# MorphIQ-Labs/VectorWave

Hardware: AMD Instinct MI355X
Metric: Msamples/sec MODWT fwd+inv db4 L=6, batch 4096×4096 fp64 @ 1/2/4/8 GPU (higher is better)
Workload: dtype f64

## Files before the change

vectorwave_amd/csrc/vw_capi.cpp:

```cpp
#include "../../include/vectorwave_amd.h"
#include "vw_internal.h"
#include "vw_deep.h"

#include <algorithm>
#include <cmath>
#include <cstdarg>
#include <cstdio>
#include <cstring>
#include <map>
#include <mutex>
#include <set>
#include <string>
#include <thread>
#include <vector>

using namespace vw;

static thread_local std::string t_err;
static thread_local int64_t t_err_index = -1;
static thread_local int64_t t_signal_base = 0;

static vw_status fail(vw_status code, const char* fmt, ...) {
  char buf[512];
  va_list ap;
  va_start(ap, fmt);
  vsnprintf(buf, sizeof(buf), fmt, ap);
  va_end(ap);
  t_err = buf;
  if (code != VW_ERR_NONFINITE) t_err_index = -1;
  return code;
}

static vw_status ok() {
  t_err.clear();
  t_err_index = -1;
  return VW_OK;
}

#define VW_HIP(call)                                                                         \
  do {                                                                                       \
    hipError_t e_ = (call);                                                                  \
    if (e_ != hipSuccess) return fail(VW_ERR_DEVICE, "%s: %s", #call, hipGetErrorString(e_)); \
  } while (0)

#define VW_TRY(expr)                      \
  do {                                    \
    vw_status s_ = (expr);                \
    if (s_ != VW_OK) return s_;           \
  } while (0)

struct TimedLaunch {
  std::string family;
  hipEvent_t start, stop;
  bool graph_owned = false;
};

struct Tuning {
  int nv = 4;
  bool fwd_persist = true;
  int fwd_buf = 0;
  bool force_tiled = false;
  int fwd_rev = 0, inv_rev = 0;
  int dma_nt = -1;
  int fwd_tile = 0;
  bool multi = true;
  int multi_div = 4;
  int multi_tile = 0;
  int inv_buf = 0;
  int inv_tile = 0;
  int multi_rblk = 1;
  int multi_pf = 1;
  int multi_pad = 1;
  int multi_inv_tile = 0;
  int multi_ni = 4;
  bool no_sweep = false;
  int sweep_qc = kSweepChunk;
  int unroll_max = kMaxTaps;
  int blk = 10;
  bool deep = true;
  bool deep_inv = false;
  int deep_lds = 80;
  int deep_waves = 4;
  int deep_pf_fwd = 1;
  int deep_pf_inv = 1;
  int fwd_nv = 0;
  int inv_nv = 0;
  int sweep2 = 3;
  int sweep2_ka = 8;
  int sweep2_uc = 2048;
  int sweep2_r = 0;
  int sweep2_minb = 64;
  int blk_fwd8 = 1;
  int ref_grid = 0;
  int mfma = 0;
};

static bool set_tuning(Tuning& t, const char* key, int v) {
  const Tuning d;
  const std::string k(key);
  if (k == "VW_NV") t.nv = v < 0 ? d.nv : v <= 4 ? 4 : 8;
  else if (k == "VW_FWD_PERSIST") t.fwd_persist = v < 0 ? d.fwd_persist : v != 0;
  else if (k == "VW_FWD_BUF") t.fwd_buf = v < 0 ? d.fwd_buf : v;
  else if (k == "VW_FORCE_TILED") t.force_tiled = v > 0;
  else if (k == "VW_FWD_REV") t.fwd_rev = v < 0 ? 0 : v;
  else if (k == "VW_INV_REV") t.inv_rev = v < 0 ? 0 : v;
  else if (k == "VW_DMA_NT") t.dma_nt = v < 0 ? d.dma_nt : v;
  else if (k == "VW_FWD_TILE") t.fwd_tile = v < 0 ? 0 : v;
  else if (k == "VW_MULTI") t.multi = v < 0 ? d.multi : v != 0;
  else if (k == "VW_MULTI_DIV") t.multi_div = v <= 0 ? d.multi_div : v;
  else if (k == "VW_MULTI_TILE") t.multi_tile = v < 0 ? 0 : v;
  else if (k == "VW_INV_BUF") t.inv_buf = v < 0 ? 0 : v;
  else if (k == "VW_INV_TILE") t.inv_tile = v < 0 ? 0 : v;
  else if (k == "VW_MULTI_RBLK") t.multi_rblk = v < 0 ? d.multi_rblk : v;
  else if (k == "VW_MULTI_PF") t.multi_pf = v < 0 ? d.multi_pf : v;
  else if (k == "VW_MULTI_PAD") t.multi_pad = v < 0 ? d.multi_pad : v;
  else if (k == "VW_MULTI_INV_TILE") t.multi_inv_tile = v < 0 ? 0 : v;
  else if (k == "VW_MULTI_NI") t.multi_ni = v < 0 ? d.multi_ni : v == 4 ? 4 : 8;
  else if (k == "VW_NO_SWEEP") t.no_sweep = v > 0;
  else if (k == "VW_SWEEP_QC") t.sweep_qc = v >= 16 ? v : d.sweep_qc;
  else if (k == "VW_UNROLL_MAX") t.unroll_max = v < 0 ? d.unroll_max : v;
  else if (k == "VW_BLK") t.blk = v < 0 ? d.blk : v;
  else if (k == "VW_DEEP") { t.deep = v < 0 ? d.deep : v != 0; t.deep_inv = v < 0 ? d.deep_inv : v != 0; }
  else if (k == "VW_DEEP_INV") t.deep_inv = v < 0 ? d.deep_inv : v != 0;
  else if (k == "VW_DEEP_LDS") t.deep_lds = v <= 0 ? d.deep_lds : v;
  else if (k == "VW_DEEP_WAVES") t.deep_waves = v <= 0 ? d.deep_waves : v;
  else if (k == "VW_DEEP_PF_FWD") t.deep_pf_fwd = v <= 0 ? d.deep_pf_fwd : std::min(v, 16);
  else if (k == "VW_DEEP_PF_INV") t.deep_pf_inv = v <= 0 ? d.deep_pf_inv : std::min(v, 16);
  else if (k == "VW_FWD_NV") t.fwd_nv = v < 0 ? d.fwd_nv : v;
  else if (k == "VW_INV_NV") t.inv_nv = v < 0 ? d.inv_nv : v;
  else if (k == "VW_SWEEP2") t.sweep2 = v < 0 ? d.sweep2 : v;
  else if (k == "VW_SWEEP2_KA") t.sweep2_ka = v == 16 ? 16 : v == 8 ? 8 : d.sweep2_ka;
  else if (k == "VW_SWEEP2_UC") t.sweep2_uc = v >= 32 ? v : d.sweep2_uc;
  else if (k == "VW_SWEEP2_R") t.sweep2_r = v == 32 ? 32 : 0;
  else if (k == "VW_SWEEP2_MINB") t.sweep2_minb = v < 0 ? d.sweep2_minb : v;
  else if (k == "VW_BLK_FWD8") t.blk_fwd8 = v < 0 ? d.blk_fwd8 : v;
  else if (k == "VW_MFMA") t.mfma = v < 0 ? d.mfma : v;
  else if (k == "VW_REF_GRID") t.ref_grid = v < 0 ? d.ref_grid : v;
  else return false;
  return true;
}

static const char* const kTuningKeys[] = {
    "VW_NV", "VW_FWD_PERSIST", "VW_FWD_BUF", "VW_FORCE_TILED", "VW_FWD_REV", "VW_INV_REV",
    "VW_FWD_TILE", "VW_MULTI", "VW_MULTI_DIV", "VW_MULTI_TILE", "VW_INV_BUF", "VW_INV_TILE", "VW_MULTI_RBLK", "VW_MULTI_PF", "VW_MULTI_PAD", "VW_MULTI_INV_TILE", "VW_NO_SWEEP", "VW_SWEEP_QC",
    "VW_UNROLL_MAX", "VW_BLK", "VW_FWD_NV",
    "VW_INV_NV", "VW_DEEP", "VW_DEEP_INV", "VW_DEEP_LDS", "VW_DEEP_WAVES", "VW_DEEP_PF_FWD", "VW_DEEP_PF_INV",
    "VW_SWEEP2", "VW_SWEEP2_KA", "VW_SWEEP2_UC", "VW_SWEEP2_R", "VW_SWEEP2_MINB", "VW_BLK_FWD8",
    "VW_DMA_NT", "VW_MULTI_NI", "VW_MFMA", "VW_REF_GRID"};

static Tuning read_tuning() {
  Tuning t;
  for (const char* k : kTuningKeys) {
    const char* e = getenv(k);
    if (!e) continue;
    const int v = (*e == '\0') ? 1 : atoi(e);
    set_tuning(t, k, v);
  }
  return t;
}

struct vw_graph;
struct vw_ctx;
static void kill_pipelines_of(vw_ctx* c);

struct vw_ctx {
  int device = 0;
  hipStream_t stream = nullptr;
  bool own_stream = false;
  bool capturing = false;
  unsigned ws_gen = 0;
  Tuning tune;
  int cus = 256;
  std::recursive_mutex mu;
  void* ws = nullptr;
  size_t ws_bytes = 0;
  void* ws2 = nullptr;
  size_t ws2_bytes = 0;
  unsigned long long* bad = nullptr;
  bool timing = false;
  std::vector<TimedLaunch> pending;
  std::vector<TimedLaunch> captured;
  std::vector<hipEvent_t> event_pool;
  std::map<std::string, std::pair<double, int64_t>> totals;
  std::set<vw_graph*> graphs;
  std::vector<std::pair<void*, size_t>> stage;
  void* med = nullptr;
  size_t med_bytes = 0;
  int* nf = nullptr;
  int64_t nf_rows = 0;
};

struct vw_graph {
  vw_ctx* ctx = nullptr;
  int device = 0;
  unsigned ws_gen = 0;
  std::vector<TimedLaunch> timed;
  hipGraph_t graph = nullptr;
  hipGraphExec_t exec = nullptr;
};

static void release_graph(vw_graph* gr) {
  for (auto& t : gr->timed) { hipEventDestroy(t.start); hipEventDestroy(t.stop); }
  gr->timed.clear();
  if (gr->exec) hipGraphExecDestroy(gr->exec);
  if (gr->graph) hipGraphDestroy(gr->graph);
  gr->exec = nullptr;
  gr->graph = nullptr;
}

struct vw_stream {
  vw_ctx* ctx = nullptr;
  std::vector<double> lo, hi;
  int L = 0;
  int boundary = 0;
  int levels = 0;
  int64_t last_batch = -1;
  bool hist_init = false;
  std::vector<double*> hist;
  std::vector<double*> snap;
  std::vector<int> hist_len;
};

static hipEvent_t pool_event(vw_ctx* c) {
  if (!c->event_pool.empty()) {
    hipEvent_t e = c->event_pool.back();
    c->event_pool.pop_back();
    return e;
  }
  hipEvent_t e = nullptr;
  if (hipEventCreate(&e) != hipSuccess) return nullptr;
  return e;
}

static bool capture_event(hipStream_t st, hipEvent_t ev) {
  hipStreamCaptureStatus status;
  unsigned long long id = 0;
  hipGraph_t g = nullptr;
  const hipGraphNode_t* deps = nullptr;
  size_t ndeps = 0;
  if (hipStreamGetCaptureInfo_v2(st, &status, &id, &g, &deps, &ndeps) == hipSuccess &&
      status == hipStreamCaptureStatusActive && g) {
    hipGraphNode_t node = nullptr;
    if (hipGraphAddEventRecordNode(&node, g, deps, ndeps, ev) == hipSuccess &&
        hipStreamUpdateCaptureDependencies(st, &node, 1, hipStreamSetCaptureDependencies) == hipSuccess)
      return true;
  }
  (void)hipGetLastError();
  if (hipEventRecordWithFlags(ev, st, hipEventRecordExternal) == hipSuccess) return true;
  (void)hipGetLastError();
  return false;
}

struct LaunchTimer {
  vw_ctx* c;
  TimedLaunch tl;
  bool on;
  LaunchTimer(vw_ctx* ctx, const char* family) : c(ctx), on(ctx->timing) {
    if (!on) return;
    tl.family = family;
    if (c->capturing) {
      tl.graph_owned = true;
      tl.start = tl.stop = nullptr;
      if (hipEventCreate(&tl.start) != hipSuccess || hipEventCreate(&tl.stop) != hipSuccess ||
          !capture_event(c->stream, tl.start)) {
        if (tl.start) hipEventDestroy(tl.start);
        if (tl.stop) hipEventDestroy(tl.stop);
        on = false;
      }
      return;
    }
    tl.start = pool_event(c);
    tl.stop = pool_event(c);
    if (!tl.start || !tl.stop) { on = false; return; }
    hipEventRecord(tl.start, c->stream);
  }
  ~LaunchTimer() {
    if (!on) return;
    if (tl.graph_owned) {
      if (capture_event(c->stream, tl.stop)) {
        c->captured.push_back(tl);
      } else {
        hipEventDestroy(tl.start);
        hipEventDestroy(tl.stop);
      }
      return;
    }
    hipEventRecord(tl.stop, c->stream);
    c->pending.push_back(tl);
  }
};

static void collect_timing(vw_ctx* c) {
  for (auto& tl : c->pending) {
    float ms = 0.f;
    if (hipEventSynchronize(tl.stop) == hipSuccess && hipEventElapsedTime(&ms, tl.start, tl.stop) == hipSuccess) {
      auto& t = c->totals[tl.family];
      t.first += ms;
      t.second += 1;
    }
    if (!tl.graph_owned) {
      c->event_pool.push_back(tl.start);
      c->event_pool.push_back(tl.stop);
    }
  }
  c->pending.clear();
}

static vw_status ensure_ws(vw_ctx* c, size_t bytes) {
  if (bytes <= c->ws_bytes) return VW_OK;
  if (c->capturing) return fail(VW_ERR_STATE, "workspace growth during capture: run the call once before capturing it");
  if (c->ws) {
    hipDeviceSynchronize();
    ++c->ws_gen;
    hipFree(c->ws);
    c->ws = nullptr;
    c->ws_bytes = 0;
  }
  size_t want = std::max(bytes, (size_t)1 << 20);
  VW_HIP(hipMalloc(&c->ws, want));
  c->ws_bytes = want;
  return VW_OK;
}

static vw_status ensure_nf(vw_ctx* c, int64_t B) {
  if (B <= c->nf_rows) return VW_OK;
  if (c->capturing) return fail(VW_ERR_STATE, "row-flag growth during capture: run the call once before capturing it");
  if (c->nf) {
    hipDeviceSynchronize();
    ++c->ws_gen;
    hipFree(c->nf);
    c->nf = nullptr;
    c->nf_rows = 0;
  }
  const int64_t rows = std::max<int64_t>(B, 4096);
  VW_HIP(hipMalloc(&c->nf, (size_t)rows * sizeof(int)));
  VW_HIP(hipMemset(c->nf, 0, (size_t)rows * sizeof(int)));
  VW_HIP(hipDeviceSynchronize());
  c->nf_rows = rows;
  return VW_OK;
}

static inline size_t align_up(size_t v, size_t a) { return (v + a - 1) / a * a; }
static inline int64_t round_up(int64_t v, int64_t a) { return (v + a - 1) / a * a; }


extern "C" int vw_max_levels(int64_t N, int L) {
  if (L <= 0 || N <= L) return 0;
  int max_level = 1;
  const long long lm1 = L - 1;
  while (max_level < 10) {
    const long long scaled = lm1 * (1LL << (max_level - 1)) + 1LL;
    if (scaled > N) break;
    max_level++;
  }
  return max_level - 1;
}

extern "C" int64_t vw_upsampled_length(int L, int level) {
  const int64_t up = (level <= 1) ? 1 : ((int64_t)1 << (level - 1));
  return (int64_t)(L - 1) * up + 1;
}

static void sym_decide(int wid, int L, int level, int* ap, int* dh, int* dp, int* dg) {
  int detailPlus = 1, deltaG = 0, deltaH = 0;
  const bool isHaar = L <= 2;
  int approxPlus = isHaar ? 1 : 0;
  if (isHaar) {
    deltaG = 0;
    deltaH = (level <= 1) ? 0 : -1;
  } else if (wid == VW_WID_DB6) {
    deltaH = (level <= 1) ? 0 : -1;
    deltaG = (level >= 3) ? 1 : 0;
  } else if (wid == VW_WID_DB8) {
    deltaH = (level <= 1) ? 0 : 1;
    deltaG = (level >= 2) ? 1 : 0;
  } else if (wid == VW_WID_SYM4) {
    approxPlus = 1; detailPlus = 0; deltaH = 0; deltaG = 0;
  } else if (wid == VW_WID_SYM8) {
    if (level <= 1) { deltaH = 0; deltaG = 0; }
    else if (level == 2) { deltaH = 1; deltaG = 0; }
    else { deltaH = 1; deltaG = 1; }
  } else if (wid == VW_WID_COIF2) {
    approxPlus = 1; deltaH = (level <= 1) ? 0 : 1; detailPlus = 0; deltaG = 0;
  } else if (wid == VW_WID_COIF3) {
    detailPlus = 0;
    if (level <= 1) { deltaH = 0; deltaG = 0; } else { deltaH = -1; deltaG = 1; }
  } else if (L >= 12) {
    if (level <= 1) { deltaH = 0; deltaG = 0; }
    else { const bool even = level % 2 == 0; deltaH = even ? 0 : -1; deltaG = even ? 0 : -1; }
  } else {
    if (level <= 1) { deltaH = 0; deltaG = 0; } else { deltaH = -1; deltaG = 0; }
  }
  *ap = approxPlus; *dh = deltaH; *dp = detailPlus; *dg = deltaG;
}

static int compute_tau(int base_len, int level) {
  const int lm1 = base_len - 1;
  if (level <= 1) return std::max(0, lm1 / 2);
  const long long up = 1LL << (level - 1);
  const long long Lj = (long long)lm1 * up + 1LL;
  const long long tau = (Lj - 1LL) / 2LL;
  if (tau < 0) return 0;
  if (tau > 2147483647LL) return 2147483647;
  return (int)tau;
}

static int next_pow2(int64_t n) {
  int64_t p = 1;
  while (p < n) p <<= 1;
  return (int)p;
}

static bool is_pow2(int64_t n) { return n > 0 && (n & (n - 1)) == 0; }

static void branch_extent(int N, int tmax, int L, int s, int dir, int off, int* hl, int* hr) {
  const long long reach = (long long)(L - 1) * s;
  long long mn, mx;
  if (dir > 0) { mn = off; mx = (long long)tmax + reach + off; }
  else { mn = (long long)off - reach; mx = (long long)tmax + off; }
  *hl = (int)std::max<long long>(*hl, -mn);
  *hr = (int)std::max<long long>(*hr, mx - (N - 1));
}

template <typename T> static constexpr int vec_width() { return 16 / (int)sizeof(T); }

static bool aligned16(const void* p) { return ((uintptr_t)p & 15u) == 0; }

extern "C" vw_status vw_ctx_create(int device, vw_ctx** out) {
  if (!out) return fail(VW_ERR_NULL, "out is null");
  int n = 0;
  VW_HIP(hipGetDeviceCount(&n));
  if (device < 0 || device >= n) return fail(VW_ERR_ARG, "device %d out of range (%d devices)", device, n);
  VW_HIP(hipSetDevice(device));
  vw_ctx* c = new vw_ctx();
  c->device = device;
  c->tune = read_tuning();
  { int n = 0; if (hipDeviceGetAttribute(&n, hipDeviceAttributeMultiprocessorCount, device) == hipSuccess && n > 0) c->cus = n; }
  if (hipStreamCreateWithFlags(&c->stream, hipStreamNonBlocking) != hipSuccess) {
    delete c;
    return fail(VW_ERR_DEVICE, "hipStreamCreate failed");
  }
  c->own_stream = true;
  if (hipMalloc(&c->bad, sizeof(unsigned long long)) != hipSuccess) {
    hipStreamDestroy(c->stream);
    delete c;
    return fail(VW_ERR_DEVICE, "hipMalloc failed");
  }
  *out = c;
  return ok();
}

// ... 425 lines not shown
}

template <typename T>
static void copy_taps(T* dst, const double* src, int L) {
  const double s = 1.0 / std::sqrt(2.0);
  for (int i = 0; i < L; ++i) dst[i] = (T)(src[i] * s);
  for (int i = L; i < kMaxTaps; ++i) dst[i] = T(0);
}

static vw_status capture_guard(vw_ctx* c, unsigned flags) {
  if (c->capturing && (flags & (VW_FLAG_VALIDATE | VW_FLAG_HOST_MEMORY | VW_FLAG_SYNC)))
    return fail(VW_ERR_STATE, "validation, host memory and SYNC cannot be captured");
  return VW_OK;
}

static vw_status read_bad(vw_ctx* c, unsigned long long* out) {
  VW_HIP(hipMemcpyAsync(out, c->bad, sizeof(unsigned long long), hipMemcpyDeviceToHost, c->stream));
  VW_HIP(hipStreamSynchronize(c->stream));
  return VW_OK;
}

static vw_status report_bad(unsigned long long bad, int64_t N) {
  if (bad == ~0ull) return VW_OK;
  const bool out = (bad >> 62) & 1ull;
  const unsigned long long flat = bad & ((1ull << 62) - 1);
  t_err_index = (int64_t)(flat % (unsigned long long)N);
  return fail(VW_ERR_NONFINITE, "%s contains non-finite value at index %lld (signal %lld)",
              out ? "coefficients" : "signal", (long long)(flat % (unsigned long long)N),
              (long long)(flat / (unsigned long long)N) + (long long)t_signal_base);
}

static bool fused_plan(const Tuning& tu, int64_t N, int V, int elem, int64_t lds_elems_extra, int* threads, int* nv,
                       int* lds, bool* fit, int nv_req = 0) {
  const int64_t nvec = (N + V - 1) / V;
  int want = tu.nv;
  if ((nvec + want - 1) / want > 512) want = 8;
  if (nv_req == 2 && nvec % 2 == 0 && nvec / 2 <= kMaxThreads) want = 2;
  const int64_t th = (nvec + want - 1) / want;
  if (th > kMaxThreads) return false;
  const int64_t bytes = lds_elems_extra * elem;
  if (bytes > kLdsBytes) return false;
  *nv = want;
  *threads = (int)th;
  *lds = (int)bytes;
  *fit = (int64_t)(want - 1) * th <= nvec;
  return true;
}


static void set_halo_images(LevelDesc& d, int64_t N, int64_t npow2, int V, int threads, int nv) {
  int64_t s_el = 0, e_el = N;
  d.il_a = 0; d.il_b = 1; d.ir_a = 0; d.ir_b = -1;
  switch (d.mode) {
    case kHaloPeriodic:
      d.il_a = 1; d.il_b = (int)-N; d.ir_a = 1; d.ir_b = (int)N;
      s_el = d.hr; e_el = N - d.hl;
      break;
    case kHaloSymmetric:
      d.il_a = -1; d.il_b = -1; d.ir_a = -1; d.ir_b = (int)(2 * N - 1);
      s_el = d.hl; e_el = N - d.hr;
      break;
    case kHaloFftPad:
      d.il_a = 1; d.il_b = (int)-npow2;
      e_el = npow2 - d.hl;
      break;
    default:
      break;
  }
  e_el = std::min<int64_t>(std::max<int64_t>(e_el, 0), N);
  d.vs = (int)((s_el + V - 1) / V);
  d.ve = (int)(e_el / V);
  d.own = (d.hl <= N && d.hr <= N && d.vs <= threads && (int64_t)d.ve >= (int64_t)(nv - 1) * threads) ? 1 : 0;
}

template <typename T>
static int multi_tile(const Tuning& tu) {
  constexpr int V = vec_width<T>();
  const int v = tu.multi_tile ? tu.multi_tile : (int)(16384 / sizeof(T));
  return v >= 64 * V ? v / V * V : 64 * V;
}

static std::vector<int> level_groups(const Tuning& tu, const std::vector<LevelDesc>& lv, int J, int L, int V, int tile,
                                     bool ok) {
  std::vector<int> g(J, 1);
  if (!ok || !tu.multi) return g;
  const int64_t cap = tile / tu.multi_div;
  for (int j = 1; j <= J;) {
    int n = 0;
    int64_t ext = 0;
    while (j + n <= J && n < kMaxGroup && lv[j + n - 1].mode == kHaloPeriodic) {
      const int64_t e2 = ext + round_up((int64_t)(L - 1) * lv[j + n - 1].s, V);
      if (e2 > cap) break;
      ext = e2;
      ++n;
    }
    if (n >= 2) {
      g[j - 1] = n;
      for (int k = 1; k < n; ++k) g[j - 1 + k] = 0;
      j += n;
    } else {
      ++j;
    }
  }
  return g;
}

template <typename T>
static bool sweepg_plan(const Tuning& tu, const std::vector<LevelDesc>& lv, int j, int levels, int L, int64_t N,
                        const std::vector<char>& in_group, const std::vector<int>& start_of, int* ka_out, int* r_out) {
  if (levels < 2 || levels > 3 || j < levels) return false;
  const int G = levels == 2 ? 2 : 4;
  const int64_t h = lv[j - levels].s;
  if (h < kSweepMinS || h % 32 != 0 || lv[j - 1].s != G * h) return false;
  for (int k = j - levels + 1; k <= j; ++k) {
    const LevelDesc& d = lv[k - 1];
    if (d.mode != kHaloPeriodic || d.dir_a != 1 || d.dir_d != 1 || d.off_a != 0 || d.off_d != 0) return false;
    if (k < j && (in_group[k] || start_of[k] != 0)) return false;
  }
  const int R = (h % 64 == 0 && tu.sweep2_r != 32) ? 64 : 32;
  const int kmin = (levels == 2 ? 1 : 2) * (L - 1);
  for (int ka : {L <= 17 ? tu.sweep2_ka : 16, 16}) {
    for (int r : {R, 32}) {
      const int64_t kb = (int64_t)G * ka;
      const int64_t lds = (levels == 2 ? 1 : 2) * 3 * kb * r * (int64_t)sizeof(T);
      if (kb < kmin || lds > kLdsBytes || h % r != 0) continue;
      if (N % (G * h) != 0 || (2 * kb + 2 * L) * G * h > N) continue;
      if (N / h < (int64_t)tu.sweep2_minb * kb) continue;
      *ka_out = ka;
      *r_out = r;
      return true;
    }
  }
  return false;
}

constexpr int kDeepTile = 128;

template <typename T>
static int deep_plan(const Tuning& tu, const std::vector<LevelDesc>& lv, int jlo, int jhi, int L, int64_t N,
                     bool inverse, DeepArgs<T>* a) {
  constexpr int V = vec_width<T>();
  const int C = 64 / (int)sizeof(T);
  const int g = jhi - jlo + 1;
  if (!(inverse ? tu.deep_inv : tu.deep) || g < 1 || g > kMaxGroup || !has_unrolled_taps(L)) return 0;
  const int P = lv[jlo - 1].s;
  if (P < C || P % C != 0 || N % P != 0 || N / P < 2 * kDeepTile) return 0;
  for (int j = jlo; j <= jhi; ++j)
    if (lv[j - 1].mode != kHaloPeriodic) return 0;
  (void)V;
  int caps[2 * kMaxGroup] = {}, nr = 0;
  int64_t reach = 0;
  const int D = inverse ? tu.deep_pf_inv : tu.deep_pf_fwd;
  for (int k = 0; k < g; ++k) {
    const int64_t H = (int64_t)(L - 1) << k;
    reach += H;
    const bool dma_fed = inverse ? (k == g - 1) : (k == 0);
    caps[k] = dma_fed ? (int)round_up(H + (D + 1) * kDeepTile, 16) : (int)(H + kDeepTile);
    if (inverse) caps[g + k] = (int)round_up(H + (D + 1) * kDeepTile, 16);
  }
  nr = inverse ? 2 * g : g;
  int64_t pos = 0;
  for (int r = 0; r < nr; ++r) pos += caps[r];
  const int64_t bytes = pos * 64;
  if (bytes > (int64_t)tu.deep_lds * 1024 || bytes > kLdsBytes) return 0;
  if (a) {
    a->P = P; a->C = C; a->nq = (int)(N / P); a->nb = P / C; a->g = g; a->N = (int)N;
    a->warm = (int)round_up(reach, kDeepTile);
    a->depth = D;
    int64_t o = 0;
    for (int r = 0; r < nr; ++r) { a->cap[r] = caps[r]; a->off[r] = (int)(o * C); o += caps[r]; }
  }
  return (int)bytes;
}

template <typename T>
static void deep_segments(const Tuning& tu, int cus, int64_t B, DeepArgs<T>* a) {
  const int64_t wg0 = B * a->nb;
  int64_t seg = std::max<int64_t>(1, ((int64_t)tu.deep_waves * cus + wg0 - 1) / wg0);
  seg = std::min<int64_t>(seg, std::max<int64_t>(1, a->nq / (4 * (int64_t)a->warm)));
  a->seg = (int)seg;
  a->seglen = (int)round_up((a->nq + seg - 1) / seg, kDeepTile);
  a->seg = (int)((a->nq + a->seglen - 1) / a->seglen);
}

template <typename T>
struct ScanPlane {
  const T* p;
  int64_t ld;
  int len;
};

template <typename T>
static vw_status ref_nonfinite(vw_ctx* c, const std::vector<ScanPlane<T>>& planes, RefArgs<T>& r,
                               bool inverse, bool flagged) {
  const int64_t B = r.B, N = r.N;
  if ((int)planes.size() > kRefPlanes) return fail(VW_ERR_ARG, "too many planes for the non-finite scan");
  int64_t grid = std::min<int64_t>(B, c->tune.ref_grid > 0 ? c->tune.ref_grid : 2LL * c->cus);
  grid = std::max<int64_t>(1, std::min<int64_t>(grid, ((int64_t)512 << 20) / (2 * N * (int64_t)sizeof(T))));
  VW_TRY(ensure_nf(c, B));
  VW_TRY(ensure_ws(c, (size_t)grid * 2 * (size_t)N * sizeof(T)));
  LaunchTimer lt(c, flagged ? "ref_nonfinite" : "ref_nonfinite_scan");
  hipError_t e;
  if (!flagged) {
    RefScan<T> s;
    memset(&s, 0, sizeof(s));
    for (const auto& p : planes) {
      s.p[s.np] = p.p;
      s.ld[s.np] = p.ld;
      s.len[s.np] = p.len;
      ++s.np;
    }
    s.B = B; s.N = (int)N; s.chunks = ref_scan_chunks((int)N); s.flag = c->nf;
    e = launch_flag_nonfinite<T>(s, c->stream);
    if (e != hipSuccess) return fail(VW_ERR_DEVICE, "non-finite scan launch failed: %s", hipGetErrorString(e));
  }
  r.flag = c->nf;
  r.scratch = reinterpret_cast<T*>(c->ws);
  e = launch_ref_cascade<T>(r, (int)grid, inverse, c->stream);
  if (e != hipSuccess) return fail(VW_ERR_DEVICE, "reference-arithmetic launch failed: %s", hipGetErrorString(e));
  return VW_OK;
}

static hipError_t mfma_forward(const FwdArgs<float>& a, int lds, hipStream_t st) { return launch_forward_mfma(a, lds, st); }
static hipError_t mfma_forward(const FwdArgs<double>&, int, hipStream_t) { return hipErrorNotSupported; }
static hipError_t mfma_inverse(const InvArgs<float>& a, int lds, hipStream_t st) { return launch_inverse_mfma(a, lds, st); }
static hipError_t mfma_inverse(const InvArgs<double>&, int, hipStream_t) { return hipErrorNotSupported; }

static int ref_mode(int boundary) {
  return boundary == VW_PERIODIC ? kHaloPeriodic : boundary == VW_ZERO_PADDING ? kHaloZero : kHaloSymmetric;
}

template <typename T>
static vw_status forward_impl(vw_ctx* c, const T* x, int64_t B, int64_t N, int64_t ldx, const double* lo,
                              const double* hi, int L, int boundary, int J, unsigned flags, T* details, T* approx,
                              bool single_level, int mode_override, T* const* hist, bool hist_update,
                              T* const* hist_snap = nullptr, bool hist_first = false) {
  constexpr int V = vec_width<T>();
  VW_TRY(capture_guard(c, flags));
  const bool fma = flags & VW_FLAG_FMA;
  const bool validate = flags & VW_FLAG_VALIDATE;
  const int64_t nvec = (N + V - 1) / V;

  std::vector<LevelDesc> lv(J);
  int max_hl = 0;
  const int npow2 = next_pow2(N);
  for (int j = 1; j <= J; ++j) {
    LevelDesc& d = lv[j - 1];
    memset(&d, 0, sizeof(d));
    d.s = 1 << (j - 1);
    const int64_t Lj = vw_upsampled_length(L, j);
    d.hl = (int)(Lj - 1);
    d.hr = 0;
    d.hist_len = (int)(Lj - 1);
    if (boundary == VW_PERIODIC) {
      d.mode = kHaloPeriodic;
      if ((flags & VW_FLAG_FFT_SWITCH) && !single_level && !(N < 64 || Lj > N / 2) && N >= 1024 &&
          (double)Lj > N * (1.0 / 8.0) && !is_pow2(N))
        d.mode = kHaloFftPad;
    } else {
      d.mode = boundary == VW_ZERO_PADDING ? kHaloZero : kHaloSymmetric;
    }
    if (mode_override >= 0) d.mode = mode_override;
    max_hl = std::max(max_hl, d.hl);
  }
  if ((flags & VW_FLAG_REF_NONFINITE) && hist && hist_update && hist_snap && !hist_first && J >= 2)
    for (int j = 0; j < J; ++j)
      if (lv[j].hist_len > 0)
        VW_HIP(hipMemcpyAsync(hist_snap[j], hist[j], (size_t)B * lv[j].hist_len * sizeof(T), hipMemcpyDeviceToDevice,
                              c->stream));

  const int hlpad = (int)round_up(max_hl, V);
  int threads = 0, lds = 0, nv = 4;
  const Tuning& tu = c->tune;
  const bool persist_on = tu.fwd_persist;
  const bool ref_nf = (flags & VW_FLAG_REF_NONFINITE) && !validate && !single_level && J >= 2 &&
                      !(flags & VW_FLAG_FFT_SWITCH) && (!hist || !hist_update || hist_first || hist_snap);
  bool nf_probed = false;
  const bool io_aligned = (ldx % V == 0) && (N % V == 0) && aligned16(x) && aligned16(details) && aligned16(approx);
  auto persist_ok = [&](int th, int nvv, bool ft) {
    return persist_on && io_aligned && ft && nvv == 4 && !validate && !hist && (int64_t)th * nvv == nvec &&
           th % 64 == 0 && nvec % 64 == 0 && has_unrolled_taps(L) && J >= 1;
  };
  const int64_t region = round_up(hlpad + nvec * V + V, V);
  bool dbl = tu.fwd_buf ? tu.fwd_buf == 2 : true;
  bool fused = false, fit = false;
  const int fwd_nv2 = (tu.fwd_nv == 2 && io_aligned && L <= 8 && L <= tu.unroll_max && has_unrolled_taps(L) &&
                       !(tu.blk > 0 && L >= tu.blk)) ? 2 : 0;
  if (J <= kMaxLevels && !tu.force_tiled) {
    if (dbl) dbl = fused_plan(tu, N, V, sizeof(T), 2 * region, &threads, &nv, &lds, &fit, fwd_nv2);
    if (dbl && !tu.fwd_buf && !fma && !persist_ok(threads, nv, fit)) dbl = false;
    fused = dbl || fused_plan(tu, N, V, sizeof(T), region, &threads, &nv, &lds, &fit, fwd_nv2);
  }
  if (fused && nv == 2 && !(fit && (int64_t)threads * 2 == nvec)) return fail(VW_ERR_STATE, "NV=2 plan without full slabs");
  if (fused) {
    for (int j = 0; j < J; ++j) set_halo_images(lv[j], N, npow2, V, threads, nv);
    FwdArgs<T> a;
    memset(&a, 0, sizeof(a));
    a.x = x; a.ldx = ldx; a.details = details; a.approx = approx; a.B = B; a.N = (int)N; a.J = J;
    a.npow2 = npow2; a.hlpad = hlpad; a.region1 = dbl ? (int)region : 0;
    a.vec_io = (ldx % V == 0) && (N % V == 0) && aligned16(x) && aligned16(details) && aligned16(approx);
    a.unrolled = a.vec_io && fit && L <= tu.unroll_max;
    a.validate = validate; a.bad = c->bad;
    a.rev = tu.fwd_rev;
    a.dma_nt = tu.dma_nt >= 0 ? tu.dma_nt : (B <= 2LL * c->cus ? 1 : 0);
    for (int j = 0; j < J; ++j) a.hist[j] = hist ? hist[j] : nullptr;
    a.hist_update = hist_update ? 1 : 0;
    a.taps = L;
    copy_taps(a.lo, lo, L);
    copy_taps(a.hi, hi, L);
    for (int j = 0; j < J; ++j) a.lv[j] = lv[j];
    if (validate) VW_HIP(hipMemsetAsync(c->bad, 0xFF, sizeof(unsigned long long), c->stream));
    const bool persist = dbl && a.unrolled && persist_ok(threads, nv, fit);
    int blk_lds = 0;
    if (tu.blk > 0 && L >= tu.blk && a.unrolled && !validate && !hist && (int64_t)threads * nv == nvec &&
        (nv == 4 || (nv == 8 && tu.blk_fwd8))) {
      bool okb = true;
      int hlv = 0;
      for (int j = 0; j < J; ++j) {
        if (lv[j].mode != kHaloPeriodic) okb = false;
        hlv = std::max<int>(hlv, (int)(((int64_t)(L - 1) * lv[j].s + V - 1) / V));
      }
      if (round_up(hlv, 16) <= nvec) hlv = (int)round_up(hlv, 16);
      const int mJ = std::max(1, lv[J - 1].s / V);
      if (nvec % ((int64_t)nv * mJ) != 0 || hlv > nvec) okb = false;
      auto buf_of = [&](int tight) {
        int64_t bf = 0;
        for (int j = 0; j < J; ++j) {
          int sh, pd;
          blk_layout_host(lv[j].s / V, nv, &sh, &pd, tight);
          const int64_t u = hlv + nvec - 1;
          bf = std::max(bf, u + (u >> sh) * pd + 1);
        }
        return bf;
      };
      int64_t buf = buf_of(0);
      if (buf * 16 + 2 * L * (int64_t)sizeof(T) > kLdsBytes && nv >= 8) {
        a.blk_tight = 1;
        buf = buf_of(1);
      }
      if (okb && buf * 16 <= kLdsBytes) {
        const bool two = 2 * buf * 16 <= 80 * 1024;
        a.region1 = two ? (int)(buf * V) : 0;
        a.hlpad = hlv * V;
        a.tap_lds = (int)(buf * V * (two ? 2 : 1));
        blk_lds = (int)(buf * 16 * (two ? 2 : 1)) + 2 * L * (int)sizeof(T);
        if (blk_lds > kLdsBytes) blk_lds = 0;
      }
    }
    int mfma_lds = 0;
    if constexpr (std::is_same<T, float>::value) {
      bool ok = (tu.mfma & 1) && fma && !single_level && a.vec_io && !validate && !hist && mfma_supported(L, N);
      for (int j = 0; ok && j < J; ++j) ok = lv[j].mode == kHaloPeriodic;
      const int H = ok ? mfma_halo(L, J) : 0;
      const int region = ok ? mfma_region((int)N + H) : 0;
      const int scratch = 8 * 256 + 4;
      if (ok && H <= N && (int64_t)(region + 2 * L + scratch) * 4 <= kLdsBytes) {
        a.hlpad = H;
        a.tap_lds = region;
        mfma_lds = (int)((region + 2 * L + scratch) * 4);
      }
    }
    if (ref_nf && !mfma_lds && (blk_lds || persist)) {
      VW_TRY(ensure_nf(c, B));
      a.nf_flag = c->nf;
      nf_probed = true;
    }
    {
      LaunchTimer lt(c, "forward");
      hipError_t e = mfma_lds ? mfma_forward(a, mfma_lds, c->stream)
                   : blk_lds ? launch_forward_blk<T>(a, threads, blk_lds, fma, nv, c->stream)
                   : persist ? launch_forward_persist<T>(a, threads, lds, fma, nv, c->stream)
                             : launch_forward_fused<T>(a, threads, lds, fma, nv, c->stream);
      if (e != hipSuccess) return fail(VW_ERR_DEVICE, "forward launch failed: %s", hipGetErrorString(e));
    }
  } else {
    for (int j = 1; hist && j <= J; ++j)
      if (lv[j - 1].hist_len > N) return fail(VW_ERR_UNSUPPORTED, "streaming block shorter than level %d history", j);
    const int tile_max = tu.fwd_tile ? tu.fwd_tile / V * V : 256 * kNV * V;
    const size_t plane = (size_t)B * (size_t)N;
    const vw_status st = ensure_ws(c, 2 * plane * sizeof(T) + 256);
    if (st != VW_OK) return st;
    T* tmp[2] = {reinterpret_cast<T*>(c->ws), reinterpret_cast<T*>(c->ws) + plane};
    if (validate) VW_HIP(hipMemsetAsync(c->bad, 0xFF, sizeof(unsigned long long), c->stream));
    const T* src = x;
    int64_t lda = ldx;
    const int mtile = multi_tile<T>(tu);
    const std::vector<int> groups = level_groups(tu, lv, J, L, V, mtile, !validate && !hist);
    for (int j = 1; j <= J; ++j) {
      T* const nxt = (src == tmp[0]) ? tmp[1] : tmp[0];
      if (groups[j - 1] == 1 && !validate && !hist && (lda % V) == 0 && aligned16(src) && aligned16(details) &&
          aligned16(approx) && deep_plan<T>(tu, lv, j, j, L, N, false, nullptr)) {
        int je = j;
        while (je < J && groups[je] == 1 && deep_plan<T>(tu, lv, j, je + 1, L, N, false, nullptr)) ++je;
        DeepArgs<T> d;
        memset(&d, 0, sizeof(d));
        const int lds = deep_plan<T>(tu, lv, j, je, L, N, false, &d);
        deep_segments<T>(tu, c->cus, B, &d);
        d.src = src; d.lda = lda; d.B = B; d.taps = L;
        d.out = (je == J) ? approx : nxt;
        if (ref_nf && je == J) {
          VW_TRY(ensure_nf(c, B));
          d.nf_flag = c->nf;
          nf_probed = true;
        }
        for (int k = 0; k < d.g; ++k) d.out_d[k] = details + (size_t)(j - 1 + k) * plane;
        copy_taps(d.lo, lo, L);
        copy_taps(d.hi, hi, L);
        {
          LaunchTimer lt(c, "forward_level");
          hipError_t e = launch_deep<T>(d, lds, fma, false, c->stream);
          if (e != hipSuccess) return fail(VW_ERR_DEVICE, "forward deep launch failed: %s", hipGetErrorString(e));
        }
        src = d.out;
        lda = N;
        j = je;
        continue;
      }
      if (groups[j - 1] >= 2) {
        const int g = groups[j - 1], je = j + g - 1;
        MultiArgs<T> m;
        memset(&m, 0, sizeof(m));
        m.src_a = src; m.lda = lda;
        m.out_a = (je == J) ? approx : nxt;
        bool al = aligned16(src) && aligned16(m.out_a);
        for (int k = 0; k < g; ++k) {
          m.out_d[k] = details + (size_t)(j - 1 + k) * plane;
          al = al && aligned16(m.out_d[k]);
        }
        m.ext[g] = 0;
        for (int k = g - 1; k >= 0; --k)
          m.ext[k] = m.ext[k + 1] + (int)round_up((int64_t)(L - 1) * lv[j - 1 + k].s, V);
        m.B = B; m.N = (int)N; m.tile = mtile; m.nlev = g; m.s0 = lv[j - 1].s;
        m.region = (int)round_up(m.ext[0] + mtile + V, V);
        m.vec_io = (N % V == 0) && (lda % V == 0) && al;
        m.taps = L;
        copy_taps(m.lo, lo, L);
        copy_taps(m.hi, hi, L);
        {
          LaunchTimer lt(c, "forward_level");
          hipError_t e = launch_forward_multi<T>(m, (int)(2 * m.region * sizeof(T)), fma, c->stream);
          if (e != hipSuccess) return fail(VW_ERR_DEVICE, "forward multi-level launch failed: %s", hipGetErrorString(e));
        }
        src = m.out_a;
        lda = N;
        j = je;
        continue;
      }
      LevelArgs<T> a;
      memset(&a, 0, sizeof(a));
      a.lv = lv[j - 1];
      const int hp = (int)round_up(a.lv.hl, V);
      const int64_t fit = ((int64_t)kLdsBytes / (int64_t)sizeof(T) - hp - 2 * V) / V * V;
      const int tile = (int)std::min<int64_t>(tile_max, fit);
      if (tile < 64 * V) return fail(VW_ERR_UNSUPPORTED, "level %d halo (%d samples) exceeds LDS", j, a.lv.hl);
      const int64_t elems = hp + tile + V;
      a.src_a = src; a.lda = lda;
      a.out_a = (j == J) ? approx : nxt;
      a.out_d = details + (size_t)(j - 1) * plane;
      a.hist = hist ? hist[j - 1] : nullptr;
      a.B = B; a.N = (int)N; a.tile = tile; a.hlpad = hp;
      a.vec_io = (N % V == 0) && (lda % V == 0) && aligned16(src) && aligned16(a.out_a) && aligned16(a.out_d);
      a.validate = validate; a.bad = c->bad; a.npow2 = npow2; a.taps = L;
      copy_taps(a.lo, lo, L);
      copy_taps(a.hi, hi, L);
      const bool sweep = a.lv.s >= kSweepMinS && has_unrolled_taps(L) && !tu.no_sweep;
      {
        LaunchTimer lt(c, "forward_level");
        hipError_t e;
        if (sweep) {
          a.tile = tu.sweep_qc;
          e = launch_forward_sweep<T>(a, fma, c->stream);
        } else {
          e = launch_forward_level<T>(a, (int)(elems * sizeof(T)), fma, c->stream);
        }
        if (e != hipSuccess) return fail(VW_ERR_DEVICE, "forward level launch failed: %s", hipGetErrorString(e));
      }
      if (hist && hist_update) {
        hipError_t e = launch_history_update<T>(src, lda, hist[j - 1], hist[j - 1], B, (int)N, a.lv.hist_len,
                                                c->stream);
        if (e != hipSuccess) return fail(VW_ERR_DEVICE, "history update failed: %s", hipGetErrorString(e));
      }
      src = a.out_a;
      lda = N;
    }
  }
  if (ref_nf) {
    std::vector<ScanPlane<T>> planes{{approx, N, 0}};
    RefArgs<T> r;
    memset(&r, 0, sizeof(r));
    r.x = x; r.ldx = ldx; r.details = details; r.approx = approx;
    r.B = B; r.N = (int)N; r.J = J; r.L = L; r.mode = ref_mode(boundary);
    if (hist) {
      r.hist_mode = 1;
      r.hist_first = hist_first ? 1 : 0;
      for (int j = 0; j < J; ++j) {
        const int hl = lv[j].hist_len;
        r.hist_len[j] = hl;
        r.hist_old[j] = hist_first ? nullptr : (hist_update ? hist_snap[j] : hist[j]);
        r.hist_new[j] = hist_update ? hist[j] : nullptr;
      }
    }
    copy_taps(r.lo, lo, L);
    copy_taps(r.hi, hi, L);
    VW_TRY(ref_nonfinite<T>(c, planes, r, false, nf_probed));
  }
  if (validate) {
    unsigned long long bad = 0;
    vw_status st = read_bad(c, &bad);
    if (st != VW_OK) return st;
    st = report_bad(bad, N);
    if (st != VW_OK) return st;
  }
  if (flags & VW_FLAG_SYNC) VW_HIP(hipStreamSynchronize(c->stream));
  return VW_OK;
}

template <typename T>
static vw_status inverse_impl(vw_ctx* c, const T* details, const T* approx, int64_t B, int64_t N, const double* lo,
                              const double* hi, int L, int wid, int boundary, int J, unsigned detail_mask,
                              int approx_zero, unsigned flags, T* y, bool single_level, const T* thr, int soft,
                              int64_t thr_ld = 0) {
  constexpr int V = vec_width<T>();
  VW_TRY(capture_guard(c, flags));
  const bool fma = flags & VW_FLAG_FMA;
  const int64_t nvec = (N + V - 1) / V;
  const int tmax = (int)(nvec * V - 1);
  const bool pair = single_level || boundary == VW_ZERO_PADDING;
  const bool ref_nf = (flags & VW_FLAG_REF_NONFINITE) && !single_level && J >= 2;
  bool nf_probed = false;

  std::vector<LevelDesc> lv(J);
  int max_hl = 0, max_hr = 0;
  for (int j = 1; j <= J; ++j) {
    LevelDesc& d = lv[j - 1];
    memset(&d, 0, sizeof(d));
    d.s = 1 << (j - 1);
    d.use_d = (detail_mask >> (j - 1)) & 1u;
    d.mode = boundary == VW_PERIODIC ? kHaloPeriodic : boundary == VW_ZERO_PADDING ? kHaloZero : kHaloSymmetric;
    if (boundary == VW_SYMMETRIC && !single_level) {
      int ap, dh, dp, dg;
      sym_decide(wid, L, j, &ap, &dh, &dp, &dg);
      const int tauH = compute_tau(L, j) + dh;
      const int tauG = compute_tau(L, j) + dg;
      d.dir_a = ap ? 1 : -1; d.off_a = ap ? -tauH : tauH;
      d.dir_d = dp ? 1 : -1; d.off_d = dp ? -tauG : tauG;
    } else if (boundary == VW_SYMMETRIC) {
      const int dir = (flags & VW_FLAG_BATCH_SYM_INVERSE) ? 1 : -1;
      d.dir_a = d.dir_d = dir; d.off_a = d.off_d = 0;
    } else {
      d.dir_a = d.dir_d = 1; d.off_a = d.off_d = 0;
    }
    int hl = 0, hr = 0;
    branch_extent((int)N, tmax, L, d.s, d.dir_a, d.off_a, &hl, &hr);
    branch_extent((int)N, tmax, L, d.s, d.dir_d, d.off_d, &hl, &hr);
    d.hl = hl; d.hr = hr;
    max_hl = std::max(max_hl, hl);
    max_hr = std::max(max_hr, hr);
  }
  const int hlpad = (int)round_up(max_hl, V);
  const int64_t region = round_up(hlpad + nvec * V + max_hr + V, V);
  int threads = 0, lds = 0, nv = 4;
  const Tuning& tu = c->tune;
  const bool blk_pref = tu.blk > 0 && L >= tu.blk && boundary == VW_PERIODIC;
  bool db = !pair && (tu.inv_buf ? tu.inv_buf == 2 : (B <= 2LL * c->cus && !blk_pref));
  bool fused = false, fit = false;
  const bool inv_io = (N % V == 0) && aligned16(details) && aligned16(approx) && aligned16(y);
  const int inv_nv2 = (tu.inv_nv == 2 && inv_io && L <= 8 && L <= tu.unroll_max && has_unrolled_taps(L)) ? 2 : 0;
  if (!tu.force_tiled) {
    if (pair || db) fused = fused_plan(tu, N, V, sizeof(T), 2 * region, &threads, &nv, &lds, &fit, inv_nv2);
    if (!fused && !pair) {
      db = false;
      fused = fused_plan(tu, N, V, sizeof(T), region, &threads, &nv, &lds, &fit, inv_nv2);
    }
  }
  if (fused) {
    for (int j = 0; j < J; ++j) set_halo_images(lv[j], N, 0, V, threads, nv);
    InvArgs<T> a;
    memset(&a, 0, sizeof(a));
    a.details = details; a.approx = approx; a.y = y; a.B = B; a.N = (int)N; a.J = J;
    a.db = db ? 1 : 0;
    a.hlpad_a = hlpad; a.hlpad_d = hlpad; a.region_d = (int)region;
    a.vec_io = (N % V == 0) && aligned16(details) && aligned16(approx) && aligned16(y);
    a.unrolled = a.vec_io && fit && L <= tu.unroll_max;
    a.pair = pair; a.approx_zero = approx_zero; a.thr = thr; a.thr_ld = thr_ld; a.soft = soft; a.taps = L;
    a.rev = tu.inv_rev;
    if (tu.blk > 0 && L >= tu.blk && nv != 2 && !pair && !db && boundary == VW_PERIODIC && a.unrolled &&
        (int64_t)threads * nv == nvec) {
      bool okb = true;
      int64_t buf = 0;
      const int mJ = std::max(1, lv[J - 1].s / V);
      if (nvec % ((int64_t)nv * mJ) != 0) okb = false;
      int64_t buf_t = 0;
      for (int j = 0; j < J && okb; ++j) {
        if (lv[j].dir_a != 1 || lv[j].dir_d != 1 || lv[j].off_a != 0 || lv[j].off_d != 0) okb = false;
        const int64_t hrv = ((int64_t)(L - 1) * lv[j].s + V - 1) / V;
        if (hrv > nvec) okb = false;
        int sh, pd;
        const int64_t u = nvec + hrv - 1;
        blk_layout_host(lv[j].s / V, nv, &sh, &pd);
        buf = std::max(buf, u + (u >> sh) * pd + 1);
        blk_layout_host(lv[j].s / V, nv, &sh, &pd, 1);
        buf_t = std::max(buf_t, u + (u >> sh) * pd + 1);
      }
      const int64_t taps_b = 2 * L * (int64_t)sizeof(T);
      if (okb && buf * 16 + taps_b > kLdsBytes && nv >= 8 && buf_t * 16 + taps_b <= kLdsBytes) {
        a.blk_tight = 1;
        buf = buf_t;
      }
      if (okb && buf * 16 + taps_b <= kLdsBytes) {
        a.blk = 1;
        a.tap_lds = (int)(buf * V);
        lds = (int)(buf * 16) + 2 * L * (int)sizeof(T);
      }
    }
    copy_taps(a.lo, lo, L);
    copy_taps(a.hi, hi, L);
    for (int j = 0; j < J; ++j) a.lv[j] = lv[j];
    int mfma_lds = 0;
    if constexpr (std::is_same<T, float>::value) {
      bool ok = (tu.mfma & 2) && fma && !pair && boundary == VW_PERIODIC && a.vec_io && mfma_supported(L, N);
      for (int j = 0; ok && j < J; ++j) ok = lv[j].dir_a == 1 && lv[j].dir_d == 1 && lv[j].off_a == 0 && lv[j].off_d == 0;
      const int H = ok ? mfma_halo(L, J) : 0;
      const int region = ok ? mfma_region((int)N + H) : 0;
      if (ok && H <= N && (int64_t)(region + 2 * L) * 4 <= kLdsBytes) {
        a.hlpad_a = H;
        a.tap_lds = region;
        mfma_lds = (int)((region + 2 * L) * 4);
      }
    }
    if (ref_nf && !mfma_lds && !a.pair && !a.db) {
      VW_TRY(ensure_nf(c, B));
      a.nf_flag = c->nf;
      nf_probed = true;
    }
    LaunchTimer lt(c, "inverse");
    hipError_t e = mfma_lds ? mfma_inverse(a, mfma_lds, c->stream) : launch_inverse_fused<T>(a, threads, lds, fma, nv, c->stream);
    if (e != hipSuccess) return fail(VW_ERR_DEVICE, "inverse launch failed: %s", hipGetErrorString(e));
  } else {
    const int tile_max = tu.inv_tile ? tu.inv_tile / V * V : 1024;
    const size_t plane = (size_t)B * (size_t)N;
    const vw_status st = ensure_ws(c, 2 * plane * sizeof(T) + 256);
    if (st != VW_OK) return st;
    T* tmp[2] = {reinterpret_cast<T*>(c->ws), reinterpret_cast<T*>(c->ws) + plane};
    const T* cur = approx_zero ? nullptr : approx;
    const int mtile = tu.multi_inv_tile >= 64 * V ? tu.multi_inv_tile / V * V : multi_tile<T>(tu);
    const std::vector<int> groups = level_groups(tu, lv, J, L, V, mtile, !pair && boundary == VW_PERIODIC);
    std::vector<int> start_of(J + 1, 0);
    for (int j = 1; j <= J; ++j) {
      if (groups[j - 1] < 2) continue;
      int64_t ext = 0;
      for (int k = 0; k < groups[j - 1]; ++k) ext += round_up((int64_t)(L - 1) * lv[j - 1 + k].s, V);
      if ((mtile + ext) / V <= (int64_t)kMultiInvNI * 256) start_of[j + groups[j - 1] - 1] = j;
    }
    std::vector<char> in_group(J + 1, 0);
    for (int e = 1; e <= J; ++e)
      for (int k = start_of[e]; start_of[e] > 0 && k <= e; ++k) in_group[k] = 1;
    for (int j = J; j >= 1; --j) {
      T* const nxt = (cur == tmp[0]) ? tmp[1] : tmp[0];
      if (!pair && boundary == VW_PERIODIC && !in_group[j] && aligned16(cur) && aligned16(details) &&
          aligned16(y) && deep_plan<T>(tu, lv, j, j, L, N, true, nullptr)) {
        int jl = j;
        while (jl > 1 && !in_group[jl - 1] && deep_plan<T>(tu, lv, jl - 1, j, L, N, true, nullptr)) --jl;
        DeepArgs<T> d;
        memset(&d, 0, sizeof(d));
        const int lds = deep_plan<T>(tu, lv, jl, j, L, N, true, &d);
        deep_segments<T>(tu, c->cus, B, &d);
        d.src = cur; d.lda = N; d.B = B; d.taps = L; d.soft = soft;
        d.out = (jl == 1) ? y : nxt;
        for (int k = 0; k < d.g; ++k) {
          const LevelDesc& ld = lv[jl - 1 + k];
          d.src_d[k] = ld.use_d ? details + (size_t)(jl - 1 + k) * plane : nullptr;
          d.thr[k] = thr ? thr + (size_t)(jl - 1 + k) * (size_t)thr_ld : nullptr;
        }
        copy_taps(d.lo, lo, L);
        copy_taps(d.hi, hi, L);
        {
          LaunchTimer lt(c, "inverse_level");
          hipError_t e = launch_deep<T>(d, lds, fma, true, c->stream);
          if (e != hipSuccess) return fail(VW_ERR_DEVICE, "inverse deep launch failed: %s", hipGetErrorString(e));
        }
        cur = d.out;
        j = jl;
        continue;
      }
      if (start_of[j] > 0) {
        const int j0 = start_of[j], g = j - j0 + 1;
        MultiArgs<T> m;
        memset(&m, 0, sizeof(m));
        m.src_a = cur;
        m.out_a = (j0 == 1) ? y : nxt;
        if (ref_nf && j0 == 1) {
          VW_TRY(ensure_nf(c, B));
          m.nf_flag = c->nf;
          nf_probed = true;
        }
        bool al = aligned16(cur) && aligned16(m.out_a);
        for (int k = 0; k < g; ++k) {
          const LevelDesc& d = lv[j0 - 1 + k];
          m.src_d[k] = d.use_d ? details + (size_t)(j0 - 1 + k) * plane : nullptr;
          m.thr[k] = thr ? thr + (size_t)(j0 - 1 + k) * (size_t)thr_ld : nullptr;
          al = al && aligned16(m.src_d[k]);
          m.ext[k] = (k > 0 ? m.ext[k - 1] : 0) + (int)round_up((int64_t)(L - 1) * d.s, V);
        }
        m.B = B; m.N = (int)N; m.tile = mtile; m.nlev = g; m.s0 = lv[j0 - 1].s;
        m.region = (int)round_up(mtile + m.ext[g - 1] + V, V);
        m.vec_io = (N % V == 0) && al;
        m.soft = soft; m.taps = L;
        m.rblk = tu.multi_rblk;
        m.pf = tu.multi_pf && m.vec_io && (int64_t)(mtile + m.ext[g - 1]) / V <= (int64_t)kMultiPF * 256;
        m.pad = tu.multi_pad && m.pf && m.rblk && has_unrolled_taps(L);
        if (m.pad) {
          const int nvmax = (mtile + m.ext[g - 1]) / V + 1;
          m.region = (nvmax + nvmax / 8 + 1) * V;
        }
        m.slack = 160;
        m.ni = kMultiInvNI;
        if (tu.multi_ni == 4 && sizeof(T) == 8 && m.pad) {
          auto fits = [&](int64_t t) {
            if ((t + m.ext[g - 1]) / V > (int64_t)kMultiPF * 256) return false;
            for (int k = 0; k < g; ++k) {
              const int64_t s = lv[j0 - 1 + k].s, M = s % V == 0 ? s / V : 0;
              const int64_t nv = (t + (k > 0 ? m.ext[k - 1] : 0)) / V;
              const bool blk = M == 1 || M == 2 || M == 4 || M == 8;
              if (blk ? (nv + 4 * M - 1) / (4 * M) * M > 256 : nv > 4 * 256) return false;
            }
            return true;
          };
          int64_t t = mtile;
          while (t >= 512 && !fits(t)) t -= 64 * V;
          if (t >= 512) {
            m.ni = 4;
            m.tile = (int)t;
            const int nvmax = (int)((t + m.ext[g - 1]) / V) + 1;
            m.region = (nvmax + nvmax / 4 + 1) * V;
          }
        }
        copy_taps(m.lo, lo, L);
        copy_taps(m.hi, hi, L);
        LaunchTimer lt(c, "inverse_level");
        hipError_t e = launch_inverse_multi<T>(m, (int)((2 * m.region + m.slack * V) * sizeof(T)), fma, c->stream);
        if (e != hipSuccess) return fail(VW_ERR_DEVICE, "inverse multi-level launch failed: %s", hipGetErrorString(e));
        cur = m.out_a;
        j = j0;
        continue;
      }
      if (tu.sweep2 && !tu.deep_inv && !tu.no_sweep && !pair && j >= 2 && has_unrolled_taps(L)) {
        int G = 0, ka = 0, R = 0;
        for (int levels = std::min(tu.sweep2 >= 3 ? 3 : 2, j); levels >= 2 && !G; --levels)
          if (sweepg_plan<T>(tu, lv, j, levels, L, N, in_group, start_of, &ka, &R)) G = levels;
        if (G) {
          const LevelDesc& lj = lv[j - 1];
          LevelArgs<T> a;
          memset(&a, 0, sizeof(a));
          a.lv = lj;
          a.src_a = cur;
          a.src_d = lj.use_d ? details + (size_t)(j - 1) * plane : nullptr;
          a.use_d = lj.use_d;
          a.thr = thr ? thr + (size_t)(j - 1) * (size_t)thr_ld : nullptr;
          a.src_d2 = lv[j - 2].use_d ? details + (size_t)(j - 2) * plane : nullptr;
          a.use_d2 = lv[j - 2].use_d;
          a.thr2 = thr ? thr + (size_t)(j - 2) * (size_t)thr_ld : nullptr;
          if (G == 3) {
            a.src_d3 = lv[j - 3].use_d ? details + (size_t)(j - 3) * plane : nullptr;
            a.use_d3 = lv[j - 3].use_d;
            a.thr3 = thr ? thr + (size_t)(j - 3) * (size_t)thr_ld : nullptr;
          }
          a.soft = soft;
          a.out_a = (j == G) ? y : nxt;
          a.B = B; a.N = (int)N; a.taps = L;
          const int kb = (G == 2 ? 2 : 4) * ka;
          a.tile = (int)round_up(tu.sweep2_uc, kb);
          copy_taps(a.lo, lo, L);
          copy_taps(a.hi, hi, L);
          LaunchTimer lt(c, "inverse_level");
          hipError_t e = launch_inverse_sweepg<T>(a, G == 2 ? 2 : 4, ka, R, fma, c->stream);
          if (e != hipSuccess) return fail(VW_ERR_DEVICE, "inverse level-group launch failed: %s", hipGetErrorString(e));
          cur = a.out_a;
          j -= G - 1;
          continue;
        }
      }
      LevelArgs<T> a;
      memset(&a, 0, sizeof(a));
      a.lv = lv[j - 1];
      const int hp = (int)round_up(a.lv.hl, V);
      const int64_t fit = ((int64_t)kLdsBytes / (int64_t)sizeof(T) / 2 - hp - a.lv.hr - 2 * V) / V * V;
      const int tile = (int)std::min<int64_t>(tile_max, fit);
      if (tile < 64 * V) return fail(VW_ERR_UNSUPPORTED, "level %d halo exceeds LDS", j);
      const int64_t reg = round_up(hp + tile + a.lv.hr + V, V);
      a.src_a = cur;
      a.src_d = a.lv.use_d ? details + (size_t)(j - 1) * plane : nullptr;
      a.use_d = a.lv.use_d;
      a.out_a = (j == 1) ? y : nxt;
      a.B = B; a.N = (int)N; a.tile = tile; a.hlpad = hp; a.hlpad_d = hp; a.region_d = (int)reg;
      a.pair = pair; a.thr = thr ? thr + (size_t)(j - 1) * (size_t)thr_ld : nullptr; a.soft = soft; a.taps = L;
      a.vec_io = (N % V == 0) && aligned16(a.out_a) && aligned16(a.src_a) && aligned16(a.src_d);
      copy_taps(a.lo, lo, L);
      copy_taps(a.hi, hi, L);
      LaunchTimer lt(c, "inverse_level");
      hipError_t e;
      if (a.lv.s >= kSweepMinS && has_unrolled_taps(L) && !tu.no_sweep) {
        a.tile = tu.sweep_qc;
        e = launch_inverse_sweep<T>(a, fma, c->stream);
      } else {
        e = launch_inverse_level<T>(a, (int)(2 * reg * sizeof(T)), fma, c->stream);
      }
      if (e != hipSuccess) return fail(VW_ERR_DEVICE, "inverse level launch failed: %s", hipGetErrorString(e));
      cur = a.out_a;
    }
  }
  if (ref_nf) {
    std::vector<ScanPlane<T>> planes{{y, N, 0}};
    RefArgs<T> r;
    memset(&r, 0, sizeof(r));
    r.x = approx_zero ? nullptr : approx; r.det_in = details; r.y = y;
    r.thr = thr; r.thr_ld = thr_ld; r.soft = soft;
    r.B = B; r.N = (int)N; r.J = J; r.L = L; r.mode = ref_mode(boundary);
    copy_taps(r.lo, lo, L);
    copy_taps(r.hi, hi, L);
    for (int j = 0; j < J; ++j) r.lv[j] = lv[j];
    VW_TRY(ref_nonfinite<T>(c, planes, r, true, nf_probed));
  }
  if (flags & VW_FLAG_SYNC) VW_HIP(hipStreamSynchronize(c->stream));
  return VW_OK;
}

struct Staging {
  vw_ctx* c;
  size_t used_block = 0, used_off = 0;
  explicit Staging(vw_ctx* ctx) : c(ctx) {}
  ~Staging() {
    hipStreamSynchronize(c->stream);
    if (c->stage.size() > 1) {
      auto big = std::max_element(c->stage.begin(), c->stage.end(),
                                  [](const std::pair<void*, size_t>& a, const std::pair<void*, size_t>& b) {
                                    return a.second < b.second;
                                  });
      const auto keep = *big;
      for (auto& blk : c->stage)
        if (blk.first != keep.first) hipFree(blk.first);
      c->stage.assign(1, keep);
    }
  }
  vw_status carve(size_t bytes, void** out) {
    bytes = align_up(std::max<size_t>(bytes, 16), 256);
    for (; used_block < c->stage.size(); ++used_block, used_off = 0) {
      auto& blk = c->stage[used_block];
      if (used_off + bytes <= blk.second) {
        *out = static_cast<char*>(blk.first) + used_off;
        used_off += bytes;
        return VW_OK;
      }
    }
    size_t carved = bytes;
    for (size_t k = 0; k < used_block && k < c->stage.size(); ++k) carved += c->stage[k].second;
    if (used_block < c->stage.size()) carved += used_off;
    const size_t want = std::max({carved, (size_t)4 << 20});
    void* p = nullptr;
    VW_HIP(hipMalloc(&p, want));
    c->stage.push_back({p, want});
    used_block = c->stage.size() - 1;
    used_off = bytes;
    *out = p;
    return VW_OK;
  }
  template <typename T>
  vw_status in(const T* host, size_t count, T** dev) {
    void* p = nullptr;
    VW_TRY(carve(count * sizeof(T), &p));
    if (host && count) VW_HIP(hipMemcpyAsync(p, host, count * sizeof(T), hipMemcpyHostToDevice, c->stream));
    *dev = reinterpret_cast<T*>(p);
    return VW_OK;
  }
  template <typename T>
  vw_status in_planes(const T* host, size_t planes, size_t count, size_t host_stride, T** dev) {
    void* p = nullptr;
    VW_TRY(carve(planes * count * sizeof(T), &p));
    if (host && count && planes)
      VW_HIP(hipMemcpy2DAsync(p, count * sizeof(T), host, host_stride * sizeof(T), count * sizeof(T), planes,
                              hipMemcpyHostToDevice, c->stream));
    *dev = reinterpret_cast<T*>(p);
    return VW_OK;
  }
  template <typename T>
  vw_status out(T* host, const T* dev, size_t count) {
    if (host && count) VW_HIP(hipMemcpyAsync(host, dev, count * sizeof(T), hipMemcpyDeviceToHost, c->stream));
    return VW_OK;
  }
// ... 1021 lines not shown
```

vectorwave_amd/csrc/vw_device.h:

```cpp
#pragma once
#include <hip/hip_runtime.h>
#include <cstdint>
#include <type_traits>
#include "vw_internal.h"

#pragma clang fp contract(off)

namespace vw {

template <typename T> struct VT;
template <> struct VT<double> { typedef double v __attribute__((ext_vector_type(2))); static constexpr int V = 2; };
template <> struct VT<float>  { typedef float  v __attribute__((ext_vector_type(4))); static constexpr int V = 4; };

__device__ __forceinline__ double fma_t(double a, double b, double c) { return __builtin_fma(a, b, c); }
__device__ __forceinline__ float fma_t(float a, float b, float c) { return __builtin_fmaf(a, b, c); }

template <bool FMA, typename T>
__device__ __forceinline__ T madd(T acc, T x, T f) {
  if constexpr (FMA) return fma_t(x, f, acc);
  else return acc + x * f;
}

#ifndef VW_PK_F32
#define VW_PK_F32 0
#endif
#ifndef VW_PK_F32_FWD
#define VW_PK_F32_FWD 1
#endif
constexpr bool kPkFwd = VW_PK_F32_FWD != 0;
template <bool FMA, bool PK = (VW_PK_F32 != 0), typename T, typename X>
__device__ __forceinline__ void vmadd(T* acc, const X& x, T f) {
  if constexpr (PK && std::is_same<T, float>::value) {
    typedef float f2 __attribute__((ext_vector_type(2)));
    const f2 fv = {f, f};
#pragma unroll
    for (int h = 0; h < 2; ++h) {
      f2 a = {acc[2 * h], acc[2 * h + 1]};
      const f2 xv = {x[2 * h], x[2 * h + 1]};
      if constexpr (FMA) a = __builtin_elementwise_fma(xv, fv, a);
      else a = a + xv * fv;
      acc[2 * h] = a[0];
      acc[2 * h + 1] = a[1];
    }
  } else {
#pragma unroll
    for (int e = 0; e < VT<T>::V; ++e) acc[e] = madd<FMA>(acc[e], x[e], f);
  }
}

template <typename T>
__device__ __forceinline__ T load_uniform(const T* q) {
  typedef const __attribute__((address_space(4))) T* cptr;
  return *(cptr)(q);
}

__device__ __forceinline__ bool finite_t(double v) { return __builtin_isfinite(v); }
__device__ __forceinline__ bool finite_t(float v) { return __builtin_isfinite(v); }

__device__ __forceinline__ int sym_index(int idx, int n) {
  if (idx >= 0 && idx < n) return idx;
  int period = 2 * n;
  idx = ((idx % period) + period) % period;
  if (idx >= n) idx = period - idx - 1;
  return idx;
}

#pragma clang diagnostic push
#pragma clang diagnostic ignored "-Wint-to-pointer-cast"
template <typename vec>
__device__ __forceinline__ vec lds_vec_at(unsigned a) {
  return *(const __attribute__((address_space(3))) vec*)a;
}
#pragma clang diagnostic pop
template <typename T>
__device__ __forceinline__ unsigned lds_base(const T* p) {
  unsigned a = (unsigned)(uintptr_t)p;
  asm volatile("" : "+v"(a));
  return a;
}

__device__ __forceinline__ void lds_barrier() {
  asm volatile("" ::: "memory");
  __builtin_amdgcn_s_waitcnt(0xC07F);
  __builtin_amdgcn_s_barrier();
  asm volatile("" ::: "memory");
}

__device__ __forceinline__ void wait_vmem() { __builtin_amdgcn_s_waitcnt(0x0F70); }

template <typename T>
__device__ __forceinline__ T halo_value_lds(const T* buf, int idx, int N, int mode, int npow2,
                                            const T* hist_b, int hist_len) {
  switch (mode) {
    case kHaloPeriodic: { int r = idx % N; if (r < 0) r += N; return buf[r]; }
    case kHaloSymmetric: return buf[sym_index(idx, N)];
    case kHaloFftPad: { int r = idx < 0 ? idx + npow2 : idx; return (r >= 0 && r < N) ? buf[r] : T(0); }
    case kHaloHistory: return (idx < 0 && idx >= -hist_len) ? hist_b[hist_len + idx] : T(0);
    default: return T(0);
  }
}

template <typename T>
__device__ __forceinline__ void fill_halo(T* buf, int N, int hl, int hr, int mode, int npow2,
                                          const T* hist_b, int hist_len) {
  const int total = hl + hr;
  if (mode == kHaloHistory) {
    for (int q = threadIdx.x; q < total; q += blockDim.x) {
      const int idx = q < hl ? q - hl : N + (q - hl);
      buf[idx] = (idx < 0 && idx >= -hist_len) ? hist_b[hist_len + idx] : T(0);
    }
    return;
  }
  for (int q = threadIdx.x; q < total; q += blockDim.x) {
    const int idx = q < hl ? q - hl : N + (q - hl);
    buf[idx] = halo_value_lds(buf, idx, N, mode, npow2, (const T*)nullptr, 0);
  }
}

constexpr int kWinTaps = 8;

__host__ __device__ constexpr int floor_div(int a, int b) { return a >= 0 ? a / b : -((-a + b - 1) / b); }

template <int C, int NC, typename F>
__device__ __forceinline__ void static_for(F&& f) {
  if constexpr (C < NC) {
    f(std::integral_constant<int, C>{});
    static_for<C + 1, NC>(f);
  }
}

template <typename T, int L, bool FMA, int S>
__device__ __forceinline__ void fwd_window(const T* buf, int t0, const T* lo, const T* hi,
                                           T (&al)[VT<T>::V], T (&ah)[VT<T>::V]) {
  constexpr int V = VT<T>::V;
  using vec = typename VT<T>::v;
  static_for<0, (L + kWinTaps - 1) / kWinTaps>([&](auto c) __attribute__((always_inline)) {
    constexpr int I0 = decltype(c)::value * kWinTaps;
    constexpr int I1 = (I0 + kWinTaps < L) ? I0 + kWinTaps : L;
    constexpr int A = floor_div(-(I1 - 1) * S, V) * V;
    constexpr int E = (floor_div(V - 1 - I0 * S, V) + 1) * V;
    constexpr int NE = E - A;
    T w[NE];
#pragma unroll
    for (int k = 0; k < NE / V; ++k) {
      vec v = *reinterpret_cast<const vec*>(buf + t0 + A + k * V);
#pragma unroll
      for (int e = 0; e < V; ++e) w[k * V + e] = v[e];
    }
    T fl[I1 - I0], fh[I1 - I0];
#pragma unroll
    for (int i = I0; i < I1; ++i) { fl[i - I0] = lo[i]; fh[i - I0] = hi[i]; }
#pragma unroll
    for (int i = I0; i < I1; ++i) {
      vmadd<FMA, kPkFwd>(al, &w[-i * S - A], fl[i - I0]);
      vmadd<FMA, kPkFwd>(ah, &w[-i * S - A], fh[i - I0]);
    }
  });
}

template <typename T, int L, bool FMA>
__device__ __forceinline__ void fwd_vec(const T* buf, int t0, int S, const T* lo, const T* hi, int taps,
                                        T (&al)[VT<T>::V], T (&ah)[VT<T>::V]) {
  constexpr int V = VT<T>::V;
  using vec = typename VT<T>::v;
  if constexpr (L > 0) {
    if (S == 1) { fwd_window<T, L, FMA, 1>(buf, t0, lo, hi, al, ah); return; }
    if constexpr (V == 4) {
      if (S == 2) { fwd_window<T, L, FMA, 2>(buf, t0, lo, hi, al, ah); return; }
    }
#pragma unroll
    for (int i = 0; i < L; ++i) {
      const vec v = *reinterpret_cast<const vec*>(buf + t0 - i * S);
      vmadd<FMA, kPkFwd>(al, v, lo[i]);
      vmadd<FMA, kPkFwd>(ah, v, hi[i]);
    }
  } else {
    for (int i = 0; i < taps; ++i) {
      const T fl = lo[i], fh = hi[i];
#pragma unroll
      for (int e = 0; e < V; ++e) {
        const T xv = buf[t0 + e - i * S];
        al[e] = madd<FMA>(al[e], xv, fl);
        ah[e] = madd<FMA>(ah[e], xv, fh);
      }
    }
  }
}

template <typename T, int L, bool FMA, int S, int DIR>
__device__ __forceinline__ void inv_window(const T* buf, int base, const T* f, T (&acc)[VT<T>::V]) {
  constexpr int V = VT<T>::V;
  using vec = typename VT<T>::v;
  static_for<0, (L + kWinTaps - 1) / kWinTaps>([&](auto c) __attribute__((always_inline)) {
    constexpr int I0 = decltype(c)::value * kWinTaps;
    constexpr int I1 = (I0 + kWinTaps < L) ? I0 + kWinTaps : L;
    constexpr int A = DIR > 0 ? floor_div(I0 * S, V) * V : floor_div(-(I1 - 1) * S, V) * V;
    constexpr int E = DIR > 0 ? (floor_div(V - 1 + (I1 - 1) * S, V) + 1) * V : (floor_div(V - 1 - I0 * S, V) + 1) * V;
    constexpr int NE = E - A;
    T w[NE];
#pragma unroll
    for (int k = 0; k < NE / V; ++k) {
      vec v = *reinterpret_cast<const vec*>(buf + base + A + k * V);
#pragma unroll
      for (int e = 0; e < V; ++e) w[k * V + e] = v[e];
    }
    T fc[I1 - I0];
#pragma unroll
    for (int i = I0; i < I1; ++i) fc[i - I0] = f[i];
#pragma unroll
    for (int i = I0; i < I1; ++i) vmadd<FMA>(acc, &w[DIR * i * S - A], fc[i - I0]);
  });
}

template <typename T, int L, bool FMA>
__device__ __forceinline__ void inv_branch(const T* buf, int t0, int S, int dir, int off, const T* f, int taps,
                                           T (&acc)[VT<T>::V]) {
  constexpr int V = VT<T>::V;
  using vec = typename VT<T>::v;
  if constexpr (L > 0) {
    if ((off & (V - 1)) == 0) {
      const int base = t0 + off;
      if (S == 1) {
        if (dir > 0) inv_window<T, L, FMA, 1, 1>(buf, base, f, acc);
        else inv_window<T, L, FMA, 1, -1>(buf, base, f, acc);
        return;
      }
      if constexpr (V == 4) {
        if (S == 2) {
          if (dir > 0) inv_window<T, L, FMA, 2, 1>(buf, base, f, acc);
          else inv_window<T, L, FMA, 2, -1>(buf, base, f, acc);
          return;
        }
      }
      const int step = dir * S;
#pragma unroll
      for (int i = 0; i < L; ++i) {
        const vec v = *reinterpret_cast<const vec*>(buf + base + i * step);
        vmadd<FMA>(acc, v, f[i]);
      }
      return;
    }
#pragma unroll
    for (int i = 0; i < L; ++i) {
#pragma unroll
      for (int e = 0; e < V; ++e) acc[e] = madd<FMA>(acc[e], buf[t0 + e + dir * i * S + off], f[i]);
    }
  } else {
    for (int i = 0; i < taps; ++i) {
      const T fi = f[i];
#pragma unroll
      for (int e = 0; e < V; ++e) acc[e] = madd<FMA>(acc[e], buf[t0 + e + dir * i * S + off], fi);
    }
  }
}

template <typename T, bool FMA>
__device__ __forceinline__ T pair_term(T h, T a, T g, T d) {
  if constexpr (FMA) return fma_t(h, a, g * d);
  else return h * a + g * d;
}

template <typename T, int L, bool FMA>
__device__ __forceinline__ void inv_pair(const T* A, const T* D, int t0, int S, int dir, const T* h, const T* g,
                                         int taps, T (&acc)[VT<T>::V]) {
  constexpr int V = VT<T>::V;
  using vec = typename VT<T>::v;
  if constexpr (L > 0) {
    if (S % V == 0) {
      const int step = dir * S;
#pragma unroll
      for (int i = 0; i < L; ++i) {
        const vec va = *reinterpret_cast<const vec*>(A + t0 + i * step);
        const vec vd = *reinterpret_cast<const vec*>(D + t0 + i * step);
#pragma unroll
        for (int e = 0; e < V; ++e) acc[e] = acc[e] + pair_term<T, FMA>(h[i], va[e], g[i], vd[e]);
        if ((i & 3) == 3) __builtin_amdgcn_sched_barrier(0);
      }
      return;
    }
#pragma unroll
    for (int i = 0; i < L; ++i) {
#pragma unroll
      for (int e = 0; e < V; ++e) {
        const int idx = t0 + e + dir * i * S;
        acc[e] = acc[e] + pair_term<T, FMA>(h[i], A[idx], g[i], D[idx]);
      }
      if ((i & 1) == 1) __builtin_amdgcn_sched_barrier(0);
    }
  } else {
    for (int i = 0; i < taps; ++i) {
#pragma unroll
      for (int e = 0; e < V; ++e) {
        const int idx = t0 + e + dir * i * S;
        acc[e] = acc[e] + pair_term<T, FMA>(h[i], A[idx], g[i], D[idx]);
      }
    }
  }
}

template <int L, int NV, typename F>
__device__ __forceinline__ void for_vecs(int nvec, F&& fn) {
  const int NT = blockDim.x;
#pragma unroll
  for (int k = 0; k < NV; ++k) {
    int w = threadIdx.x + k * NT;
    asm volatile("" : "+v"(w));
    if ((L > 0 && k < NV - 1) || w < nvec) fn(k, w);
    __builtin_amdgcn_sched_barrier(0);
  }
}

#ifndef VW_STORE_AUX
#define VW_STORE_AUX -1
#endif
#ifndef VW_LOAD_AUX
#define VW_LOAD_AUX -1
#endif
#ifndef VW_FWD_STORE_AUX
#define VW_FWD_STORE_AUX 16
#endif
#ifndef VW_BLK_NT_M
#define VW_BLK_NT_M 8
#endif
#ifndef VW_INV_STORE_AUX
#define VW_INV_STORE_AUX VW_STORE_AUX
#endif
typedef int vw_i4 __attribute__((ext_vector_type(4)));

__device__ __forceinline__ __amdgpu_buffer_rsrc_t row_rsrc(const void* p) {
  return __builtin_amdgcn_make_buffer_rsrc(const_cast<void*>(p), (short)0, 0x7fffffff, 0x00020000);
}

template <int AUX, typename V16, typename T>
__device__ __forceinline__ void stream_store(T* base, int i, V16 v) {
  if constexpr (AUX < 0) {
    __builtin_nontemporal_store(v, reinterpret_cast<V16*>(base) + i);
  } else {
    __builtin_amdgcn_raw_buffer_store_b128(__builtin_bit_cast(vw_i4, v), row_rsrc(base), i * 16, 0, AUX);
  }
}

template <typename V16, typename T>
__device__ __forceinline__ V16 stream_load(const T* base, int i) {
  if constexpr (VW_LOAD_AUX < 0) {
    return __builtin_nontemporal_load(reinterpret_cast<const V16*>(base) + i);
  } else {
    return __builtin_bit_cast(V16, __builtin_amdgcn_raw_buffer_load_b128(row_rsrc(base), i * 16, 0, VW_LOAD_AUX));
  }
}

template <int AUX = VW_STORE_AUX, typename T>
__device__ __forceinline__ void store_vec(T* __restrict__ dst, int t0, int N, bool vec_ok, const T (&v)[VT<T>::V]) {
  constexpr int V = VT<T>::V;
  using vec = typename VT<T>::v;
  if (vec_ok && t0 + V <= N) {
    vec o;
#pragma unroll
    for (int e = 0; e < V; ++e) o[e] = v[e];
    stream_store<AUX, vec>(dst, t0 / V, o);
  } else {
#pragma unroll
    for (int e = 0; e < V; ++e)
      if (t0 + e < N) dst[t0 + e] = v[e];
  }
}

template <typename T>
__device__ __forceinline__ void check_out(int validate, unsigned long long* bad, unsigned long long flat0, int t0,
                                          int N, const T (&v)[VT<T>::V]) {
  if (!validate) return;
  constexpr int V = VT<T>::V;
#pragma unroll
  for (int e = 0; e < V; ++e)
    if (t0 + e < N && !finite_t(v[e])) atomicMin(bad, (1ull << 62) | (flat0 + (unsigned long long)(t0 + e)));
}

template <typename T>
__device__ __forceinline__ T threshold_t(T c, T thr, int soft) {
  const T av = c < T(0) ? -c : c;
  if (soft) {
    if (av > thr) return c == T(0) ? c * (av - thr) : __builtin_copysign(av - thr, c);
    return T(0);
  }
  return av <= thr ? T(0) : c;
}

template <typename T, int NV>
__device__ __forceinline__ void load_row_regs(T (&r)[NV][VT<T>::V], const T* __restrict__ src, int N, int nvec,
                                              bool vec_ok, bool zero) {
  constexpr int V = VT<T>::V;
  using vec = typename VT<T>::v;
  const int NT = blockDim.x;
  if (zero) return;
  if (vec_ok) {
#pragma unroll
    for (int k = 0; k < NV; ++k) {
      int w = (int)threadIdx.x + k * NT;
      asm volatile("" : "+v"(w));
      w = min(w, nvec - 1);
      const vec v = stream_load<vec>(src, w);
#pragma unroll
      for (int e = 0; e < V; ++e) r[k][e] = v[e];
    }
  } else {
#pragma unroll
    for (int k = 0; k < NV; ++k) {
      const int w = threadIdx.x + k * NT;
      if (w < nvec) {
        const int t0 = w * V;
#pragma unroll
        for (int e = 0; e < V; ++e) r[k][e] = (t0 + e < N) ? src[t0 + e] : T(0);
      }
    }
  }
}

template <typename T>
__device__ __forceinline__ void halo_images(T* buf, int w, const typename VT<T>::v& o, int N, const LevelDesc& lv) {
  constexpr int V = VT<T>::V;
#pragma unroll
  for (int e = 0; e < V; ++e) {
    const int t = w * V + e;
    if (t < N) {
      const int l = lv.il_a * t + lv.il_b;
      const int r = lv.ir_a * t + lv.ir_b;
      if (l < 0 && l >= -lv.hl) buf[l] = o[e];
      if (r >= N && r < N + lv.hr) buf[r] = o[e];
    }
  }
}

template <typename T>
__device__ __forceinline__ void halo_fixed(T* buf, int N, const LevelDesc& lv, int npow2, const T* hist_b) {
  if (lv.mode == kHaloPeriodic || lv.mode == kHaloSymmetric) return;
  const int total = lv.hl + lv.hr;
  for (int q = threadIdx.x; q < total; q += blockDim.x) {
    const int idx = q < lv.hl ? q - lv.hl : N + (q - lv.hl);
    if (lv.mode == kHaloFftPad && idx < 0 && idx + npow2 < N) continue;
    T v = T(0);
    if (lv.mode == kHaloHistory && idx < 0 && idx >= -lv.hist_len) v = hist_b[lv.hist_len + idx];
    buf[idx] = v;
  }
}

template <typename T, int L, int NV, int MODE>
__device__ __forceinline__ void regs_to_level_m(T* buf, const T (&r)[NV][VT<T>::V], int nvec, int N,
                                                const LevelDesc& lv, T thr_b, int soft) {
  constexpr int V = VT<T>::V;
  using vec = typename VT<T>::v;
  const bool own = lv.own != 0;
  for_vecs<L, NV>(nvec, [&](int k, int w) {
    vec o;
#pragma unroll
    for (int e = 0; e < V; ++e) {
      if constexpr (MODE == 1) {
        T z = T(0);
        asm volatile("" : "+v"(z));
        o[e] = z;
      }
      else if constexpr (MODE == 2) o[e] = threshold_t(r[k][e], thr_b, soft);
      else o[e] = r[k][e];
    }
    if (L > 0 || w * V + V <= N) {
      *reinterpret_cast<vec*>(buf + w * V) = o;
    } else {
#pragma unroll
      for (int e = 0; e < V; ++e)
        if (w * V + e < N) buf[w * V + e] = o[e];
    }
    if (own && ((k == 0 && w < lv.vs) || (k == NV - 1 && w >= lv.ve))) halo_images(buf, w, o, N, lv);
  });
}

template <typename T, int L, int NV>
__device__ __forceinline__ void regs_to_level(T* buf, const T (&r)[NV][VT<T>::V], int nvec, int N, const LevelDesc& lv,
                                              int npow2, const T* hist_b, bool zero = false, const T* thr = nullptr,
                                              T thr_b = T(0), int soft = 0) {
  if (zero) regs_to_level_m<T, L, NV, 1>(buf, r, nvec, N, lv, thr_b, soft);
  else if (thr) regs_to_level_m<T, L, NV, 2>(buf, r, nvec, N, lv, thr_b, soft);
  else regs_to_level_m<T, L, NV, 0>(buf, r, nvec, N, lv, thr_b, soft);
  if (lv.own) {
    halo_fixed(buf, N, lv, npow2, hist_b);
  } else {
    lds_barrier();
    fill_halo(buf, N, lv.hl, lv.hr, lv.mode, npow2, hist_b, lv.hist_len);
  }
}

template <typename T, int L, bool FMA, int NV, int SC, typename Emit>
__device__ __forceinline__ void fwd_row_t(const T* buf, int nvec, int s, const T* lo, const T* hi, int taps,
                                          Emit&& emit) {
  constexpr int V = VT<T>::V;
  using vec = typename VT<T>::v;
  for_vecs<L, NV>(nvec, [&](int k, int w) {
    const int t0 = w * V;
    T al[V], ah[V];
#pragma unroll
    for (int e = 0; e < V; ++e) { al[e] = T(0); ah[e] = T(0); }
    if constexpr (L > 0 && SC > 0) {
      fwd_window<T, L, FMA, SC>(buf, t0, lo, hi, al, ah);
    } else if constexpr (L > 0) {
#pragma unroll
      for (int i = 0; i < L; ++i) {
        const vec v = *reinterpret_cast<const vec*>(buf + t0 - i * s);
        vmadd<FMA, kPkFwd>(al, v, lo[i]);
        vmadd<FMA, kPkFwd>(ah, v, hi[i]);
        if ((i & 3) == 3) __builtin_amdgcn_sched_barrier(0);
      }
    } else {
      fwd_vec<T, 0, FMA>(buf, t0, s, lo, hi, taps, al, ah);
    }
    emit(k, w, al, ah);
  });
}

template <typename T, int L, bool FMA, int NV, typename Emit>
__device__ __forceinline__ void fwd_row(const T* buf, int nvec, int s, const T* lo, const T* hi, int taps,
                                        Emit&& emit) {
  constexpr int V = VT<T>::V;
  if constexpr (L > 0) {
    if (s == 1) return fwd_row_t<T, L, FMA, NV, 1>(buf, nvec, s, lo, hi, taps, emit);
    if constexpr (V == 4) {
      if (s == 2) return fwd_row_t<T, L, FMA, NV, 2>(buf, nvec, s, lo, hi, taps, emit);
    }
  }
  fwd_row_t<T, L, FMA, NV, 0>(buf, nvec, s, lo, hi, taps, emit);
}

template <typename T, int L, bool FMA, int NV, int SC, int DIR>
__device__ __forceinline__ void inv_row_t(const T* buf, int nvec, int s, int dir, int off, const T* f, int taps,
                                          T (&acc)[NV][VT<T>::V]) {
  constexpr int V = VT<T>::V;
  using vec = typename VT<T>::v;
  for_vecs<L, NV>(nvec, [&](int k, int w) {
    const int t0 = w * V;
    if constexpr (L > 0 && SC > 0) {
      inv_window<T, L, FMA, SC, DIR>(buf, t0 + off, f, acc[k]);
    } else if constexpr (L > 0 && SC == 0) {
#pragma unroll
      for (int i = 0; i < L; ++i) {
        const vec v = *reinterpret_cast<const vec*>(buf + t0 + off + DIR * i * s);
        vmadd<FMA>(acc[k], v, f[i]);
        if ((i & 3) == 3) __builtin_amdgcn_sched_barrier(0);
      }
    } else {
      inv_branch<T, L, FMA>(buf, t0, s, dir, off, f, taps, acc[k]);
    }
#pragma unroll
    for (int e = 0; e < V; ++e) asm volatile("" : "+v"(acc[k][e]));
  });
}

template <typename T, int L, bool FMA, int NV>
__device__ __forceinline__ void inv_row(const T* buf, int nvec, int s, int dir, int off, const T* f, int taps,
                                        T (&acc)[NV][VT<T>::V]) {
  constexpr int V = VT<T>::V;
  if constexpr (L > 0) {
    if ((off & (V - 1)) == 0) {
      if (s == 1) {
        if (dir > 0) return inv_row_t<T, L, FMA, NV, 1, 1>(buf, nvec, s, dir, off, f, taps, acc);
        return inv_row_t<T, L, FMA, NV, 1, -1>(buf, nvec, s, dir, off, f, taps, acc);
      }
      if constexpr (V == 4) {
        if (s == 2) {
          if (dir > 0) return inv_row_t<T, L, FMA, NV, 2, 1>(buf, nvec, s, dir, off, f, taps, acc);
          return inv_row_t<T, L, FMA, NV, 2, -1>(buf, nvec, s, dir, off, f, taps, acc);
        }
      }
      if (dir > 0) return inv_row_t<T, L, FMA, NV, 0, 1>(buf, nvec, s, dir, off, f, taps, acc);
      return inv_row_t<T, L, FMA, NV, 0, -1>(buf, nvec, s, dir, off, f, taps, acc);
    }
  }
  inv_row_t<T, L, FMA, NV, -1, 1>(buf, nvec, s, dir, off, f, taps, acc);
}

template <typename T, int NV>
__device__ __forceinline__ void zero_regs(T (&r)[NV][VT<T>::V]) {
#pragma unroll
  for (int k = 0; k < NV; ++k)
#pragma unroll
    for (int e = 0; e < VT<T>::V; ++e) r[k][e] = T(0);
}

#ifndef VW_LONG_WAVES
#define VW_LONG_WAVES 4
#endif
#define VW_FUSED_W(L, W) ((L) <= 8 ? (W) : VW_LONG_WAVES)
#define VW_FUSED_BOUNDS(NV, W)                                                        \
  __attribute__((amdgpu_flat_work_group_size(1, ((NV) <= 4 && (NV) != 2) ? 512 : 1024), \
                 amdgpu_waves_per_eu((NV) == 2 ? 8 : (NV) <= 4 ? (W) : 4)))

template <typename T>
__device__ __forceinline__ T nf_step(T v, T z) {
  if constexpr (sizeof(T) == 8) return __builtin_fma(v, T(0), z);
  else return __builtin_fmaf(v, T(0), z);
}
template <typename T, int V>
__device__ __forceinline__ void nf_probe(T& z, const T (&v)[V]) {
#pragma unroll
  for (int e = 0; e < V; ++e) z = nf_step<T>(v[e], z);
}
template <typename T, int L, int NV, int V>
__device__ __forceinline__ void nf_probe_rows(T& z, const T (&v)[NV][V], int nvec) {
  for_vecs<L, NV>(nvec, [&](int k, int) { nf_probe<T, V>(z, v[k]); });
}
template <typename T>
__device__ __forceinline__ void nf_flag_row(int* flag, long long b, T z) {
  if (__any(z != z) && (threadIdx.x & 63) == 0) flag[b] = 1;
}

template <typename T, int L, bool FMA, int NV, bool VALIDATE, bool NFP = false>
__device__ __forceinline__ void fwd_level(const FwdArgs<T>& p, const T* X, int nvec, const LevelDesc& lv, T* dout,
                                          T* aout, bool vec_ok, unsigned long long flat0, T (&areg)[NV][VT<T>::V],
                                          T* nf = nullptr) {
  constexpr int V = VT<T>::V;
  const int N = p.N;
  fwd_row<T, L, FMA, NV>(X, nvec, lv.s, p.lo, p.hi, p.taps, [&](int k, int w, const T (&al)[V], const T (&ah)[V]) {
    const int t0 = w * V;
    store_vec<VW_FWD_STORE_AUX>(dout, t0, N, vec_ok, ah);
    if (aout) store_vec<VW_FWD_STORE_AUX>(aout, t0, N, vec_ok, al);
    if constexpr (VALIDATE) {
      check_out<T>(1, p.bad, flat0, t0, N, ah);
      check_out<T>(1, p.bad, flat0, t0, N, al);
    }
    if constexpr (NFP) {
      if (aout) nf_probe<T, V>(*nf, al);
    }
#pragma unroll
    for (int e = 0; e < V; ++e) areg[k][e] = al[e];
  });
}

template <typename T, int L, bool FMA, int NV, bool HIST>
__global__ void VW_FUSED_BOUNDS(NV, VW_FUSED_W(L, 8)) k_forward_fused(const FwdArgs<T> p) {
  constexpr int V = VT<T>::V;
  extern __shared__ __attribute__((aligned(16))) unsigned char smem[];
  T* X = reinterpret_cast<T*>(smem) + p.hlpad;
  T* Y = p.region1 ? reinterpret_cast<T*>(smem) + p.region1 + p.hlpad : X;
  const bool dbl = p.region1 != 0;
  const long long b = p.rev ? p.B - 1 - (long long)blockIdx.x : (long long)blockIdx.x;
  const int N = p.N;
  const int nvec = (N + V - 1) / V;
  const int NT = blockDim.x;
  const int tid = threadIdx.x;
  const bool vec_ok = (L > 0) || p.vec_io != 0;
  const unsigned long long flat0 = (unsigned long long)b * (unsigned long long)N;
  auto hist_of = [&](int j) -> const T* {
    if constexpr (!HIST) return nullptr;
    const LevelDesc& d = p.lv[j - 1];
    return d.mode == kHaloHistory ? p.hist[j - 1] + b * d.hist_len : nullptr;
  };

  T areg[NV][V];
  load_row_regs<T, NV>(areg, p.x + b * p.ldx, N, nvec, vec_ok, false);
  wait_vmem();
  if (p.validate) {
    for_vecs<L, NV>(nvec, [&](int k, int w) {
#pragma unroll
      for (int e = 0; e < V; ++e)
        if (w * V + e < N && !finite_t(areg[k][e])) atomicMin(p.bad, flat0 + (unsigned long long)(w * V + e));
    });
  }
  regs_to_level<T, L, NV>(X, areg, nvec, N, p.lv[0], p.npow2, hist_of(1));

  for (int j = 1; j <= p.J; ++j) {
    const LevelDesc lv = p.lv[j - 1];
    lds_barrier();
    T* dout = p.details + ((size_t)(j - 1) * (size_t)p.B + (size_t)b) * (size_t)N;
    T* aout = (j == p.J) ? p.approx + b * (size_t)N : nullptr;
    if (p.validate) fwd_level<T, L, FMA, NV, true>(p, X, nvec, lv, dout, aout, vec_ok, flat0, areg);
    else fwd_level<T, L, FMA, NV, false>(p, X, nvec, lv, dout, aout, vec_ok, flat0, areg);
    if (HIST && p.hist_update && lv.hist_len > 0) {
      T* hnew = p.hist[j - 1] + b * lv.hist_len;
      for (int q = tid; q < lv.hist_len; q += NT) hnew[q] = X[q + N - lv.hist_len];
    }
    if (j < p.J) {
      if (!dbl) lds_barrier();
      regs_to_level<T, L, NV>(Y, areg, nvec, N, p.lv[j], p.npow2, hist_of(j + 1));
      T* t = X; X = Y; Y = t;
    }
  }
}

__device__ __forceinline__ void lds_dma16(unsigned lds, const void* g, bool nt) {
  unsigned keep;
  if (nt) {
    asm volatile(
        "s_mov_b32 %0, m0\n\t"
        "s_mov_b32 m0, %2\n\t"
        "s_nop 0\n\t"
        "global_load_lds_dwordx4 %1, off nt\n\t"
        "s_mov_b32 m0, %0"
        : "=&s"(keep)
        : "v"(g), "s"(__builtin_amdgcn_readfirstlane(lds))
        : "memory");
  } else {
    asm volatile(
        "s_mov_b32 %0, m0\n\t"
        "s_mov_b32 m0, %2\n\t"
        "s_nop 0\n\t"
        "global_load_lds_dwordx4 %1, off\n\t"
        "s_mov_b32 m0, %0"
        : "=&s"(keep)
        : "v"(g), "s"(__builtin_amdgcn_readfirstlane(lds))
        : "memory");
  }
}

template <typename T>
__device__ __forceinline__ void dma_row(T* buf, const T* __restrict__ src, int nvec, bool nt) {
  constexpr int V = VT<T>::V;
  const int lane = threadIdx.x & 63, wv = __builtin_amdgcn_readfirstlane(threadIdx.x >> 6), nw = blockDim.x >> 6;
  for (int c = wv; c * 64 < nvec; c += nw)
    lds_dma16((unsigned)(uintptr_t)(buf + c * 64 * V), src + (size_t)(c * 64 + lane) * V, nt);
}

template <int N>
__device__ __forceinline__ void wait_vmcnt() {
  static_assert(N >= 0 && N < 64, "vmcnt range");
  __builtin_amdgcn_s_waitcnt((N & 0xF) | ((N >> 4) << 14) | (0x7 << 4) | (0xF << 8));
}

__device__ __forceinline__ void wait_vmcnt_rt(int n) {
  switch (__builtin_amdgcn_readfirstlane(n)) {
    case 0: wait_vmcnt<0>(); break;
    case 1: wait_vmcnt<1>(); break;
    case 2: wait_vmcnt<2>(); break;
    case 3: wait_vmcnt<3>(); break;
    case 4: wait_vmcnt<4>(); break;
    case 5: wait_vmcnt<5>(); break;
    case 6: wait_vmcnt<6>(); break;
    case 7: wait_vmcnt<7>(); break;
    case 8: wait_vmcnt<8>(); break;
    case 9: wait_vmcnt<9>(); break;
    case 10: wait_vmcnt<10>(); break;
    case 11: wait_vmcnt<11>(); break;
    case 12: wait_vmcnt<12>(); break;
    case 13: wait_vmcnt<13>(); break;
    case 14: wait_vmcnt<14>(); break;
    case 15: wait_vmcnt<15>(); break;
    case 16: wait_vmcnt<16>(); break;
    case 17: wait_vmcnt<17>(); break;
    case 18: wait_vmcnt<18>(); break;
    case 19: wait_vmcnt<19>(); break;
    case 20: wait_vmcnt<20>(); break;
    case 21: wait_vmcnt<21>(); break;
    case 22: wait_vmcnt<22>(); break;
    case 23: wait_vmcnt<23>(); break;
    case 24: wait_vmcnt<24>(); break;
    case 25: wait_vmcnt<25>(); break;
    case 26: wait_vmcnt<26>(); break;
    case 27: wait_vmcnt<27>(); break;
    case 28: wait_vmcnt<28>(); break;
    case 29: wait_vmcnt<29>(); break;
    case 30: wait_vmcnt<30>(); break;
    case 31: wait_vmcnt<31>(); break;
    case 32: wait_vmcnt<32>(); break;
    case 33: wait_vmcnt<33>(); break;
    case 34: wait_vmcnt<34>(); break;
    case 35: wait_vmcnt<35>(); break;
    case 36: wait_vmcnt<36>(); break;
    case 37: wait_vmcnt<37>(); break;
    case 38: wait_vmcnt<38>(); break;
    case 39: wait_vmcnt<39>(); break;
    case 40: wait_vmcnt<40>(); break;
    case 41: wait_vmcnt<41>(); break;
    case 42: wait_vmcnt<42>(); break;
    case 43: wait_vmcnt<43>(); break;
    case 44: wait_vmcnt<44>(); break;
    case 45: wait_vmcnt<45>(); break;
    case 46: wait_vmcnt<46>(); break;
    case 47: wait_vmcnt<47>(); break;
    case 48: wait_vmcnt<48>(); break;
    case 49: wait_vmcnt<49>(); break;
    case 50: wait_vmcnt<50>(); break;
    case 51: wait_vmcnt<51>(); break;
    case 52: wait_vmcnt<52>(); break;
    case 53: wait_vmcnt<53>(); break;
    case 54: wait_vmcnt<54>(); break;
    case 55: wait_vmcnt<55>(); break;
    case 56: wait_vmcnt<56>(); break;
    case 57: wait_vmcnt<57>(); break;
    case 58: wait_vmcnt<58>(); break;
    case 59: wait_vmcnt<59>(); break;
    case 60: wait_vmcnt<60>(); break;
    case 61: wait_vmcnt<61>(); break;
    case 62: wait_vmcnt<62>(); break;
    case 63: wait_vmcnt<63>(); break;
    default: wait_vmcnt<63>(); break;
  }
}

template <typename T, int L, bool FMA, int NV>
__global__ void __attribute__((amdgpu_flat_work_group_size(1, NV <= 4 ? 512 : 1024), amdgpu_waves_per_eu(4)))
k_forward_persist(const FwdArgs<T> p) {
  constexpr int V = VT<T>::V;
  extern __shared__ __attribute__((aligned(16))) unsigned char smem[];
  T* const B0 = reinterpret_cast<T*>(smem) + p.hlpad;
  T* const B1 = reinterpret_cast<T*>(smem) + p.region1 + p.hlpad;
  const int N = p.N;
  const int nvec = N / V;
  const long long G = gridDim.x;
  long long b = blockIdx.x;
  if (b >= p.B) return;
  int cur = 0;
  T nf = T(0);
  dma_row<T>(B0, p.x + b * p.ldx, nvec, p.dma_nt != 0);
  wait_vmem();
  for (;;) {
    T* X = cur ? B1 : B0;
    T* Y = cur ? B0 : B1;
    lds_barrier();
    const LevelDesc lv0 = p.lv[0];
    fill_halo(X, N, lv0.hl, lv0.hr, lv0.mode, p.npow2, (const T*)nullptr, 0);
    const long long bn = b + G;
    T areg[NV][V];
    for (int j = 1; j <= p.J; ++j) {
      const LevelDesc lv = p.lv[j - 1];
      lds_barrier();
      if (j == p.J && bn < p.B) {
        dma_row<T>(Y, p.x + bn * p.ldx, nvec, p.dma_nt != 0);
      }
      T* dout = p.details + ((size_t)(j - 1) * (size_t)p.B + (size_t)b) * (size_t)N;
      T* aout = (j == p.J) ? p.approx + b * (size_t)N : nullptr;
      if (p.nf_flag) fwd_level<T, L, FMA, NV, false, true>(p, X, nvec, lv, dout, aout, true, 0ull, areg, &nf);
      else fwd_level<T, L, FMA, NV, false>(p, X, nvec, lv, dout, aout, true, 0ull, areg);
      if (j < p.J) {
        regs_to_level<T, L, NV>(Y, areg, nvec, N, p.lv[j], p.npow2, (const T*)nullptr);
        T* t = X; X = Y; Y = t;
      }
    }
    if (p.nf_flag) {
      nf_flag_row<T>(p.nf_flag, b, nf);
      nf = T(0);
    }
    if (bn >= p.B) break;
    wait_vmcnt<2 * NV>();
    cur = (cur + p.J) & 1;
    b = bn;
  }
}

template <typename T, int L, bool FMA, int NV>
__global__ void VW_FUSED_BOUNDS(NV, VW_FUSED_W(L, 6)) k_inverse_fused(const InvArgs<T> p) {
  constexpr int V = VT<T>::V;
  extern __shared__ __attribute__((aligned(16))) unsigned char smem[];
  T* A = reinterpret_cast<T*>(smem) + p.hlpad_a;
  T* D = reinterpret_cast<T*>(smem) + p.region_d + p.hlpad_d;
  const long long b = p.rev ? p.B - 1 - (long long)blockIdx.x : (long long)blockIdx.x;
  const int N = p.N;
  const int nvec = (N + V - 1) / V;
  const bool vec_ok = (L > 0) || p.vec_io != 0;
  auto thr_of = [&](int j) { return p.thr ? load_uniform(p.thr + (size_t)(j - 1) * (size_t)p.thr_ld + (size_t)b) : T(0); };
  const size_t plane = (size_t)p.B * (size_t)N;

  T reg[NV][V];
  T dnext[NV][V];
  load_row_regs<T, NV>(reg, p.approx + b * (size_t)N, N, nvec, vec_ok, p.approx_zero != 0);
  load_row_regs<T, NV>(dnext, p.details + (size_t)(p.J - 1) * plane + b * (size_t)N, N, nvec, vec_ok,
                       p.lv[p.J - 1].use_d == 0);
  wait_vmem();
  regs_to_level<T, L, NV>(A, reg, nvec, N, p.lv[p.J - 1], 0, (const T*)nullptr, p.approx_zero != 0);
  regs_to_level<T, L, NV>(D, dnext, nvec, N, p.lv[p.J - 1], 0, (const T*)nullptr, p.lv[p.J - 1].use_d == 0, p.thr,
                          thr_of(p.J), p.soft);

  for (int j = p.J; j >= 1; --j) {
    const LevelDesc lv = p.lv[j - 1];
    lds_barrier();
    if (j > 1) {
      load_row_regs<T, NV>(dnext, p.details + (size_t)(j - 2) * plane + b * (size_t)N, N, nvec, vec_ok,
                           p.lv[j - 2].use_d == 0);
    }
    for_vecs<L, NV>(nvec, [&](int k, int w) {
      T acc[V];
#pragma unroll
      for (int e = 0; e < V; ++e) acc[e] = T(0);
      inv_pair<T, L, FMA>(A, D, w * V, lv.s, lv.dir_a, p.lo, p.hi, p.taps, acc);
#pragma unroll
      for (int e = 0; e < V; ++e) {
        asm volatile("" : "+v"(acc[e]));
        reg[k][e] = acc[e];
      }
    });
    if (j == 1) {
      for_vecs<L, NV>(nvec, [&](int k, int w) { store_vec<VW_INV_STORE_AUX>(p.y + b * (size_t)N, w * V, N, vec_ok, reg[k]); });
    } else {
      const LevelDesc ln = p.lv[j - 2];
      lds_barrier();
      regs_to_level<T, L, NV>(A, reg, nvec, N, ln, 0, (const T*)nullptr);
      wait_vmem();
      regs_to_level<T, L, NV>(D, dnext, nvec, N, ln, 0, (const T*)nullptr, ln.use_d == 0, p.thr, thr_of(j - 1), p.soft);
    }
  }
}

template <typename T, int L, bool FMA, int NV>
__global__ void VW_FUSED_BOUNDS(NV, VW_FUSED_W(L, 6)) k_inverse_db(const InvArgs<T> p) {
  constexpr int V = VT<T>::V;
  extern __shared__ __attribute__((aligned(16))) unsigned char smem[];
  T* const X = reinterpret_cast<T*>(smem) + p.hlpad_a;
  T* const Y = reinterpret_cast<T*>(smem) + p.region_d + p.hlpad_d;
  const long long b = p.rev ? p.B - 1 - (long long)blockIdx.x : (long long)blockIdx.x;
  const int N = p.N;
  const int nvec = (N + V - 1) / V;
  const bool vec_ok = (L > 0) || p.vec_io != 0;
  auto thr_of = [&](int j) { return p.thr ? load_uniform(p.thr + (size_t)(j - 1) * (size_t)p.thr_ld + (size_t)b) : T(0); };
  const size_t plane = (size_t)p.B * (size_t)N;

  T acc[NV][V];
  T dreg[NV][V];
  load_row_regs<T, NV>(acc, p.approx + b * (size_t)N, N, nvec, vec_ok, p.approx_zero != 0);
  load_row_regs<T, NV>(dreg, p.details + (size_t)(p.J - 1) * plane + b * (size_t)N, N, nvec, vec_ok,
                       p.lv[p.J - 1].use_d == 0);
  wait_vmem();
  regs_to_level<T, L, NV>(X, acc, nvec, N, p.lv[p.J - 1], 0, (const T*)nullptr, p.approx_zero != 0);

  for (int j = p.J; j >= 1; --j) {
    const LevelDesc lv = p.lv[j - 1];
    lds_barrier();
    wait_vmem();
    regs_to_level<T, L, NV>(Y, dreg, nvec, N, lv, 0, (const T*)nullptr, lv.use_d == 0, p.thr, thr_of(j), p.soft);
    if (j > 1)
      load_row_regs<T, NV>(dreg, p.details + (size_t)(j - 2) * plane + b * (size_t)N, N, nvec, vec_ok,
                           p.lv[j - 2].use_d == 0);
    zero_regs<T, NV>(acc);
    inv_row<T, L, FMA, NV>(X, nvec, lv.s, lv.dir_a, lv.off_a, p.lo, p.taps, acc);
    lds_barrier();
    inv_row<T, L, FMA, NV>(Y, nvec, lv.s, lv.dir_d, lv.off_d, p.hi, p.taps, acc);
    if (j > 1) regs_to_level<T, L, NV>(X, acc, nvec, N, p.lv[j - 2], 0, (const T*)nullptr);
  }
  for_vecs<L, NV>(nvec, [&](int k, int w) { store_vec<VW_INV_STORE_AUX>(p.y + b * (size_t)N, w * V, N, vec_ok, acc[k]); });
}

#ifndef VW_INV_LATE_PF
#define VW_INV_LATE_PF 0
#endif
#ifndef VW_INV_W
#define VW_INV_W 6
#endif
template <typename T, int L, bool FMA, int NV>
__global__ void VW_FUSED_BOUNDS(NV, VW_FUSED_W(L, VW_INV_W)) k_inverse_seq(const InvArgs<T> p) {
  constexpr int V = VT<T>::V;
  extern __shared__ __attribute__((aligned(16))) unsigned char smem[];
  T* R = reinterpret_cast<T*>(smem) + p.hlpad_a;
  const long long b = p.rev ? p.B - 1 - (long long)blockIdx.x : (long long)blockIdx.x;
  const int N = p.N;
  const int nvec = (N + V - 1) / V;
  const bool vec_ok = (L > 0) || p.vec_io != 0;
  auto thr_of = [&](int j) { return p.thr ? load_uniform(p.thr + (size_t)(j - 1) * (size_t)p.thr_ld + (size_t)b) : T(0); };
  const size_t plane = (size_t)p.B * (size_t)N;

  T acc[NV][V];
  T dreg[NV][V];
  T nf = T(0);
  const bool nfp = p.nf_flag != nullptr;
  load_row_regs<T, NV>(acc, p.approx + b * (size_t)N, N, nvec, vec_ok, p.approx_zero != 0);
  load_row_regs<T, NV>(dreg, p.details + (size_t)(p.J - 1) * plane + b * (size_t)N, N, nvec, vec_ok,
                       p.lv[p.J - 1].use_d == 0);
  wait_vmem();
  regs_to_level<T, L, NV>(R, acc, nvec, N, p.lv[p.J - 1], 0, (const T*)nullptr, p.approx_zero != 0);

  for (int j = p.J; j >= 1; --j) {
    const LevelDesc lv = p.lv[j - 1];
    lds_barrier();
#if VW_INV_LATE_PF
    if (j < p.J)
      load_row_regs<T, NV>(dreg, p.details + (size_t)(j - 1) * plane + b * (size_t)N, N, nvec, vec_ok,
                           lv.use_d == 0);
#endif
    zero_regs<T, NV>(acc);
    inv_row<T, L, FMA, NV>(R, nvec, lv.s, lv.dir_a, lv.off_a, p.lo, p.taps, acc);
    lds_barrier();
    wait_vmem();
    regs_to_level<T, L, NV>(R, dreg, nvec, N, lv, 0, (const T*)nullptr, lv.use_d == 0, p.thr, thr_of(j), p.soft);
#if !VW_INV_LATE_PF
    if (j > 1)
      load_row_regs<T, NV>(dreg, p.details + (size_t)(j - 2) * plane + b * (size_t)N, N, nvec, vec_ok,
                           p.lv[j - 2].use_d == 0);
#endif
    lds_barrier();
    inv_row<T, L, FMA, NV>(R, nvec, lv.s, lv.dir_d, lv.off_d, p.hi, p.taps, acc);
    if (j > 1) {
      lds_barrier();
      regs_to_level<T, L, NV>(R, acc, nvec, N, p.lv[j - 2], 0, (const T*)nullptr);
    }
  }
  for_vecs<L, NV>(nvec, [&](int k, int w) { store_vec<VW_INV_STORE_AUX>(p.y + b * (size_t)N, w * V, N, vec_ok, acc[k]); });
  if (nfp) {
    nf_probe_rows<T, L, NV, V>(nf, acc, nvec);
    nf_flag_row<T>(p.nf_flag, b, nf);
  }
}

struct BlkLayout {
  int sh, pad;
};

__device__ __forceinline__ BlkLayout blk_layout(int m, int nv, int tight = 0) {
  if (m <= 0 || m >= 16) return BlkLayout{30, 0};
  if (nv >= 8) return tight ? BlkLayout{4, 1} : BlkLayout{3, 1};
  if (m == 8) return BlkLayout{3, 2};
  return BlkLayout{2, 1};
}

__device__ __forceinline__ int blk_phys(const BlkLayout& lo, int u) { return u + (u >> lo.sh) * lo.pad; }

template <typename T>
__device__ __forceinline__ void blk_store(T* R, const BlkLayout& lo, int u, const typename VT<T>::v& o) {
  *reinterpret_cast<typename VT<T>::v*>(R + blk_phys(lo, u) * VT<T>::V) = o;
}

template <int NV>
__device__ __forceinline__ int blk_base(int m) {
  const int tid = threadIdx.x;
  return (tid / m) * (m * NV) + tid % m;
}

template <typename T, int NV>
constexpr int blk_chunk() { return (NV >= 8 && sizeof(T) == 8) ? 4 : kWinTaps; }

template <typename T, int L, bool FMA, int NV>
__device__ __forceinline__ void blk_inv_branch(const T* R, const BlkLayout& lo, int vb, int m, const T* f,
                                               T (&acc)[NV][VT<T>::V]) {
  constexpr int V = VT<T>::V;
  using vec = typename VT<T>::v;
  constexpr int TC = blk_chunk<T, NV>();
  static_for<0, (L + TC - 1) / TC>([&](auto c) __attribute__((always_inline)) {
    constexpr int I0 = decltype(c)::value * TC;
    constexpr int I1 = (I0 + TC < L) ? I0 + TC : L;
    T fc[I1 - I0];
#pragma unroll
    for (int i = I0; i < I1; ++i) fc[i - I0] = f[i];
#pragma unroll
    for (int q = I0; q < I1 + NV - 1; ++q) {
      const vec x = *reinterpret_cast<const vec*>(R + blk_phys(lo, vb + q * m) * V);
#pragma unroll
      for (int r = 0; r < NV; ++r) {
        const int i = q - r;
        if (i >= I0 && i < I1) {
          vmadd<FMA>(acc[r], x, fc[i - I0]);
        }
      }
      if (((q - I0) & 3) == 3) __builtin_amdgcn_sched_barrier(0);
    }
  });
#pragma unroll
  for (int r = 0; r < NV; ++r)
#pragma unroll
    for (int e = 0; e < V; ++e) asm volatile("" : "+v"(acc[r][e]));
}

template <int M, int NV, int TIGHT>
struct BlkC {
  static constexpr int SH = (M >= 16) ? 30 : (NV >= 8 ? (TIGHT ? 4 : 3) : (M == 8 ? 3 : 2));
  static constexpr int PAD = (M >= 16) ? 0 : (NV >= 8 ? 1 : (M == 8 ? 2 : 1));
  static constexpr bool ok = PAD == 0 || (M * NV) % (1 << SH) == 0;
  static constexpr int off(int q) { return q * M + ((q * M) >> SH) * PAD; }
};

template <typename T, int L, bool FMA, int NV, int M, int TIGHT>
__device__ __forceinline__ void blk_inv_branch_c(const T* Rb, const T* f, T (&acc)[NV][VT<T>::V]) {
  constexpr int V = VT<T>::V;
  using vec = typename VT<T>::v;
  using C = BlkC<M, NV, TIGHT>;
  constexpr int TC = blk_chunk<T, NV>();
  static_for<0, (L + TC - 1) / TC>([&](auto c) __attribute__((always_inline)) {
    constexpr int I0 = decltype(c)::value * TC;
    constexpr int I1 = (I0 + TC < L) ? I0 + TC : L;
    T fc[I1 - I0];
#pragma unroll
    for (int i = I0; i < I1; ++i) fc[i - I0] = f[i];
#pragma unroll
    for (int q = I0; q < I1 + NV - 1; ++q) {
      const vec x = *reinterpret_cast<const vec*>(Rb + C::off(q) * V);
#pragma unroll
      for (int r = 0; r < NV; ++r) {
        const int i = q - r;
        if (i >= I0 && i < I1) {
          vmadd<FMA>(acc[r], x, fc[i - I0]);
        }
      }
      if (((q - I0) & 3) == 3) __builtin_amdgcn_sched_barrier(0);
    }
  });
#pragma unroll
  for (int r = 0; r < NV; ++r)
#pragma unroll
    for (int e = 0; e < V; ++e) asm volatile("" : "+v"(acc[r][e]));
}

template <typename T, int L, bool FMA, int NV>
__device__ __forceinline__ void blk_inv_branch_s(const T* Rb, int m, int sh, int pad, const T* f,
                                                 T (&acc)[NV][VT<T>::V]) {
  constexpr int V = VT<T>::V;
  using vec = typename VT<T>::v;
  constexpr int TC = blk_chunk<T, NV>();
  static_for<0, (L + TC - 1) / TC>([&](auto c) __attribute__((always_inline)) {
    constexpr int I0 = decltype(c)::value * TC;
    constexpr int I1 = (I0 + TC < L) ? I0 + TC : L;
    T fc[I1 - I0];
#pragma unroll
    for (int i = I0; i < I1; ++i) fc[i - I0] = f[i];
#pragma unroll
    for (int q = I0; q < I1 + NV - 1; ++q) {
      const int qm = __builtin_amdgcn_readfirstlane(q * m);
      const int off = __builtin_amdgcn_readfirstlane(qm + (qm >> sh) * pad);
      const vec x = *reinterpret_cast<const vec*>(Rb + off * V);
#pragma unroll
      for (int r = 0; r < NV; ++r) {
        const int i = q - r;
        if (i >= I0 && i < I1) {
          vmadd<FMA>(acc[r], x, fc[i - I0]);
        }
      }
      if (((q - I0) & 3) == 3) __builtin_amdgcn_sched_barrier(0);
    }
  });
#pragma unroll
  for (int r = 0; r < NV; ++r)
#pragma unroll
    for (int e = 0; e < V; ++e) asm volatile("" : "+v"(acc[r][e]));
}

#ifndef VW_BLK_SOFF
#define VW_BLK_SOFF 1
#endif
#ifndef VW_BLK_CK8
#define VW_BLK_CK8 1
#endif

template <typename T, int L, bool FMA, int NV, int M, int TIGHT>
__device__ __forceinline__ void blk_inv_branch_cl(const T* Rb, const T* f, T (&acc)[NV][VT<T>::V]) {
  constexpr int V = VT<T>::V;
  using vec = typename VT<T>::v;
  using C = BlkC<M, NV, TIGHT>;
  constexpr int TC = blk_chunk<T, NV>();
  const unsigned ab = lds_base(Rb);
  static_for<0, (L + TC - 1) / TC>([&](auto c) __attribute__((always_inline)) {
    constexpr int I0 = decltype(c)::value * TC;
    constexpr int I1 = (I0 + TC < L) ? I0 + TC : L;
    T fc[I1 - I0];
#pragma unroll
    for (int i = I0; i < I1; ++i) fc[i - I0] = f[i];
#pragma unroll
    for (int q = I0; q < I1 + NV - 1; ++q) {
      const vec x = lds_vec_at<vec>(ab + (unsigned)(C::off(q) * V * (int)sizeof(T)));
#pragma unroll
      for (int r = 0; r < NV; ++r) {
        const int i = q - r;
        if (i >= I0 && i < I1) {
          vmadd<FMA>(acc[r], x, fc[i - I0]);
        }
      }
      if (((q - I0) & 3) == 3) __builtin_amdgcn_sched_barrier(0);
    }
  });
#pragma unroll
  for (int r = 0; r < NV; ++r)
#pragma unroll
    for (int e = 0; e < V; ++e) asm volatile("" : "+v"(acc[r][e]));
}

template <typename T, int L, bool FMA, int NV>
__device__ __forceinline__ void blk_inv_any(const T* R, const BlkLayout& lo, int tight, int vb, int m, const T* f,
                                            T (&acc)[NV][VT<T>::V]) {
  constexpr int V = VT<T>::V;
  if constexpr (NV >= 8) {
    const int sh = __builtin_amdgcn_readfirstlane(lo.sh), pad = __builtin_amdgcn_readfirstlane(lo.pad);
    if constexpr (VW_BLK_CK8 != 0 && FMA) {
      const T* Rb = R + blk_phys(lo, vb) * V;
      const int sel = (m == 1 || m == 2 || m == 4 || m == 8) && pad == 1 ? m * 2 + (tight ? 1 : 0)
                      : (m == 16 || m == 32 || m == 64) && pad == 0 ? 4 * m : 0;
      switch (sel) {
        case 2: blk_inv_branch_cl<T, L, FMA, NV, 1, 0>(Rb, f, acc); return;
        case 4: blk_inv_branch_cl<T, L, FMA, NV, 2, 0>(Rb, f, acc); return;
        case 5: blk_inv_branch_cl<T, L, FMA, NV, 2, 1>(Rb, f, acc); return;
        case 8: blk_inv_branch_cl<T, L, FMA, NV, 4, 0>(Rb, f, acc); return;
        case 9: blk_inv_branch_cl<T, L, FMA, NV, 4, 1>(Rb, f, acc); return;
        case 16: blk_inv_branch_cl<T, L, FMA, NV, 8, 0>(Rb, f, acc); return;
        case 17: blk_inv_branch_cl<T, L, FMA, NV, 8, 1>(Rb, f, acc); return;
        case 64: blk_inv_branch_cl<T, L, FMA, NV, 16, 0>(Rb, f, acc); return;
        case 128: blk_inv_branch_cl<T, L, FMA, NV, 32, 0>(Rb, f, acc); return;
        case 256: blk_inv_branch_cl<T, L, FMA, NV, 64, 0>(Rb, f, acc); return;
        default: break;
      }
    }
    if (VW_BLK_SOFF && (pad == 0 || ((m * NV) & ((1 << sh) - 1)) == 0))
      blk_inv_branch_s<T, L, FMA, NV>(R + blk_phys(lo, vb) * V, m, sh, pad, f, acc);
    else
      blk_inv_branch<T, L, FMA, NV>(R, lo, vb, m, f, acc);
  } else {
    const T* Rb = R + blk_phys(lo, vb) * V;
    auto go = [&](auto mc, auto tc) __attribute__((always_inline)) {
      constexpr int M = decltype(mc)::value, TT = decltype(tc)::value;
      if constexpr (BlkC<M, NV, TT>::ok) blk_inv_branch_c<T, L, FMA, NV, M, TT>(Rb, f, acc);
      else blk_inv_branch<T, L, FMA, NV>(R, lo, vb, m, f, acc);
    };
    auto go_m = [&](auto mc) __attribute__((always_inline)) { go(mc, std::integral_constant<int, 0>{}); };
    (void)tight;
    switch (m) {
      case 1: go_m(std::integral_constant<int, 1>{}); break;
      case 2: go_m(std::integral_constant<int, 2>{}); break;
      case 4: go_m(std::integral_constant<int, 4>{}); break;
      case 8: go_m(std::integral_constant<int, 8>{}); break;
      case 16: go_m(std::integral_constant<int, 16>{}); break;
      case 32: go_m(std::integral_constant<int, 32>{}); break;
      case 64: go_m(std::integral_constant<int, 64>{}); break;
      default: blk_inv_branch<T, L, FMA, NV>(R, lo, vb, m, f, acc); break;
    }
  }
}

template <typename T, int L, bool FMA, int NV>
__device__ __forceinline__ void blk_fwd(const T* X, const BlkLayout& lo, int HLV, int vb, int m, const T* flo,
                                        const T* fhi, T (&al)[NV][VT<T>::V], T (&ah)[NV][VT<T>::V]) {
  constexpr int V = VT<T>::V;
  using vec = typename VT<T>::v;
  constexpr int TC = blk_chunk<T, NV>();
#pragma unroll
  for (int r = 0; r < NV; ++r)
#pragma unroll
    for (int e = 0; e < V; ++e) { al[r][e] = T(0); ah[r][e] = T(0); }
  static_for<0, (L + TC - 1) / TC>([&](auto c) __attribute__((always_inline)) {
    constexpr int I0 = decltype(c)::value * TC;
    constexpr int I1 = (I0 + TC < L) ? I0 + TC : L;
    T fl[I1 - I0], fh[I1 - I0];
#pragma unroll
    for (int i = I0; i < I1; ++i) { fl[i - I0] = flo[i]; fh[i - I0] = fhi[i]; }
#pragma unroll
    for (int q = NV - 1 - I0; q > -I1; --q) {
      const vec x = *reinterpret_cast<const vec*>(X + blk_phys(lo, vb + q * m + HLV) * V);
#pragma unroll
      for (int r = 0; r < NV; ++r) {
        const int i = r - q;
        if (i >= I0 && i < I1) {
          vmadd<FMA, kPkFwd>(al[r], x, fl[i - I0]);
          vmadd<FMA, kPkFwd>(ah[r], x, fh[i - I0]);
        }
      }
      if (((NV - 1 - I0 - q) & 3) == 3) __builtin_amdgcn_sched_barrier(0);
    }
  });
#pragma unroll
  for (int r = 0; r < NV; ++r)
#pragma unroll
    for (int e = 0; e < V; ++e) {
      asm volatile("" : "+v"(al[r][e]));
      asm volatile("" : "+v"(ah[r][e]));
    }
}

template <typename T, int L, bool FMA, int NV>
__device__ __forceinline__ void blk_fwd_s(const T* Xb, int m, int sh, int pad, const T* flo, const T* fhi,
                                          T (&al)[NV][VT<T>::V], T (&ah)[NV][VT<T>::V]) {
  constexpr int V = VT<T>::V;
  using vec = typename VT<T>::v;
  constexpr int TC = blk_chunk<T, NV>();
#pragma unroll
  for (int r = 0; r < NV; ++r)
#pragma unroll
    for (int e = 0; e < V; ++e) { al[r][e] = T(0); ah[r][e] = T(0); }
  static_for<0, (L + TC - 1) / TC>([&](auto c) __attribute__((always_inline)) {
    constexpr int I0 = decltype(c)::value * TC;
    constexpr int I1 = (I0 + TC < L) ? I0 + TC : L;
    T fl[I1 - I0], fh[I1 - I0];
#pragma unroll
    for (int i = I0; i < I1; ++i) { fl[i - I0] = flo[i]; fh[i - I0] = fhi[i]; }
#pragma unroll
    for (int q = NV - 1 - I0; q > -I1; --q) {
      const int qm = __builtin_amdgcn_readfirstlane(q * m);
      const int off = __builtin_amdgcn_readfirstlane(qm + (qm >> sh) * pad);
      const vec x = *reinterpret_cast<const vec*>(Xb + off * V);
#pragma unroll
      for (int r = 0; r < NV; ++r) {
        const int i = r - q;
        if (i >= I0 && i < I1) {
          vmadd<FMA, kPkFwd>(al[r], x, fl[i - I0]);
          vmadd<FMA, kPkFwd>(ah[r], x, fh[i - I0]);
        }
      }
      if (((NV - 1 - I0 - q) & 3) == 3) __builtin_amdgcn_sched_barrier(0);
    }
  });
#pragma unroll
  for (int r = 0; r < NV; ++r)
#pragma unroll
    for (int e = 0; e < V; ++e) {
      asm volatile("" : "+v"(al[r][e]));
      asm volatile("" : "+v"(ah[r][e]));
    }
}

#ifndef VW_INV_KTAPS
#define VW_INV_KTAPS -1
#endif

#ifndef VW_FWD_KTAPS
#define VW_FWD_KTAPS -1
#endif

#ifndef VW_BLK_FWD_C
#define VW_BLK_FWD_C 1
#endif

template <typename T, int L, bool FMA, int NV, int M>
__device__ __forceinline__ void blk_fwd_c(const T* Xb, const T* flo, const T* fhi, T (&al)[NV][VT<T>::V],
                                          T (&ah)[NV][VT<T>::V]) {
  constexpr int V = VT<T>::V;
  using vec = typename VT<T>::v;
  using C = BlkC<M, NV, 0>;
  constexpr int TC = blk_chunk<T, NV>();
  constexpr int QMIN = -(L - 1);
  const unsigned aq = lds_base(Xb + C::off(QMIN) * V);
#pragma unroll
  for (int r = 0; r < NV; ++r)
#pragma unroll
    for (int e = 0; e < V; ++e) { al[r][e] = T(0); ah[r][e] = T(0); }
  static_for<0, (L + TC - 1) / TC>([&](auto c) __attribute__((always_inline)) {
    constexpr int I0 = decltype(c)::value * TC;
    constexpr int I1 = (I0 + TC < L) ? I0 + TC : L;
    T fl[I1 - I0], fh[I1 - I0];
#pragma unroll
    for (int i = I0; i < I1; ++i) { fl[i - I0] = flo[i]; fh[i - I0] = fhi[i]; }
#pragma unroll
    for (int q = NV - 1 - I0; q > -I1; --q) {
      const vec x = lds_vec_at<vec>(aq + (unsigned)((C::off(q) - C::off(QMIN)) * V * (int)sizeof(T)));
#pragma unroll
      for (int r = 0; r < NV; ++r) {
        const int i = r - q;
        if (i >= I0 && i < I1) {
          vmadd<FMA, kPkFwd>(al[r], x, fl[i - I0]);
          vmadd<FMA, kPkFwd>(ah[r], x, fh[i - I0]);
        }
      }
      if (((NV - 1 - I0 - q) & 3) == 3) __builtin_amdgcn_sched_barrier(0);
    }
  });
#pragma unroll
  for (int r = 0; r < NV; ++r)
#pragma unroll
    for (int e = 0; e < V; ++e) {
      asm volatile("" : "+v"(al[r][e]));
      asm volatile("" : "+v"(ah[r][e]));
    }
}

template <typename T, int L, bool FMA, int NV>
__device__ __forceinline__ void blk_fwd_any(const T* X, const BlkLayout& lo, int HLV, int vb, int m, const T* flo,
                                            const T* fhi, T (&al)[NV][VT<T>::V], T (&ah)[NV][VT<T>::V]) {
  constexpr int V = VT<T>::V;
  const T* Xb = X + blk_phys(lo, vb + HLV) * V;
  auto go = [&](auto mc) __attribute__((always_inline)) {
    constexpr int M = decltype(mc)::value;
    if constexpr (BlkC<M, NV, 0>::ok) blk_fwd_c<T, L, FMA, NV, M>(Xb, flo, fhi, al, ah);
    else blk_fwd<T, L, FMA, NV>(X, lo, HLV, vb, m, flo, fhi, al, ah);
  };
  switch (m) {
    case 1: go(std::integral_constant<int, 1>{}); break;
    case 2: go(std::integral_constant<int, 2>{}); break;
    case 4: go(std::integral_constant<int, 4>{}); break;
    case 8: go(std::integral_constant<int, 8>{}); break;
    case 16: go(std::integral_constant<int, 16>{}); break;
    case 32: go(std::integral_constant<int, 32>{}); break;
    case 64: go(std::integral_constant<int, 64>{}); break;
    default: blk_fwd<T, L, FMA, NV>(X, lo, HLV, vb, m, flo, fhi, al, ah); break;
  }
}

template <typename T, int L, bool FMA, int NV>
__global__ void VW_FUSED_BOUNDS(NV, VW_FUSED_W(L, 8)) k_forward_blk(const FwdArgs<T> p) {
  constexpr int V = VT<T>::V;
  using vec = typename VT<T>::v;
  extern __shared__ __attribute__((aligned(16))) unsigned char smem[];
  T* X = reinterpret_cast<T*>(smem);
  T* Y = p.region1 ? X + p.region1 : X;
  const bool dbl = p.region1 != 0;
  const long long b = blockIdx.x;
  T* const taps = reinterpret_cast<T*>(smem) + p.tap_lds;
  for (int i = threadIdx.x; i < 2 * L; i += blockDim.x) taps[i] = i < L ? p.lo[i] : p.hi[i - L];
  constexpr bool ktaps = VW_FWD_KTAPS < 0 ? NV >= 8 : VW_FWD_KTAPS != 0;
  const T* const flo = ktaps ? p.lo : taps;
  const T* const fhi = ktaps ? p.hi : taps + L;
  const int N = p.N;
  const int nvec = N / V;
  const int NT = blockDim.x;
  const int tid = threadIdx.x;
  const int HLV = p.hlpad / V;
  auto m_of = [&](int j) { return p.lv[j - 1].s / V; };
  auto hlv_of = [&](int j) { return ((L - 1) * p.lv[j - 1].s + V - 1) / V; };
  auto put = [&](T* buf, int j, int w, const vec& o) {
    const BlkLayout lo = blk_layout(m_of(j), NV, p.blk_tight);
    blk_store<T>(buf, lo, w + HLV, o);
    if (w >= nvec - hlv_of(j)) blk_store<T>(buf, lo, w - nvec + HLV, o);
  };
  {
    T r0[NV][V];
    load_row_regs<T, NV>(r0, p.x + b * p.ldx, N, nvec, true, false);
    wait_vmem();
#pragma unroll
    for (int k = 0; k < NV; ++k) {
      int w = tid + k * NT;
      asm volatile("" : "+v"(w));
      vec o;
#pragma unroll
      for (int e = 0; e < V; ++e) o[e] = r0[k][e];
      put(X, 1, w, o);
      __builtin_amdgcn_sched_barrier(0);
    }
  }
  T nf = T(0);
  for (int j = 1; j <= p.J; ++j) {
    const int m = m_of(j);
    lds_barrier();
    T* dout = p.details + ((size_t)(j - 1) * (size_t)p.B + (size_t)b) * (size_t)N;
    T* aout = p.approx + b * (size_t)N;
    const bool last = j == p.J;
    T al[NV][V], ah[NV][V];
    int vb = 0;
    if (m) {
      vb = blk_base<NV>(m);
      const BlkLayout lo = blk_layout(m, NV, p.blk_tight);
      const int sh = __builtin_amdgcn_readfirstlane(lo.sh), pad = __builtin_amdgcn_readfirstlane(lo.pad);
      bool fc = false;
      if constexpr (NV < 8) {
        if (VW_BLK_FWD_C && (HLV & 15) == 0) {
          blk_fwd_any<T, L, FMA, NV>(X, lo, HLV, vb, m, flo, fhi, al, ah);
          fc = true;
        }
      }
      if (fc) {
      } else if (VW_BLK_SOFF && NV >= 8 && (pad == 0 || (((m * NV) & ((1 << sh) - 1)) == 0 && (HLV & ((1 << sh) - 1)) == 0)))
        blk_fwd_s<T, L, FMA, NV>(X + blk_phys(lo, vb + HLV) * V, m, sh, pad, flo, fhi, al, ah);
      else
        blk_fwd<T, L, FMA, NV>(X, lo, HLV, vb, m, flo, fhi, al, ah);
      if (m < VW_BLK_NT_M) {
#pragma unroll
        for (int r = 0; r < NV; ++r) {
          store_vec<0>(dout, (vb + r * m) * V, N, true, ah[r]);
          if (last) store_vec<0>(aout, (vb + r * m) * V, N, true, al[r]);
        }
      } else {
#pragma unroll
        for (int r = 0; r < NV; ++r) {
          store_vec<VW_FWD_STORE_AUX>(dout, (vb + r * m) * V, N, true, ah[r]);
          if (last) store_vec<VW_FWD_STORE_AUX>(aout, (vb + r * m) * V, N, true, al[r]);
        }
      }
    } else {
      auto em = [&](int k, int w, const T (&l)[V], const T (&h)[V]) {
        store_vec<VW_FWD_STORE_AUX>(dout, w * V, N, true, h);
        if (last) store_vec<VW_FWD_STORE_AUX>(aout, w * V, N, true, l);
#pragma unroll
        for (int e = 0; e < V; ++e) { al[k][e] = l[e]; ah[k][e] = h[e]; }
      };
      if constexpr (V == 4) {
        if (p.lv[j - 1].s == 2) fwd_row_t<T, L, FMA, NV, 2>(X + HLV * V, nvec, 2, flo, fhi, p.taps, em);
        else fwd_row_t<T, L, FMA, NV, 1>(X + HLV * V, nvec, 1, flo, fhi, p.taps, em);
      } else {
        fwd_row_t<T, L, FMA, NV, 1>(X + HLV * V, nvec, 1, flo, fhi, p.taps, em);
      }
    }
    if (p.nf_flag && last) {
#pragma unroll
      for (int r = 0; r < NV; ++r) nf_probe<T, V>(nf, al[r]);
    }
    if (!last) {
      if (!dbl) lds_barrier();
#pragma unroll
      for (int r = 0; r < NV; ++r) {
        int w = m ? vb + r * m : tid + r * NT;
        asm volatile("" : "+v"(w));
        vec o;
#pragma unroll
        for (int e = 0; e < V; ++e) o[e] = al[r][e];
        put(Y, j + 1, w, o);
        __builtin_amdgcn_sched_barrier(0);
      }
      T* t = X; X = Y; Y = t;
    }
  }
  if (p.nf_flag) nf_flag_row<T>(p.nf_flag, b, nf);
}

template <typename T, int L, bool FMA, int NV>
__global__ void VW_FUSED_BOUNDS(NV, VW_FUSED_W(L, 6)) k_inverse_blk(const InvArgs<T> p) {
  constexpr int V = VT<T>::V;
  using vec = typename VT<T>::v;
  extern __shared__ __attribute__((aligned(16))) unsigned char smem[];
  T* R = reinterpret_cast<T*>(smem);
  const long long b = p.rev ? p.B - 1 - (long long)blockIdx.x : (long long)blockIdx.x;
  const int N = p.N;
  const int nvec = N / V;
  const int NT = blockDim.x;
  const int tid = threadIdx.x;
  T* const taps = reinterpret_cast<T*>(smem) + p.tap_lds;
  for (int i = tid; i < 2 * L; i += NT) taps[i] = i < L ? p.lo[i] : p.hi[i - L];
  constexpr bool ktaps = VW_INV_KTAPS < 0 ? NV >= 8 : VW_INV_KTAPS != 0;
  const T* const flo = ktaps ? p.lo : taps;
  const T* const fhi = ktaps ? p.hi : taps + L;
  auto thr_of = [&](int j) { return p.thr ? load_uniform(p.thr + (size_t)(j - 1) * (size_t)p.thr_ld + (size_t)b) : T(0); };
  const size_t plane = (size_t)p.B * (size_t)N;
  auto m_of = [&](int j) { return p.lv[j - 1].s / V; };
  auto hrv_of = [&](int j) { return ((L - 1) * p.lv[j - 1].s + V - 1) / V; };
  auto put = [&](int j, int w, const vec& o) {
    const BlkLayout lo = blk_layout(m_of(j), NV, p.blk_tight);
    blk_store<T>(R, lo, w, o);
    if (w < hrv_of(j)) blk_store<T>(R, lo, w + nvec, o);
  };
  auto stage_std = [&](const T (&r)[NV][V], int j, int mode, T thr_b) {
#pragma unroll
    for (int k = 0; k < NV; ++k) {
      int w = tid + k * NT;
      asm volatile("" : "+v"(w));
      vec o;
#pragma unroll
      for (int e = 0; e < V; ++e) {
        if (mode == 1) o[e] = T(0);
        else if (mode == 2) o[e] = threshold_t(r[k][e], thr_b, p.soft);
        else o[e] = r[k][e];
      }
      put(j, w, o);
      __builtin_amdgcn_sched_barrier(0);
    }
  };

  T acc[NV][V];
  T dreg[NV][V];
  load_row_regs<T, NV>(acc, p.approx + b * (size_t)N, N, nvec, true, p.approx_zero != 0);
  load_row_regs<T, NV>(dreg, p.details + (size_t)(p.J - 1) * plane + b * (size_t)N, N, nvec, true,
                       p.lv[p.J - 1].use_d == 0);
  wait_vmem();
  stage_std(acc, p.J, p.approx_zero ? 1 : 0, T(0));

  for (int j = p.J; j >= 1; --j) {
    const LevelDesc lv = p.lv[j - 1];
    const int m = m_of(j);
    const BlkLayout lo = blk_layout(m, NV, p.blk_tight);
    const int vb = m ? blk_base<NV>(m) : 0;
    lds_barrier();
    zero_regs<T, NV>(acc);
    if (m) blk_inv_any<T, L, FMA, NV>(R, lo, p.blk_tight, vb, m, flo, acc);
    else inv_row<T, L, FMA, NV>(R, nvec, lv.s, 1, 0, flo, p.taps, acc);
    lds_barrier();
    wait_vmem();
    stage_std(dreg, j, lv.use_d == 0 ? 1 : (p.thr ? 2 : 0), thr_of(j));
    if (j > 1)
      load_row_regs<T, NV>(dreg, p.details + (size_t)(j - 2) * plane + b * (size_t)N, N, nvec, true,
                           p.lv[j - 2].use_d == 0);
    lds_barrier();
    if (m) blk_inv_any<T, L, FMA, NV>(R, lo, p.blk_tight, vb, m, fhi, acc);
    else inv_row<T, L, FMA, NV>(R, nvec, lv.s, 1, 0, fhi, p.taps, acc);
    if (j > 1) {
      lds_barrier();
#pragma unroll
      for (int r = 0; r < NV; ++r) {
        int w = m ? vb + r * m : tid + r * NT;
        asm volatile("" : "+v"(w));
        vec o;
#pragma unroll
        for (int e = 0; e < V; ++e) o[e] = acc[r][e];
        put(j - 1, w, o);
        __builtin_amdgcn_sched_barrier(0);
      }
    }
  }
#pragma unroll
  for (int k = 0; k < NV; ++k) store_vec<VW_INV_STORE_AUX>(p.y + b * (size_t)N, (tid + k * NT) * V, N, true, acc[k]);
  if (p.nf_flag) {
    T nf = T(0);
#pragma unroll
    for (int k = 0; k < NV; ++k) nf_probe<T, V>(nf, acc[k]);
    nf_flag_row<T>(p.nf_flag, b, nf);
  }
}

template <typename T>
__device__ __forceinline__ T halo_value_global(const T* __restrict__ src, int idx, int N, int mode, int npow2,
                                               const T* hist_b, int hist_len) {
  if (idx >= 0 && idx < N) return src[idx];
  switch (mode) {
    case kHaloPeriodic: { int r = idx % N; if (r < 0) r += N; return src[r]; }
    case kHaloSymmetric: return src[sym_index(idx, N)];
    case kHaloFftPad: { int r = idx < 0 ? idx + npow2 : idx; return (r >= 0 && r < N) ? src[r] : T(0); }
    case kHaloHistory: return (idx < 0 && idx >= -hist_len) ? hist_b[hist_len + idx] : T(0);
    default: return T(0);
  }
}

template <typename T>
__device__ __forceinline__ void tile_to_lds(T* buf, const T* __restrict__ src, int N, int ts, int lo_q, int hi_q,
                                            int mode, int npow2, const T* hist_b, int hist_len, const T* thr,
                                            T thr_b, int soft, bool zero, bool vec_ok = false) {
  constexpr int V = VT<T>::V;
  using vec = typename VT<T>::v;
  int qa = lo_q, qb = lo_q;
  if (vec_ok && !zero) {
    qa = max(lo_q, -ts);
    qa = (qa + V - 1) / V * V;
    qb = min(hi_q, N - ts);
    qb = qb >= qa ? qa + (qb - qa) / V * V : qa;
  }
  for (int q = qa + (int)threadIdx.x * V; q < qb; q += blockDim.x * V) {
    vec v = __builtin_nontemporal_load(reinterpret_cast<const vec*>(src + ts + q));
    if (thr) {
#pragma unroll
      for (int e = 0; e < V; ++e) v[e] = threshold_t(v[e], thr_b, soft);
    }
    *reinterpret_cast<vec*>(buf + q) = v;
  }
  const int tail = (hi_q - lo_q) - (qb - qa);
  for (int r = (int)threadIdx.x; r < tail; r += blockDim.x) {
    const int q = (lo_q + r < qa) ? lo_q + r : qb + (r - (qa - lo_q));
    T v = zero ? T(0) : halo_value_global(src, ts + q, N, mode, npow2, hist_b, hist_len);
    if (thr) v = threshold_t(v, thr_b, soft);
    buf[q] = v;
  }
}

template <typename T, int L, bool FMA>
__global__ void __launch_bounds__(256) k_forward_level(const LevelArgs<T> p) {
  constexpr int V = VT<T>::V;
  extern __shared__ __attribute__((aligned(16))) unsigned char smem[];
  T* buf = reinterpret_cast<T*>(smem) + p.hlpad;
  const long long b = blockIdx.y;
  const int N = p.N;
  const int ts = blockIdx.x * p.tile;
  const int cnt = min(p.tile, N - ts);
  const int nv = (cnt + V - 1) / V;
  const LevelDesc lv = p.lv;
  const T* src = p.src_a + b * p.lda;
  const T* hist_b = (lv.mode == kHaloHistory) ? p.hist + b * lv.hist_len : nullptr;
  tile_to_lds(buf, src, N, ts, -lv.hl, nv * V, lv.mode, p.npow2, hist_b, lv.hist_len, (const T*)nullptr, T(0), 0,
              false, p.vec_io != 0 && (p.lda % V) == 0);
  if (p.validate) {
    for (int q = threadIdx.x; q < cnt; q += blockDim.x)
      if (!finite_t(buf[q])) atomicMin(p.bad, (unsigned long long)b * N + ts + q);
  }
  __syncthreads();
  const bool vec_ok = p.vec_io != 0;
  for (int w = threadIdx.x; w < nv; w += blockDim.x) {
    const int t0 = w * V;
    T al[V], ah[V];
#pragma unroll
    for (int e = 0; e < V; ++e) { al[e] = T(0); ah[e] = T(0); }
    fwd_vec<T, L, FMA>(buf, t0, lv.s, p.lo, p.hi, p.taps, al, ah);
    store_vec(p.out_a + b * (size_t)N + ts, t0, cnt, vec_ok, al);
    store_vec(p.out_d + b * (size_t)N + ts, t0, cnt, vec_ok, ah);
    check_out<T>(p.validate, p.bad, (unsigned long long)b * N + ts, t0, cnt, al);
    check_out<T>(p.validate, p.bad, (unsigned long long)b * N + ts, t0, cnt, ah);
  }
}

template <typename T, int L, bool FMA>
__global__ void __launch_bounds__(256) k_inverse_level(const LevelArgs<T> p) {
  constexpr int V = VT<T>::V;
  extern __shared__ __attribute__((aligned(16))) unsigned char smem[];
  T* A = reinterpret_cast<T*>(smem) + p.hlpad;
  T* D = reinterpret_cast<T*>(smem) + p.region_d + p.hlpad_d;
  const long long b = blockIdx.y;
  const int N = p.N;
  const int ts = blockIdx.x * p.tile;
  const int cnt = min(p.tile, N - ts);
  const int nv = (cnt + V - 1) / V;
  const LevelDesc lv = p.lv;
  const T thr_b = p.thr ? p.thr[b] : T(0);
  const int span = nv * V;
  tile_to_lds(A, p.src_a + b * (size_t)N, N, ts, -lv.hl, span + lv.hr, lv.mode, 0, (const T*)nullptr, 0,
              (const T*)nullptr, T(0), 0, p.src_a == nullptr, p.vec_io != 0);
  tile_to_lds(D, p.src_d + b * (size_t)N, N, ts, -lv.hl, span + lv.hr, lv.mode, 0, (const T*)nullptr, 0, p.thr,
              thr_b, p.soft, p.use_d == 0 || p.src_d == nullptr, p.vec_io != 0);
  __syncthreads();
  const bool vec_ok = p.vec_io != 0;
  for (int w = threadIdx.x; w < nv; w += blockDim.x) {
    const int t0 = w * V;
    T acc[V];
#pragma unroll
    for (int e = 0; e < V; ++e) acc[e] = T(0);
    if (p.pair) {
      inv_pair<T, L, FMA>(A, D, t0, lv.s, lv.dir_a, p.lo, p.hi, p.taps, acc);
    } else {
      inv_branch<T, L, FMA>(A, t0, lv.s, lv.dir_a, lv.off_a, p.lo, p.taps, acc);
      inv_branch<T, L, FMA>(D, t0, lv.s, lv.dir_d, lv.off_d, p.hi, p.taps, acc);
    }
    store_vec(p.out_a + b * (size_t)N + ts, t0, cnt, vec_ok, acc);
  }
}


struct SweepPos {
  long long b;
  int r, q0, q1;
  bool ok;
};

__device__ __forceinline__ SweepPos sweep_pos(long long B, int N, int s, int qc) {
  const int qn = (N + s - 1) / s;
  const int chunks = (qn + qc - 1) / qc;
  const long long g = (long long)blockIdx.x * blockDim.x + threadIdx.x;
  const long long per = (long long)chunks * s;
  SweepPos p;
  p.b = g / per;
  const long long rem = g - p.b * per;
  const int c = (int)(rem / s);
  p.r = (int)(rem - (long long)c * s);
  const int qr = p.r < N ? (N - 1 - p.r) / s + 1 : 0;
  p.q0 = c * qc;
  p.q1 = min(p.q0 + qc, qr);
  p.ok = p.b < B && p.q0 < p.q1;
  return p;
}

template <typename T>
__device__ __forceinline__ T sweep_fetch(const T* __restrict__ src, long long u, int N, int mode, int npow2,
                                         const T* hist_b, int hist_len) {
  if (u >= 0 && u < N) return src[u];
  return halo_value_global(src, (int)u, N, mode, npow2, hist_b, hist_len);
}

template <typename T, int L, int K, int DIR>
struct SweepWin {
  T w[K + L - 1];
  __device__ __forceinline__ long long first(long long tb, int s, int off) const {
    return tb + off + (DIR < 0 ? -(long long)(L - 1) * s : 0);
  }
  template <typename Fetch>
  __device__ __forceinline__ void fill_head(long long tb, int s, int off, Fetch&& fetch) {
    const long long u0 = first(tb, s, off);
#pragma unroll
    for (int j = 0; j < L - 1; ++j) w[j] = fetch(u0 + (long long)j * s);
  }
  template <typename Fetch>
  __device__ __forceinline__ void load_block(long long tb, int s, int off, Fetch&& fetch) {
    const long long u0 = first(tb, s, off);
#pragma unroll
    for (int j = L - 1; j < K + L - 1; ++j) w[j] = fetch(u0 + (long long)j * s);
  }
  __device__ __forceinline__ void shift() {
#pragma unroll
    for (int j = 0; j < L - 1; ++j) w[j] = w[j + K];
  }
  __device__ __forceinline__ T tap(int k, int i) const { return DIR < 0 ? w[k - i + L - 1] : w[k + i]; }
};

template <int L> struct SweepK { static constexpr int K = L <= 16 ? 16 : 8; };

template <typename T, int L, bool FMA>
__global__ void __launch_bounds__(256) k_forward_sweep(const LevelArgs<T> p) {
  constexpr int K = SweepK<L>::K;
  const LevelDesc lv = p.lv;
  const int s = lv.s, N = p.N;
  const SweepPos sp = sweep_pos(p.B, N, s, p.tile);
  if (!sp.ok) return;
  const T* src = p.src_a + sp.b * p.lda;
  const T* hist_b = (lv.mode == kHaloHistory) ? p.hist + sp.b * lv.hist_len : nullptr;
  T* oa = p.out_a + sp.b * (size_t)N;
  T* od = p.out_d + sp.b * (size_t)N;
  const unsigned long long flat0 = (unsigned long long)sp.b * N;
  const long long tend = (long long)sp.r + (long long)sp.q1 * s;
  auto fetch = [&](long long u) -> T {
    if (u >= tend) return T(0);
    return sweep_fetch(src, u, N, lv.mode, p.npow2, hist_b, lv.hist_len);
  };
  SweepWin<T, L, K, -1> X;
  long long tb = (long long)sp.r + (long long)sp.q0 * s;
  X.fill_head(tb, s, 0, fetch);
  for (int q = sp.q0; q < sp.q1; q += K, tb += (long long)K * s) {
    X.load_block(tb, s, 0, fetch);
#pragma unroll
    for (int k = 0; k < K; ++k) {
      if (q + k < sp.q1) {
        T al = T(0), ah = T(0);
#pragma unroll
        for (int i = 0; i < L; ++i) {
          al = madd<FMA>(al, X.tap(k, i), p.lo[i]);
          ah = madd<FMA>(ah, X.tap(k, i), p.hi[i]);
        }
        const long long t = tb + (long long)k * s;
        oa[t] = al;
        od[t] = ah;
        if (p.validate) {
          if (!finite_t(X.tap(k, 0))) atomicMin(p.bad, flat0 + t);
          if (!finite_t(al) || !finite_t(ah)) atomicMin(p.bad, (1ull << 62) | (flat0 + t));
        }
      }
    }
    X.shift();
  }
}

template <typename T, int L, bool FMA, int DA, int DD>
__global__ void __launch_bounds__(256) k_inverse_sweep(const LevelArgs<T> p) {
  constexpr int K = SweepK<L>::K;
  const LevelDesc lv = p.lv;
  const int s = lv.s, N = p.N;
  const SweepPos sp = sweep_pos(p.B, N, s, p.tile);
  if (!sp.ok) return;
  const T thr_b = p.thr ? p.thr[sp.b] : T(0);
  const T* sa = p.src_a ? p.src_a + sp.b * (size_t)N : nullptr;
  const T* sd = p.src_d ? p.src_d + sp.b * (size_t)N : nullptr;
  const bool za = sa == nullptr, zd = sd == nullptr || p.use_d == 0;
  T* y = p.out_a + sp.b * (size_t)N;
  auto fa = [&](long long u) -> T { return za ? T(0) : sweep_fetch(sa, u, N, lv.mode, 0, (const T*)nullptr, 0); };
  auto fd = [&](long long u) -> T {
    if (zd) return T(0);
    const T v = sweep_fetch(sd, u, N, lv.mode, 0, (const T*)nullptr, 0);
    return p.thr ? threshold_t(v, thr_b, p.soft) : v;
  };
  SweepWin<T, L, K, DA> A;
  SweepWin<T, L, K, DD> D;
  long long tb = (long long)sp.r + (long long)sp.q0 * s;
  A.fill_head(tb, s, lv.off_a, fa);
  D.fill_head(tb, s, lv.off_d, fd);
  for (int q = sp.q0; q < sp.q1; q += K, tb += (long long)K * s) {
    A.load_block(tb, s, lv.off_a, fa);
    D.load_block(tb, s, lv.off_d, fd);
#pragma unroll
    for (int k = 0; k < K; ++k) {
      if (q + k < sp.q1) {
        T acc = T(0);
        if (p.pair) {
#pragma unroll
          for (int i = 0; i < L; ++i) acc = acc + pair_term<T, FMA>(p.lo[i], A.tap(k, i), p.hi[i], D.tap(k, i));
        } else {
#pragma unroll
          for (int i = 0; i < L; ++i) acc = madd<FMA>(acc, A.tap(k, i), p.lo[i]);
#pragma unroll
          for (int i = 0; i < L; ++i) acc = madd<FMA>(acc, D.tap(k, i), p.hi[i]);
        }
        y[tb + (long long)k * s] = acc;
      }
    }
    A.shift();
    D.shift();
  }
}


template <typename T, int L, bool FMA, int KA, int R, int RING>
__device__ __forceinline__ void sweep_ring_stage(const T* ring, int lane, int sl0, int st, const T* sd, bool thr_on,
                                                 T thr_b, int soft, long long tb, long long ts, int N, const T* lo,
                                                 const T* hi, T (&acc)[KA]) {
  T wd[KA + L - 1];
#pragma unroll
  for (int x = 0; x < KA + L - 1; ++x) {
    if (sd) {
      long long t = tb + (long long)x * ts;
      t = t >= N ? t - N : t;
      const T v = sd[t];
      wd[x] = thr_on ? threshold_t(v, thr_b, soft) : v;
    } else {
      wd[x] = T(0);
    }
  }
  T w[KA + L - 1];
// ... 530 lines not shown
```

vectorwave_amd/csrc/vw_fwd.hip:

```cpp
#include "vw_launch.h"
#include <algorithm>

namespace vw {

template <typename T, int L, bool FMA, int NV>
static hipError_t run_forward_fused_nv(const FwdArgs<T>& a, int threads, int lds, hipStream_t st) {
  const bool hist = a.hist[0] != nullptr;
  auto k = hist ? k_forward_fused<T, L, FMA, NV, true> : k_forward_fused<T, L, FMA, NV, false>;
  static LdsOnce configured, configured_h;
  hipError_t e = set_lds(k, lds, hist ? &configured_h : &configured);
  if (e != hipSuccess) return e;
  hipLaunchKernelGGL(k, dim3((unsigned)a.B), dim3(threads), lds, st, a);
  return hipGetLastError();
}

template <typename T, int L, bool FMA>
static hipError_t run_forward_fused(const FwdArgs<T>& a, int threads, int lds, int nv, hipStream_t st) {
  if constexpr (L > 0 && L <= 8) {
    if (nv == 2) return run_forward_fused_nv<T, L, FMA, 2>(a, threads, lds, st);
  }
  return nv <= 4 ? run_forward_fused_nv<T, L, FMA, 4>(a, threads, lds, st) : run_forward_fused_nv<T, L, FMA, 8>(a, threads, lds, st);
}

template <typename T>
hipError_t launch_forward_fused(const FwdArgs<T>& a, int threads, int lds, bool fma, int nv, hipStream_t st) {
  switch (a.unrolled ? a.taps : 0) {
#define VW_CASE(n) \
    case n: return fma ? run_forward_fused<T, n, true>(a, threads, lds, nv, st) : run_forward_fused<T, n, false>(a, threads, lds, nv, st);
    VW_TAP_LIST(VW_CASE)
#undef VW_CASE
    default:
      return fma ? run_forward_fused<T, 0, true>(a, threads, lds, nv, st) : run_forward_fused<T, 0, false>(a, threads, lds, nv, st);
  }
}
template hipError_t launch_forward_fused<VW_T>(const FwdArgs<VW_T>&, int, int, bool, int, hipStream_t);
template <typename T, int L, bool FMA, int NV>
static hipError_t run_forward_blk_nv(const FwdArgs<T>& a, int threads, int lds, hipStream_t st) {
  auto k = k_forward_blk<T, L, FMA, NV>;
  static LdsOnce configured;
  hipError_t e = set_lds(k, lds, &configured);
  if (e != hipSuccess) return e;
  hipLaunchKernelGGL(k, dim3((unsigned)a.B), dim3(threads), lds, st, a);
  return hipGetLastError();
}

template <typename T>
hipError_t launch_forward_blk(const FwdArgs<T>& a, int threads, int lds, bool fma, int nv, hipStream_t st) {
  switch (a.taps) {
#define VW_CASE(n)                                                                                       \
    case n:                                                                                              \
      if (nv <= 4) return fma ? run_forward_blk_nv<T, n, true, 4>(a, threads, lds, st)                  \
                              : run_forward_blk_nv<T, n, false, 4>(a, threads, lds, st);                 \
      return fma ? run_forward_blk_nv<T, n, true, 8>(a, threads, lds, st) : run_forward_blk_nv<T, n, false, 8>(a, threads, lds, st);
    VW_TAP_LIST(VW_CASE)
#undef VW_CASE
    default:
      return hipErrorNotSupported;
  }
}
template hipError_t launch_forward_blk<VW_T>(const FwdArgs<VW_T>&, int, int, bool, int, hipStream_t);

template <typename T, int L, bool FMA, int NV>
static hipError_t run_forward_persist(const FwdArgs<T>& a, int threads, int lds, hipStream_t st) {
  auto k = k_forward_persist<T, L, FMA, NV>;
  static LdsOnce configured;
  hipError_t e = set_lds(k, lds, &configured);
  if (e != hipSuccess) return e;
  static int cus = 0;
  if (!cus) {
    int dev = 0;
    if ((e = hipGetDevice(&dev)) != hipSuccess) return e;
    if ((e = hipDeviceGetAttribute(&cus, hipDeviceAttributeMultiprocessorCount, dev)) != hipSuccess) return e;
  }
  static int q_threads = -1, q_lds = -1, q_per_cu = 0;
  if (threads != q_threads || lds != q_lds) {
    int per_cu = 0;
    if ((e = hipOccupancyMaxActiveBlocksPerMultiprocessor(&per_cu, k, threads, lds)) != hipSuccess) return e;
    q_threads = threads; q_lds = lds; q_per_cu = per_cu;
  }
  const int per_cu = q_per_cu;
  if (per_cu < 1) return hipErrorInvalidConfiguration;
  const long long grid = std::min<long long>(a.B, (long long)per_cu * cus);
  hipLaunchKernelGGL(k, dim3((unsigned)grid), dim3(threads), lds, st, a);
  return hipGetLastError();
}

template <typename T, int L, bool FMA>
static hipError_t run_forward_persist_nv(const FwdArgs<T>& a, int threads, int lds, int nv, hipStream_t st) {
  (void)nv;
  return run_forward_persist<T, L, FMA, 4>(a, threads, lds, st);
}

template <typename T>
hipError_t launch_forward_persist(const FwdArgs<T>& a, int threads, int lds, bool fma, int nv, hipStream_t st) {
  switch (a.taps) {
#define VW_CASE(n) \
    case n: return fma ? run_forward_persist_nv<T, n, true>(a, threads, lds, nv, st) : run_forward_persist_nv<T, n, false>(a, threads, lds, nv, st);
    VW_TAP_LIST(VW_CASE)
#undef VW_CASE
    default:
      return hipErrorNotSupported;
  }
}
template hipError_t launch_forward_persist<VW_T>(const FwdArgs<VW_T>&, int, int, bool, int, hipStream_t);
}
```

vectorwave_amd/csrc/vw_internal.h:

```cpp
#pragma once
#include <hip/hip_runtime.h>
#include <atomic>
#include <cstdint>

namespace vw {

constexpr int kMaxTaps = 64;
constexpr int kMaxLevels = 24;
constexpr int kNV = 8;
constexpr int kMaxThreads = 1024;
constexpr int kLdsBytes = 160 * 1024;
constexpr int kSweepMinS = 16;
constexpr int kSweepChunk = 128;

enum HaloMode : int {
  kHaloPeriodic = 0,
  kHaloZero = 1,
  kHaloSymmetric = 2,
  kHaloFftPad = 3,
  kHaloHistory = 4
};

struct LevelDesc {
  int s;
  int hl, hr;
  int mode;
  int dir_a;
  int off_a;
  int dir_d;
  int off_d;
  int use_d;
  int hist_len;
  int own;
  int il_a, il_b;
  int ir_a, ir_b;
  int vs, ve;
};

template <typename T>
struct FwdArgs {
  const T* x;
  long long ldx;
  T* details;
  T* approx;
  long long B;
  int N;
  int J;
  int npow2;
  int hlpad;
  int region1;
  int vec_io;
  int unrolled;
  int dma_nt;
  int validate;
  int rev;
  unsigned long long* bad;
  T* hist[kMaxLevels];
  int hist_update;
  int taps;
  int tap_lds;
  int blk_tight;
  int* nf_flag;
  T lo[kMaxTaps];
  T hi[kMaxTaps];
  LevelDesc lv[kMaxLevels];
};

template <typename T>
struct InvArgs {
  const T* details;
  const T* approx;
  T* y;
  long long B;
  int N;
  int J;
  int hlpad_a, hlpad_d;
  int region_d;
  int vec_io;
  int pair;
  int unrolled;
  int db;
  int blk;
  int approx_zero;
  int rev;
  const T* thr;
  long long thr_ld;
  int soft;
  int taps;
  int tap_lds;
  int blk_tight;
  int* nf_flag;
  T lo[kMaxTaps];
  T hi[kMaxTaps];
  LevelDesc lv[kMaxLevels];
};

template <typename T>
struct LevelArgs {
  const T* src_a;
  long long lda;
  const T* src_d;
  const T* src_d2;
  const T* thr2;
  int use_d2;
  const T* src_d3;
  const T* thr3;
  int use_d3;
  T* out_a;
  T* out_d;
  const T* hist;
  long long B;
  int N;
  int tile;
  int hlpad;
  int region_d, hlpad_d;
  int pair;
  const T* thr;
  int soft;
  int use_d;
  int vec_io;
  int validate;
  unsigned long long* bad;
  int npow2;
  int taps;
  T lo[kMaxTaps];
  T hi[kMaxTaps];
  LevelDesc lv;
};

constexpr int kMaxGroup = 8;
constexpr int kMultiInvNI = 8;
constexpr int kMultiPF = 6;
template <typename T>
struct MultiArgs {
  const T* src_a;
  long long lda;
  const T* src_d[kMaxGroup];
  T* out_d[kMaxGroup];
  T* out_a;
  const T* thr[kMaxGroup];
  long long B;
  int N;
  int tile;
  int nlev;
  int s0;
  int ext[kMaxGroup + 1];
  int region;
  int vec_io;
  int soft;
  int taps;
  int rblk;
  int pf;
  int pad;
  int* nf_flag;
  int slack;
  int ni;
  T lo[kMaxTaps];
  T hi[kMaxTaps];
};

enum ThrMethod { kThrUniversal = 0, kThrSure = 1, kThrMinimax = 2, kThrBayes = 3, kThrFixed = 4 };
constexpr int kSigmaRegN = 16384;
constexpr int kSureMaxN = 16384;
struct DenoiseConsts {
  double level_scale[kMaxLevels];
  double univ_c;
  double log_n;
  int method;
  int n;
};

constexpr int kRefPlanes = 2 * kMaxLevels + 3;
template <typename T>
struct RefScan {
  const T* p[kRefPlanes];
  long long ld[kRefPlanes];
  int len[kRefPlanes];
  int np;
  long long B;
  int N;
  int chunks;
  int* flag;
};
template <typename T>
struct RefArgs {
  const T* x;
  long long ldx;
  const T* det_in;
  T* details;
  T* approx;
  T* y;
  const T* thr;
  long long thr_ld;
  int soft;
  long long B;
  int N;
  int J;
  int L;
  int mode;
  int hist_mode;
  int hist_first;
  const T* hist_old[kMaxLevels];
  T* hist_new[kMaxLevels];
  int hist_len[kMaxLevels];
  int* flag;
  T* scratch;
  T lo[kMaxTaps];
  T hi[kMaxTaps];
  LevelDesc lv[kMaxLevels];
};
template <typename T>
hipError_t launch_flag_nonfinite(const RefScan<T>& a, hipStream_t st);
template <typename T>
hipError_t launch_ref_cascade(const RefArgs<T>& a, int grid, bool inverse, hipStream_t st);
int ref_scan_chunks(int N);

bool mfma_supported(int L, long long N);
int mfma_halo(int L, int J);
int mfma_region(int n);
hipError_t launch_forward_mfma(const FwdArgs<float>& a, int lds, hipStream_t st);
hipError_t launch_inverse_mfma(const InvArgs<float>& a, int lds, hipStream_t st);

constexpr int kFinMaxN = 16384;
constexpr int kFinMaxTaps = 30;
constexpr int kFinPerThread = 16;
struct FinArgs {
  const double* x;
  long long ld;
  long long B;
  int N;
  int L;
  int tree;
  int validate;
  int wavelet;
  double k;
  double* out;
  unsigned long long* bad;
  double lo[kFinMaxTaps];
  double hi[kFinMaxTaps];
};
hipError_t launch_fin_analyze(const FinArgs& a, hipStream_t st);
hipError_t launch_fin_sharpe(const FinArgs& a, hipStream_t st);

constexpr int kMaxDevices = 64;
struct LdsOnce {
  std::atomic<int> limit[kMaxDevices];
};
template <typename Kern>
static hipError_t set_lds(Kern k, int lds_bytes, LdsOnce* once, int want = kLdsBytes) {
  if (lds_bytes <= 64 * 1024) return hipSuccess;
  int dev = 0;
  if (hipGetDevice(&dev) != hipSuccess || dev < 0) dev = 0;
  std::atomic<int>* f = dev < kMaxDevices ? &once->limit[dev] : nullptr;
  if (f && f->load(std::memory_order_acquire) >= lds_bytes) return hipSuccess;
  if (want < lds_bytes) want = lds_bytes;
  hipError_t e = hipFuncSetAttribute(reinterpret_cast<const void*>(k), hipFuncAttributeMaxDynamicSharedMemorySize, want);
  if (e != hipSuccess) return e;
  if (f) f->store(want, std::memory_order_release);
  return hipSuccess;
}

template <typename T>
hipError_t launch_forward_fused(const FwdArgs<T>& a, int threads, int lds_bytes, bool fma, int nv, hipStream_t st);
template <typename T>
hipError_t launch_forward_persist(const FwdArgs<T>& a, int threads, int lds_bytes, bool fma, int nv, hipStream_t st);
template <typename T>
hipError_t launch_forward_blk(const FwdArgs<T>& a, int threads, int lds_bytes, bool fma, int nv, hipStream_t st);
template <typename T>
hipError_t launch_inverse_fused(const InvArgs<T>& a, int threads, int lds_bytes, bool fma, int nv, hipStream_t st);
template <typename T>
hipError_t launch_forward_level(const LevelArgs<T>& a, int lds_bytes, bool fma, hipStream_t st);
template <typename T>
hipError_t launch_inverse_level(const LevelArgs<T>& a, int lds_bytes, bool fma, hipStream_t st);
template <typename T>
hipError_t launch_forward_sweep(const LevelArgs<T>& a, bool fma, hipStream_t st);
template <typename T>
hipError_t launch_inverse_sweep(const LevelArgs<T>& a, bool fma, hipStream_t st);
template <typename T>
hipError_t launch_inverse_sweepg(const LevelArgs<T>& a, int levels, int ka, int R, bool fma, hipStream_t st);
template <typename T>
hipError_t launch_forward_multi(const MultiArgs<T>& a, int lds_bytes, bool fma, hipStream_t st);

template <typename T>
hipError_t launch_inverse_multi(const MultiArgs<T>& a, int lds_bytes, bool fma, hipStream_t st);
template <typename T>
hipError_t launch_history_update(const T* level_in, long long ld_in, const T* old_hist, T* new_hist,
                                 long long B, int n, int hist_len, hipStream_t st);

hipError_t launch_level_threshold(const double* coeffs, long long level_stride, const double* sigma,
                                  const DenoiseConsts& k, long long B, int levels, double* thr, hipStream_t st);
hipError_t launch_noise_sigma(const double* coeffs, long long ld, long long B, int N, double scale_c,
                              double* sigma_out, double* thr_out, hipStream_t st);
hipError_t launch_median(const double* x, long long ld, long long B, int N, const double* center, double* median_out,
                         hipStream_t st);
hipError_t launch_abs_center(const double* x, long long ld, long long B, int N, const double* center, double* out,
                             hipStream_t st);
hipError_t launch_seq_std(const double* x, int n, double* out, hipStream_t st);
hipError_t launch_gather_abs(const double* src, const int* idx, int count, double* window, int wsize, int start,
                             hipStream_t st);
template <typename T>
hipError_t launch_transpose(const T* in, long long rows, long long cols, T* out, hipStream_t st);
template <typename T>
hipError_t launch_threshold(T* c, long long B, long long N, const T* thr, int soft, hipStream_t st);
template <typename T>
hipError_t launch_fill_uniform(T* x, long long count, unsigned long long seed, long long offset, hipStream_t st);
template <typename T>
hipError_t launch_single_haar_batch(const T* x, long long ldx, long long B, int N, T* approx, T* detail,
                                    hipStream_t st);

inline void blk_layout_host(int m, int nv, int* sh, int* pad, int tight = 0) {
  if (m <= 0 || m >= 16) { *sh = 30; *pad = 0; }
  else if (nv >= 8) { *sh = tight ? 4 : 3; *pad = 1; }
  else if (m == 8) { *sh = 3; *pad = 2; }
  else { *sh = 2; *pad = 1; }
}

bool has_unrolled_taps(int L);
int fused_max_threads();

}
```

vectorwave_amd/csrc/vw_inv.hip:

```cpp
#include "vw_launch.h"
#include <algorithm>

namespace vw {

template <typename T, int L, bool FMA, int NV>
static hipError_t run_inverse_fused_nv(const InvArgs<T>& a, int threads, int lds, hipStream_t st) {
  static LdsOnce configured_pair, configured_seq, configured_db, configured_blk;
  const bool blk = L > 0 && NV != 2 && a.blk && !a.pair && !a.db;
  auto k = a.pair ? k_inverse_fused<T, L, FMA, NV> : a.db ? k_inverse_db<T, L, FMA, NV> : k_inverse_seq<T, L, FMA, NV>;
  if constexpr (NV != 2) {
    if (blk) k = k_inverse_blk<T, (L > 0 ? L : 2), FMA, NV>;
  }
  hipError_t e = set_lds(k, lds, a.pair ? &configured_pair : a.db ? &configured_db
                                 : blk ? &configured_blk : &configured_seq);
  if (e != hipSuccess) return e;
  hipLaunchKernelGGL(k, dim3((unsigned)a.B), dim3(threads), lds, st, a);
  return hipGetLastError();
}

template <typename T, int L, bool FMA>
static hipError_t run_inverse_fused(const InvArgs<T>& a, int threads, int lds, int nv, hipStream_t st) {
  if constexpr (L > 0 && L <= 8) {
    if (nv == 2) return run_inverse_fused_nv<T, L, FMA, 2>(a, threads, lds, st);
  }
  return nv <= 4 ? run_inverse_fused_nv<T, L, FMA, 4>(a, threads, lds, st) : run_inverse_fused_nv<T, L, FMA, 8>(a, threads, lds, st);
}

template <typename T>
hipError_t launch_inverse_fused(const InvArgs<T>& a, int threads, int lds, bool fma, int nv, hipStream_t st) {
  switch (a.unrolled ? a.taps : 0) {
#define VW_CASE(n) \
    case n: return fma ? run_inverse_fused<T, n, true>(a, threads, lds, nv, st) : run_inverse_fused<T, n, false>(a, threads, lds, nv, st);
    VW_TAP_LIST(VW_CASE)
#undef VW_CASE
    default:
      return fma ? run_inverse_fused<T, 0, true>(a, threads, lds, nv, st) : run_inverse_fused<T, 0, false>(a, threads, lds, nv, st);
  }
}
template hipError_t launch_inverse_fused<VW_T>(const InvArgs<VW_T>&, int, int, bool, int, hipStream_t);
}
```

Before: 45880.

## Specialize MODWT level rows on compile-time dilation and full-slab bounds

Adds compile-time-spacing variants of the forward and inverse row filters for dilations 2..64, so LDS reads use constant immediate offsets from a single base address. Also adds a FULL template flag that drops per-vector bounds checks and index clamps when threads*NV exactly covers the row, used by the persistent forward kernel and the sequential inverse kernel. Both are on by default through a new VW_LEVEL_CT knob. The cost is many more kernel instantiations, and there is some risk around how the FULL path is selected in the forward persist kernel.

```diff
diff --git a/vectorwave_amd/csrc/vw_capi.cpp b/vectorwave_amd/csrc/vw_capi.cpp
--- a/vectorwave_amd/csrc/vw_capi.cpp
+++ b/vectorwave_amd/csrc/vw_capi.cpp
@@ -92,6 +92,7 @@
   int sweep2_minb = 64;
   int blk_fwd8 = 1;
   int ref_grid = 0;
+  int level_ct = 1;
   int mfma = 0;
 };
 
@@ -134,6 +135,7 @@
   else if (k == "VW_SWEEP2_R") t.sweep2_r = v == 32 ? 32 : 0;
   else if (k == "VW_SWEEP2_MINB") t.sweep2_minb = v < 0 ? d.sweep2_minb : v;
   else if (k == "VW_BLK_FWD8") t.blk_fwd8 = v < 0 ? d.blk_fwd8 : v;
+  else if (k == "VW_LEVEL_CT") t.level_ct = v < 0 ? d.level_ct : v != 0;
   else if (k == "VW_MFMA") t.mfma = v < 0 ? d.mfma : v;
   else if (k == "VW_REF_GRID") t.ref_grid = v < 0 ? d.ref_grid : v;
   else return false;
@@ -146,7 +148,7 @@
     "VW_UNROLL_MAX", "VW_BLK", "VW_FWD_NV",
     "VW_INV_NV", "VW_DEEP", "VW_DEEP_INV", "VW_DEEP_LDS", "VW_DEEP_WAVES", "VW_DEEP_PF_FWD", "VW_DEEP_PF_INV",
     "VW_SWEEP2", "VW_SWEEP2_KA", "VW_SWEEP2_UC", "VW_SWEEP2_R", "VW_SWEEP2_MINB", "VW_BLK_FWD8",
-    "VW_DMA_NT", "VW_MULTI_NI", "VW_MFMA", "VW_REF_GRID"};
+    "VW_DMA_NT", "VW_MULTI_NI", "VW_MFMA", "VW_REF_GRID", "VW_LEVEL_CT"};
 
 static Tuning read_tuning() {
   Tuning t;
@@ -1178,6 +1180,7 @@
     a.unrolled = a.vec_io && fit && L <= tu.unroll_max;
     a.validate = validate; a.bad = c->bad;
     a.rev = tu.fwd_rev;
+    a.level_ct = tu.level_ct;
     a.dma_nt = tu.dma_nt >= 0 ? tu.dma_nt : (B <= 2LL * c->cus ? 1 : 0);
     for (int j = 0; j < J; ++j) a.hist[j] = hist ? hist[j] : nullptr;
     a.hist_update = hist_update ? 1 : 0;
@@ -1460,6 +1463,8 @@
     a.unrolled = a.vec_io && fit && L <= tu.unroll_max;
     a.pair = pair; a.approx_zero = approx_zero; a.thr = thr; a.thr_ld = thr_ld; a.soft = soft; a.taps = L;
     a.rev = tu.inv_rev;
+    a.level_ct = tu.level_ct;
+    a.full = tu.level_ct && a.unrolled && (int64_t)threads * nv == nvec;
     if (tu.blk > 0 && L >= tu.blk && nv != 2 && !pair && !db && boundary == VW_PERIODIC && a.unrolled &&
         (int64_t)threads * nv == nvec) {
       bool okb = true;
diff --git a/vectorwave_amd/csrc/vw_device.h b/vectorwave_amd/csrc/vw_device.h
--- a/vectorwave_amd/csrc/vw_device.h
+++ b/vectorwave_amd/csrc/vw_device.h
@@ -298,14 +298,14 @@
   }
 }
 
-template <int L, int NV, typename F>
+template <int L, int NV, bool FULL = false, typename F>
 __device__ __forceinline__ void for_vecs(int nvec, F&& fn) {
   const int NT = blockDim.x;
 #pragma unroll
   for (int k = 0; k < NV; ++k) {
     int w = threadIdx.x + k * NT;
     asm volatile("" : "+v"(w));
-    if ((L > 0 && k < NV - 1) || w < nvec) fn(k, w);
+    if (FULL || (L > 0 && k < NV - 1) || w < nvec) fn(k, w);
     __builtin_amdgcn_sched_barrier(0);
   }
 }
@@ -349,11 +349,11 @@
   }
 }
 
-template <int AUX = VW_STORE_AUX, typename T>
+template <int AUX = VW_STORE_AUX, bool FULL = false, typename T>
 __device__ __forceinline__ void store_vec(T* __restrict__ dst, int t0, int N, bool vec_ok, const T (&v)[VT<T>::V]) {
   constexpr int V = VT<T>::V;
   using vec = typename VT<T>::v;
-  if (vec_ok && t0 + V <= N) {
+  if (FULL || (vec_ok && t0 + V <= N)) {
     vec o;
 #pragma unroll
     for (int e = 0; e < V; ++e) o[e] = v[e];
@@ -385,7 +385,7 @@
   return av <= thr ? T(0) : c;
 }
 
-template <typename T, int NV>
+template <typename T, int NV, bool FULL = false>
 __device__ __forceinline__ void load_row_regs(T (&r)[NV][VT<T>::V], const T* __restrict__ src, int N, int nvec,
                                               bool vec_ok, bool zero) {
   constexpr int V = VT<T>::V;
@@ -397,7 +397,7 @@
     for (int k = 0; k < NV; ++k) {
       int w = (int)threadIdx.x + k * NT;
       asm volatile("" : "+v"(w));
-      w = min(w, nvec - 1);
+      if constexpr (!FULL) w = min(w, nvec - 1);
       const vec v = stream_load<vec>(src, w);
 #pragma unroll
       for (int e = 0; e < V; ++e) r[k][e] = v[e];
@@ -415,13 +415,13 @@
   }
 }
 
-template <typename T>
+template <typename T, bool FULL = false>
 __device__ __forceinline__ void halo_images(T* buf, int w, const typename VT<T>::v& o, int N, const LevelDesc& lv) {
   constexpr int V = VT<T>::V;
 #pragma unroll
   for (int e = 0; e < V; ++e) {
     const int t = w * V + e;
-    if (t < N) {
+    if (FULL || t < N) {
       const int l = lv.il_a * t + lv.il_b;
       const int r = lv.ir_a * t + lv.ir_b;
       if (l < 0 && l >= -lv.hl) buf[l] = o[e];
@@ -443,13 +443,13 @@
   }
 }
 
-template <typename T, int L, int NV, int MODE>
+template <typename T, int L, int NV, int MODE, bool FULL = false>
 __device__ __forceinline__ void regs_to_level_m(T* buf, const T (&r)[NV][VT<T>::V], int nvec, int N,
                                                 const LevelDesc& lv, T thr_b, int soft) {
   constexpr int V = VT<T>::V;
   using vec = typename VT<T>::v;
   const bool own = lv.own != 0;
-  for_vecs<L, NV>(nvec, [&](int k, int w) {
+  for_vecs<L, NV, FULL>(nvec, [&](int k, int w) {
     vec o;
 #pragma unroll
     for (int e = 0; e < V; ++e) {
@@ -468,17 +468,17 @@
       for (int e = 0; e < V; ++e)
         if (w * V + e < N) buf[w * V + e] = o[e];
     }
-    if (own && ((k == 0 && w < lv.vs) || (k == NV - 1 && w >= lv.ve))) halo_images(buf, w, o, N, lv);
+    if (own && ((k == 0 && w < lv.vs) || (k == NV - 1 && w >= lv.ve))) halo_images<T, FULL>(buf, w, o, N, lv);
   });
 }
 
-template <typename T, int L, int NV>
+template <typename T, int L, int NV, bool FULL = false>
 __device__ __forceinline__ void regs_to_level(T* buf, const T (&r)[NV][VT<T>::V], int nvec, int N, const LevelDesc& lv,
                                               int npow2, const T* hist_b, bool zero = false, const T* thr = nullptr,
                                               T thr_b = T(0), int soft = 0) {
-  if (zero) regs_to_level_m<T, L, NV, 1>(buf, r, nvec, N, lv, thr_b, soft);
-  else if (thr) regs_to_level_m<T, L, NV, 2>(buf, r, nvec, N, lv, thr_b, soft);
-  else regs_to_level_m<T, L, NV, 0>(buf, r, nvec, N, lv, thr_b, soft);
+  if (zero) regs_to_level_m<T, L, NV, 1, FULL>(buf, r, nvec, N, lv, thr_b, soft);
+  else if (thr) regs_to_level_m<T, L, NV, 2, FULL>(buf, r, nvec, N, lv, thr_b, soft);
+  else regs_to_level_m<T, L, NV, 0, FULL>(buf, r, nvec, N, lv, thr_b, soft);
   if (lv.own) {
     halo_fixed(buf, N, lv, npow2, hist_b);
   } else {
@@ -487,12 +487,12 @@
   }
 }
 
-template <typename T, int L, bool FMA, int NV, int SC, typename Emit>
+template <typename T, int L, bool FMA, int NV, int SC, bool FULL = false, typename Emit>
 __device__ __forceinline__ void fwd_row_t(const T* buf, int nvec, int s, const T* lo, const T* hi, int taps,
                                           Emit&& emit) {
   constexpr int V = VT<T>::V;
   using vec = typename VT<T>::v;
-  for_vecs<L, NV>(nvec, [&](int k, int w) {
+  for_vecs<L, NV, FULL>(nvec, [&](int k, int w) {
     const int t0 = w * V;
     T al[V], ah[V];
 #pragma unroll
@@ -514,25 +514,62 @@
   });
 }
 
-template <typename T, int L, bool FMA, int NV, typename Emit>
-__device__ __forceinline__ void fwd_row(const T* buf, int nvec, int s, const T* lo, const T* hi, int taps,
+#define VW_CT_SPACINGS(X) X(2) X(4) X(8) X(16) X(32) X(64)
+template <typename T, int L, bool FMA, int NV, int S, bool FULL, typename Emit>
+__device__ __forceinline__ void fwd_row_ct(const T* buf, int nvec, const T* lo, const T* hi, Emit&& emit) {
+  constexpr int V = VT<T>::V;
+  using vec = typename VT<T>::v;
+  static_assert(S % V == 0 && (L - 1) * S * (int)sizeof(T) < 65536, "aligned reads, 16-bit offsets");
+  const T* const low = buf - (L - 1) * S;
+  for_vecs<L, NV, FULL>(nvec, [&](int k, int w) {
+    const int t0 = w * V;
+    T al[V], ah[V];
+#pragma unroll
+    for (int e = 0; e < V; ++e) { al[e] = T(0); ah[e] = T(0); }
+    const unsigned a0 = lds_base(low + t0);
+#pragma unroll
+    for (int i = 0; i < L; ++i) {
+      const vec v = lds_vec_at<vec>(a0 + (unsigned)((L - 1 - i) * S * (int)sizeof(T)));
+      vmadd<FMA, kPkFwd>(al, v, lo[i]);
+      vmadd<FMA, kPkFwd>(ah, v, hi[i]);
+      if ((i & 3) == 3) __builtin_amdgcn_sched_barrier(0);
+    }
+    emit(k, w, al, ah);
+  });
+}
+
+template <typename T, int L, bool FMA, int NV, bool FULL = false, typename Emit>
+__device__ __forceinline__ void fwd_row(const T* buf, int nvec, int s, const T* lo, const T* hi, int taps, int ct,
                                         Emit&& emit) {
   constexpr int V = VT<T>::V;
   if constexpr (L > 0) {
-    if (s == 1) return fwd_row_t<T, L, FMA, NV, 1>(buf, nvec, s, lo, hi, taps, emit);
+    if (s == 1) return fwd_row_t<T, L, FMA, NV, 1, FULL>(buf, nvec, s, lo, hi, taps, emit);
     if constexpr (V == 4) {
-      if (s == 2) return fwd_row_t<T, L, FMA, NV, 2>(buf, nvec, s, lo, hi, taps, emit);
-    }
-  }
-  fwd_row_t<T, L, FMA, NV, 0>(buf, nvec, s, lo, hi, taps, emit);
-}
-
-template <typename T, int L, bool FMA, int NV, int SC, int DIR>
+      if (s == 2) return fwd_row_t<T, L, FMA, NV, 2, FULL>(buf, nvec, s, lo, hi, taps, emit);
+    }
+  }
+  if constexpr (L > 0 && L <= 8) {
+    if (ct) {
+      switch (s) {
+#define VW_CASE(n) \
+        case n:    \
+          if constexpr (n % V == 0) return fwd_row_ct<T, L, FMA, NV, n, FULL>(buf, nvec, lo, hi, emit); \
+          break;
+        VW_CT_SPACINGS(VW_CASE)
+#undef VW_CASE
+        default: break;
+      }
+    }
+  }
+  fwd_row_t<T, L, FMA, NV, 0, FULL>(buf, nvec, s, lo, hi, taps, emit);
+}
+
+template <typename T, int L, bool FMA, int NV, int SC, int DIR, bool FULL = false>
 __device__ __forceinline__ void inv_row_t(const T* buf, int nvec, int s, int dir, int off, const T* f, int taps,
                                           T (&acc)[NV][VT<T>::V]) {
   constexpr int V = VT<T>::V;
   using vec = typename VT<T>::v;
-  for_vecs<L, NV>(nvec, [&](int k, int w) {
+  for_vecs<L, NV, FULL>(nvec, [&](int k, int w) {
     const int t0 = w * V;
     if constexpr (L > 0 && SC > 0) {
       inv_window<T, L, FMA, SC, DIR>(buf, t0 + off, f, acc[k]);
@@ -551,27 +588,63 @@
   });
 }
 
-template <typename T, int L, bool FMA, int NV>
-__device__ __forceinline__ void inv_row(const T* buf, int nvec, int s, int dir, int off, const T* f, int taps,
+template <typename T, int L, bool FMA, int NV, int S, int DIR, bool FULL>
+__device__ __forceinline__ void inv_row_ct(const T* buf, int nvec, int off, const T* f, T (&acc)[NV][VT<T>::V]) {
+  constexpr int V = VT<T>::V;
+  using vec = typename VT<T>::v;
+  static_assert(S % V == 0 && (L - 1) * S * (int)sizeof(T) < 65536, "aligned reads, 16-bit offsets");
+  const T* const low = buf + off - (DIR > 0 ? 0 : (L - 1) * S);
+  for_vecs<L, NV, FULL>(nvec, [&](int k, int w) {
+    const int t0 = w * V;
+    const unsigned a0 = lds_base(low + t0);
+#pragma unroll
+    for (int i = 0; i < L; ++i) {
+      const vec v = lds_vec_at<vec>(a0 + (unsigned)((DIR > 0 ? i : L - 1 - i) * S * (int)sizeof(T)));
+      vmadd<FMA>(acc[k], v, f[i]);
+      if ((i & 3) == 3) __builtin_amdgcn_sched_barrier(0);
+    }
+#pragma unroll
+    for (int e = 0; e < V; ++e) asm volatile("" : "+v"(acc[k][e]));
+  });
+}
+
+template <typename T, int L, bool FMA, int NV, bool FULL = false>
+__device__ __forceinline__ void inv_row(const T* buf, int nvec, int s, int dir, int off, const T* f, int taps, int ct,
                                         T (&acc)[NV][VT<T>::V]) {
   constexpr int V = VT<T>::V;
   if constexpr (L > 0) {
     if ((off & (V - 1)) == 0) {
       if (s == 1) {
-        if (dir > 0) return inv_row_t<T, L, FMA, NV, 1, 1>(buf, nvec, s, dir, off, f, taps, acc);
-        return inv_row_t<T, L, FMA, NV, 1, -1>(buf, nvec, s, dir, off, f, taps, acc);
+        if (dir > 0) return inv_row_t<T, L, FMA, NV, 1, 1, FULL>(buf, nvec, s, dir, off, f, taps, acc);
+        return inv_row_t<T, L, FMA, NV, 1, -1, FULL>(buf, nvec, s, dir, off, f, taps, acc);
       }
       if constexpr (V == 4) {
         if (s == 2) {
-          if (dir > 0) return inv_row_t<T, L, FMA, NV, 2, 1>(buf, nvec, s, dir, off, f, taps, acc);
-          return inv_row_t<T, L, FMA, NV, 2, -1>(buf, nvec, s, dir, off, f, taps, acc);
+          if (dir > 0) return inv_row_t<T, L, FMA, NV, 2, 1, FULL>(buf, nvec, s, dir, off, f, taps, acc);
+          return inv_row_t<T, L, FMA, NV, 2, -1, FULL>(buf, nvec, s, dir, off, f, taps, acc);
         }
       }
-      if (dir > 0) return inv_row_t<T, L, FMA, NV, 0, 1>(buf, nvec, s, dir, off, f, taps, acc);
-      return inv_row_t<T, L, FMA, NV, 0, -1>(buf, nvec, s, dir, off, f, taps, acc);
-    }
-  }
-  inv_row_t<T, L, FMA, NV, -1, 1>(buf, nvec, s, dir, off, f, taps, acc);
+      if constexpr (L <= 8) {
+        if (ct) {
+          switch (s) {
+#define VW_CASE(n)                                                                                  \
+            case n:                                                                                 \
+              if constexpr (n % V == 0) {                                                           \
+                if (dir > 0) return inv_row_ct<T, L, FMA, NV, n, 1, FULL>(buf, nvec, off, f, acc);  \
+                return inv_row_ct<T, L, FMA, NV, n, -1, FULL>(buf, nvec, off, f, acc);              \
+              }                                                                                     \
+              break;
+            VW_CT_SPACINGS(VW_CASE)
+#undef VW_CASE
+            default: break;
+          }
+        }
+      }
+      if (dir > 0) return inv_row_t<T, L, FMA, NV, 0, 1, FULL>(buf, nvec, s, dir, off, f, taps, acc);
+      return inv_row_t<T, L, FMA, NV, 0, -1, FULL>(buf, nvec, s, dir, off, f, taps, acc);
+    }
+  }
+  inv_row_t<T, L, FMA, NV, -1, 1, FULL>(buf, nvec, s, dir, off, f, taps, acc);
 }
 
 template <typename T, int NV>
@@ -600,25 +673,26 @@
 #pragma unroll
   for (int e = 0; e < V; ++e) z = nf_step<T>(v[e], z);
 }
-template <typename T, int L, int NV, int V>
+template <typename T, int L, int NV, int V, bool FULL = false>
 __device__ __forceinline__ void nf_probe_rows(T& z, const T (&v)[NV][V], int nvec) {
-  for_vecs<L, NV>(nvec, [&](int k, int) { nf_probe<T, V>(z, v[k]); });
+  for_vecs<L, NV, FULL>(nvec, [&](int k, int) { nf_probe<T, V>(z, v[k]); });
 }
 template <typename T>
 __device__ __forceinline__ void nf_flag_row(int* flag, long long b, T z) {
   if (__any(z != z) && (threadIdx.x & 63) == 0) flag[b] = 1;
 }
 
-template <typename T, int L, bool FMA, int NV, bool VALIDATE, bool NFP = false>
+template <typename T, int L, bool FMA, int NV, bool VALIDATE, bool NFP = false, bool FULL = false>
 __device__ __forceinline__ void fwd_level(const FwdArgs<T>& p, const T* X, int nvec, const LevelDesc& lv, T* dout,
                                           T* aout, bool vec_ok, unsigned long long flat0, T (&areg)[NV][VT<T>::V],
                                           T* nf = nullptr) {
   constexpr int V = VT<T>::V;
   const int N = p.N;
-  fwd_row<T, L, FMA, NV>(X, nvec, lv.s, p.lo, p.hi, p.taps, [&](int k, int w, const T (&al)[V], const T (&ah)[V]) {
+  const int ct = VALIDATE ? 0 : p.level_ct;
+  fwd_row<T, L, FMA, NV, FULL>(X, nvec, lv.s, p.lo, p.hi, p.taps, ct, [&](int k, int w, const T (&al)[V], const T (&ah)[V]) {
     const int t0 = w * V;
-    store_vec<VW_FWD_STORE_AUX>(dout, t0, N, vec_ok, ah);
-    if (aout) store_vec<VW_FWD_STORE_AUX>(aout, t0, N, vec_ok, al);
+    store_vec<VW_FWD_STORE_AUX, FULL>(dout, t0, N, vec_ok, ah);
+    if (aout) store_vec<VW_FWD_STORE_AUX, FULL>(aout, t0, N, vec_ok, al);
     if constexpr (VALIDATE) {
       check_out<T>(1, p.bad, flat0, t0, N, ah);
       check_out<T>(1, p.bad, flat0, t0, N, al);
@@ -791,7 +865,7 @@
   }
 }
 
-template <typename T, int L, bool FMA, int NV>
+template <typename T, int L, bool FMA, int NV, bool FULL>
 __global__ void __attribute__((amdgpu_flat_work_group_size(1, NV <= 4 ? 512 : 1024), amdgpu_waves_per_eu(4)))
 k_forward_persist(const FwdArgs<T> p) {
   constexpr int V = VT<T>::V;
@@ -823,10 +897,10 @@
       }
       T* dout = p.details + ((size_t)(j - 1) * (size_t)p.B + (size_t)b) * (size_t)N;
       T* aout = (j == p.J) ? p.approx + b * (size_t)N : nullptr;
-      if (p.nf_flag) fwd_level<T, L, FMA, NV, false, true>(p, X, nvec, lv, dout, aout, true, 0ull, areg, &nf);
-      else fwd_level<T, L, FMA, NV, false>(p, X, nvec, lv, dout, aout, true, 0ull, areg);
+      if (p.nf_flag) fwd_level<T, L, FMA, NV, false, true, FULL>(p, X, nvec, lv, dout, aout, true, 0ull, areg, &nf);
+      else fwd_level<T, L, FMA, NV, false, false, FULL>(p, X, nvec, lv, dout, aout, true, 0ull, areg);
       if (j < p.J) {
-        regs_to_level<T, L, NV>(Y, areg, nvec, N, p.lv[j], p.npow2, (const T*)nullptr);
+        regs_to_level<T, L, NV, FULL>(Y, areg, nvec, N, p.lv[j], p.npow2, (const T*)nullptr);
         T* t = X; X = Y; Y = t;
       }
     }
@@ -924,9 +998,9 @@
       load_row_regs<T, NV>(dreg, p.details + (size_t)(j - 2) * plane + b * (size_t)N, N, nvec, vec_ok,
                            p.lv[j - 2].use_d == 0);
     zero_regs<T, NV>(acc);
-    inv_row<T, L, FMA, NV>(X, nvec, lv.s, lv.dir_a, lv.off_a, p.lo, p.taps, acc);
+    inv_row<T, L, FMA, NV>(X, nvec, lv.s, lv.dir_a, lv.off_a, p.lo, p.taps, p.level_ct, acc);
     lds_barrier();
-    inv_row<T, L, FMA, NV>(Y, nvec, lv.s, lv.dir_d, lv.off_d, p.hi, p.taps, acc);
+    inv_row<T, L, FMA, NV>(Y, nvec, lv.s, lv.dir_d, lv.off_d, p.hi, p.taps, p.level_ct, acc);
     if (j > 1) regs_to_level<T, L, NV>(X, acc, nvec, N, p.lv[j - 2], 0, (const T*)nullptr);
   }
   for_vecs<L, NV>(nvec, [&](int k, int w) { store_vec<VW_INV_STORE_AUX>(p.y + b * (size_t)N, w * V, N, vec_ok, acc[k]); });
@@ -938,7 +1012,7 @@
 #ifndef VW_INV_W
 #define VW_INV_W 6
 #endif
-template <typename T, int L, bool FMA, int NV>
+template <typename T, int L, bool FMA, int NV, bool FULL = false>
 __global__ void VW_FUSED_BOUNDS(NV, VW_FUSED_W(L, VW_INV_W)) k_inverse_seq(const InvArgs<T> p) {
   constexpr int V = VT<T>::V;
   extern __shared__ __attribute__((aligned(16))) unsigned char smem[];
@@ -954,40 +1028,40 @@
   T dreg[NV][V];
   T nf = T(0);
   const bool nfp = p.nf_flag != nullptr;
-  load_row_regs<T, NV>(acc, p.approx + b * (size_t)N, N, nvec, vec_ok, p.approx_zero != 0);
-  load_row_regs<T, NV>(dreg, p.details + (size_t)(p.J - 1) * plane + b * (size_t)N, N, nvec, vec_ok,
+  load_row_regs<T, NV, FULL>(acc, p.approx + b * (size_t)N, N, nvec, vec_ok, p.approx_zero != 0);
+  load_row_regs<T, NV, FULL>(dreg, p.details + (size_t)(p.J - 1) * plane + b * (size_t)N, N, nvec, vec_ok,
                        p.lv[p.J - 1].use_d == 0);
   wait_vmem();
-  regs_to_level<T, L, NV>(R, acc, nvec, N, p.lv[p.J - 1], 0, (const T*)nullptr, p.approx_zero != 0);
+  regs_to_level<T, L, NV, FULL>(R, acc, nvec, N, p.lv[p.J - 1], 0, (const T*)nullptr, p.approx_zero != 0);
 
   for (int j = p.J; j >= 1; --j) {
     const LevelDesc lv = p.lv[j - 1];
     lds_barrier();
 #if VW_INV_LATE_PF
     if (j < p.J)
-      load_row_regs<T, NV>(dreg, p.details + (size_t)(j - 1) * plane + b * (size_t)N, N, nvec, vec_ok,
+      load_row_regs<T, NV, FULL>(dreg, p.details + (size_t)(j - 1) * plane + b * (size_t)N, N, nvec, vec_ok,
                            lv.use_d == 0);
 #endif
     zero_regs<T, NV>(acc);
-    inv_row<T, L, FMA, NV>(R, nvec, lv.s, lv.dir_a, lv.off_a, p.lo, p.taps, acc);
+    inv_row<T, L, FMA, NV, FULL>(R, nvec, lv.s, lv.dir_a, lv.off_a, p.lo, p.taps, p.level_ct, acc);
     lds_barrier();
     wait_vmem();
-    regs_to_level<T, L, NV>(R, dreg, nvec, N, lv, 0, (const T*)nullptr, lv.use_d == 0, p.thr, thr_of(j), p.soft);
+    regs_to_level<T, L, NV, FULL>(R, dreg, nvec, N, lv, 0, (const T*)nullptr, lv.use_d == 0, p.thr, thr_of(j), p.soft);
 #if !VW_INV_LATE_PF
     if (j > 1)
-      load_row_regs<T, NV>(dreg, p.details + (size_t)(j - 2) * plane + b * (size_t)N, N, nvec, vec_ok,
+      load_row_regs<T, NV, FULL>(dreg, p.details + (size_t)(j - 2) * plane + b * (size_t)N, N, nvec, vec_ok,
                            p.lv[j - 2].use_d == 0);
 #endif
     lds_barrier();
-    inv_row<T, L, FMA, NV>(R, nvec, lv.s, lv.dir_d, lv.off_d, p.hi, p.taps, acc);
+    inv_row<T, L, FMA, NV, FULL>(R, nvec, lv.s, lv.dir_d, lv.off_d, p.hi, p.taps, p.level_ct, acc);
     if (j > 1) {
       lds_barrier();
-      regs_to_level<T, L, NV>(R, acc, nvec, N, p.lv[j - 2], 0, (const T*)nullptr);
-    }
-  }
-  for_vecs<L, NV>(nvec, [&](int k, int w) { store_vec<VW_INV_STORE_AUX>(p.y + b * (size_t)N, w * V, N, vec_ok, acc[k]); });
+      regs_to_level<T, L, NV, FULL>(R, acc, nvec, N, p.lv[j - 2], 0, (const T*)nullptr);
+    }
+  }
+  for_vecs<L, NV, FULL>(nvec, [&](int k, int w) { store_vec<VW_INV_STORE_AUX, FULL>(p.y + b * (size_t)N, w * V, N, vec_ok, acc[k]); });
   if (nfp) {
-    nf_probe_rows<T, L, NV, V>(nf, acc, nvec);
+    nf_probe_rows<T, L, NV, V, FULL>(nf, acc, nvec);
     nf_flag_row<T>(p.nf_flag, b, nf);
   }
 }
@@ -1540,7 +1614,7 @@
     lds_barrier();
     zero_regs<T, NV>(acc);
     if (m) blk_inv_any<T, L, FMA, NV>(R, lo, p.blk_tight, vb, m, flo, acc);
-    else inv_row<T, L, FMA, NV>(R, nvec, lv.s, 1, 0, flo, p.taps, acc);
+    else inv_row<T, L, FMA, NV>(R, nvec, lv.s, 1, 0, flo, p.taps, 0, acc);
     lds_barrier();
     wait_vmem();
     stage_std(dreg, j, lv.use_d == 0 ? 1 : (p.thr ? 2 : 0), thr_of(j));
@@ -1549,7 +1623,7 @@
                            p.lv[j - 2].use_d == 0);
     lds_barrier();
     if (m) blk_inv_any<T, L, FMA, NV>(R, lo, p.blk_tight, vb, m, fhi, acc);
-    else inv_row<T, L, FMA, NV>(R, nvec, lv.s, 1, 0, fhi, p.taps, acc);
+    else inv_row<T, L, FMA, NV>(R, nvec, lv.s, 1, 0, fhi, p.taps, 0, acc);
     if (j > 1) {
       lds_barrier();
 #pragma unroll
diff --git a/vectorwave_amd/csrc/vw_fwd.hip b/vectorwave_amd/csrc/vw_fwd.hip
--- a/vectorwave_amd/csrc/vw_fwd.hip
+++ b/vectorwave_amd/csrc/vw_fwd.hip
@@ -60,9 +60,9 @@
 }
 template hipError_t launch_forward_blk<VW_T>(const FwdArgs<VW_T>&, int, int, bool, int, hipStream_t);
 
-template <typename T, int L, bool FMA, int NV>
+template <typename T, int L, bool FMA, int NV, bool FULL>
 static hipError_t run_forward_persist(const FwdArgs<T>& a, int threads, int lds, hipStream_t st) {
-  auto k = k_forward_persist<T, L, FMA, NV>;
+  auto k = k_forward_persist<T, L, FMA, NV, FULL>;
   static LdsOnce configured;
   hipError_t e = set_lds(k, lds, &configured);
   if (e != hipSuccess) return e;
@@ -88,7 +88,8 @@
 template <typename T, int L, bool FMA>
 static hipError_t run_forward_persist_nv(const FwdArgs<T>& a, int threads, int lds, int nv, hipStream_t st) {
   (void)nv;
-  return run_forward_persist<T, L, FMA, 4>(a, threads, lds, st);
+  return a.level_ct ? run_forward_persist<T, L, FMA, 4, true>(a, threads, lds, st)
+                    : run_forward_persist<T, L, FMA, 4, false>(a, threads, lds, st);
 }
 
 template <typename T>
diff --git a/vectorwave_amd/csrc/vw_internal.h b/vectorwave_amd/csrc/vw_internal.h
--- a/vectorwave_amd/csrc/vw_internal.h
+++ b/vectorwave_amd/csrc/vw_internal.h
@@ -52,6 +52,7 @@
   int vec_io;
   int unrolled;
   int dma_nt;
+  int level_ct;
   int validate;
   int rev;
   unsigned long long* bad;
@@ -79,6 +80,8 @@
   int vec_io;
   int pair;
   int unrolled;
+  int level_ct;
+  int full;
   int db;
   int blk;
   int approx_zero;
diff --git a/vectorwave_amd/csrc/vw_inv.hip b/vectorwave_amd/csrc/vw_inv.hip
--- a/vectorwave_amd/csrc/vw_inv.hip
+++ b/vectorwave_amd/csrc/vw_inv.hip
@@ -5,14 +5,19 @@
 
 template <typename T, int L, bool FMA, int NV>
 static hipError_t run_inverse_fused_nv(const InvArgs<T>& a, int threads, int lds, hipStream_t st) {
-  static LdsOnce configured_pair, configured_seq, configured_db, configured_blk;
+  static LdsOnce configured_pair, configured_seq, configured_db, configured_blk, configured_full;
   const bool blk = L > 0 && NV != 2 && a.blk && !a.pair && !a.db;
   auto k = a.pair ? k_inverse_fused<T, L, FMA, NV> : a.db ? k_inverse_db<T, L, FMA, NV> : k_inverse_seq<T, L, FMA, NV>;
   if constexpr (NV != 2) {
     if (blk) k = k_inverse_blk<T, (L > 0 ? L : 2), FMA, NV>;
   }
+  bool full = false;
+  if constexpr (NV == 4 && L > 0 && L <= 8) {
+    full = a.full && !a.pair && !a.db && !blk;
+    if (full) k = k_inverse_seq<T, L, FMA, NV, true>;
+  }
   hipError_t e = set_lds(k, lds, a.pair ? &configured_pair : a.db ? &configured_db
-                                 : blk ? &configured_blk : &configured_seq);
+                                 : blk ? &configured_blk : full ? &configured_full : &configured_seq);
   if (e != hipSuccess) return e;
   hipLaunchKernelGGL(k, dim3((unsigned)a.B), dim3(threads), lds, st, a);
   return hipGetLastError();
```

New measurement: 46950, median of 6. 1.02x the previous value.
